# HKUDS/GPT-ST

Hardware: AMD Instinct MI355X
Metric: pretrain steps/sec at (B=32,T=12,N=170,C=64) (higher is better)
Workload: dtype f32; 1 GPU; BASELINE configs[1]: PEMS08-shape synthetic pretrain step, per-GPU B=32 T=12 N=170 C=64 base=1, epoch 200/300 (adaptive mask + KL), fwd+loss+bwd+clip+Adam, hipGraph=True, 4 full optimiser steps on 4 different resident batches per graph replay; global_batch=32, parallelism=dp1

## Files before the change

### gpt-st_amd/csrc/cap_mfma.hip

```cpp
#include "mfma_tile.h"
#include "poolgen_dev.h"
#include <vector>
#ifdef GPTST_DEBUG
__device__ long long g_cap_ts[64];
static thread_local int g_cap_dbg = 0;
extern "C" int gptst_tune2(int v) { g_cap_dbg = v; return 0; }
extern "C" int gptst_cap_ts(long long* out) { return (int)hipMemcpyFromSymbol(out, HIP_SYMBOL(g_cap_ts), sizeof(long long) * 64); }
#else
static constexpr int g_cap_dbg = 0;
#endif

GPTST_STAMP_TABLES(capmfma)
GPTST_HANDOFF_COUNTER(capmfma)

#define CM_NT 512
#define CM_NW (CM_NT / 64)

__host__ __device__ inline int cm_rows(int N) { return (N + 15) / 16 * 16; }
__host__ __device__ inline int cm_np(int N) { return ((N + 3) / 4 * 4) | 1; }
__host__ __device__ inline int cm_hsp(int HS) { return (HS + 15) / 16 * 16; }

template <int C>
__device__ __forceinline__ void cm_type1(const float* __restrict__ Ps, const float* __restrict__ cs, float* __restrict__ S, int N,
                                         int NP, int HSP) {
// ... 499 lines not shown
                const bool valid = i < nz;
                const int k = valid ? i / LPR : 0, c4 = i % LPR;
                const float4 sv = valid ? sv4[u] : f4zero(), rt = valid ? rt4[u] : f4zero(), g = valid ? g4[u] : f4zero();
                const float4 u_ = f4add(rt, sv);
                const float q = group_sum<LPR>(f4dot(u_, u_));
                const float udg = group_sum<LPR>(f4dot(u_, g));
                const float r = sqrtf(q), den = (1.f + q) * (r + 1e-8f);
                const float gq = q / den;
                float gp = 0.f;
                if (r > 0.f) gp = (den - q * ((r + 1e-8f) + (1.f + q) * 0.5f / r)) / (den * den);
                const float k2 = 2.f * gp * udg;
                const float4 du = make_float4(fmaf(k2, u_.x, gq * g.x), fmaf(k2, u_.y, gq * g.y), fmaf(k2, u_.z, gq * g.z), fmaf(k2, u_.w, gq * g.w));
                if (valid) {
                    st4(Gs + k * P + 4 * c4, make_float4(du.x * lrelu_grad_from_out(rt.x), du.y * lrelu_grad_from_out(rt.y),
                                                         du.z * lrelu_grad_from_out(rt.z), du.w * lrelu_grad_from_out(rt.w)));
                    if (k >= k0 && k < k0 + nown) {
                        const float tm = tmpl[k / HS];
                        st4((GLOBAL ? Uo : Vs) + (k - k0) * P + 4 * c4, du);
                        st4(Zo + (k - k0) * P + 4 * c4, make_float4(sv.x + tm, sv.y + tm, sv.z + tm, sv.w + tm));
                    }
                }
            }
        }
        for (int i = CM_NT + tid; i < nd; i += CM_NT) st4(dyns + 4 * i, ld4(db + 4 * (size_t)i));
        for (int i = CM_NT + tid; i < nh; i += CM_NT) st4(Hs + (i / LPR) * P + 4 * (i % LPR), ld4(hb + 4 * (size_t)i));
    }
    __syncthreads();
    {
        const int lane = tid & 63, wave = tid >> 6, li = lane & 15, kk = lane >> 4;
        if (wave < C / 16) {
            for (int jt = 0; jt < HT; jt += 16) {
                const int ja = jt + li;
                f32x4 acc = {0.f, 0.f, 0.f, 0.f};
                const float* ar = dyns + min(ja, HT - 1) * KK + kk;
                const float* br = Gs + kk * P + 16 * wave + li;
                const int ns4 = KK / 4;
                int s4 = 0;
                for (; s4 + 6 <= ns4; s4 += 6) {
                    float av[6], bv[6];
#pragma unroll
                    for (int u = 0; u < 6; ++u) { av[u] = ja < HT ? ar[4 * (s4 + u)] : 0.f; bv[u] = br[4 * (s4 + u) * P]; }
#pragma unroll
                    for (int u = 0; u < 6; ++u) acc = __builtin_amdgcn_mfma_f32_16x16x4f32(av[u], bv[u], acc, 0, 0, 0);
                }
                for (; s4 < ns4; ++s4) acc = __builtin_amdgcn_mfma_f32_16x16x4f32(ja < HT ? ar[4 * s4] : 0.f, br[4 * s4 * P], acc, 0, 0, 0);
#pragma unroll
                for (int r = 0; r < 4; ++r) {
                    const int jj = jt + 4 * kk + r;
                    if (jj < HT) dHs[jj * P + 16 * wave + li] = acc[r] * lrelu_grad_from_out(Hs[jj * P + 16 * wave + li]);
                }
            }
        }
    }
    __syncthreads();
    for (int i = tid; i < HT * nown; i += CM_NT) {
        const int j = i / nown, h = i % nown, k = k0 + h;
        float acc = 0.f;
#pragma unroll 4
        for (int c4 = 0; c4 < LPR; ++c4) {
            acc += f4dot(ld4(Hs + j * P + 4 * c4), ld4(Gs + k * P + 4 * c4));
            acc += f4dot(ld4(dHs + j * P + 4 * c4), ld4(Zo + h * P + 4 * c4));
        }
        ddyn[((size_t)b * HT + j) * KK + k] = acc;
    }
    for (int i = tid; i < nown * LPR; i += CM_NT) {
        const int h = i / LPR, c4 = i % LPR, k = k0 + h;
        float4 acc = f4zero();
#pragma unroll 8
        for (int j = 0; j < HT; ++j) acc = f4fma(dyns[j * KK + k], ld4(dHs + j * P + 4 * c4), acc);
        if (GLOBAL) {
            typedef int i32x4_ __attribute__((ext_vector_type(4)));
            const float4 r4 = f4add(ld4(Uo + h * P + 4 * c4), acc);
            const f32x4 v4 = {r4.x, r4.y, r4.z, r4.w};
            const __amdgpu_buffer_rsrc_t rs = __builtin_amdgcn_make_buffer_rsrc(dSg + ((size_t)b * KK + k0) * C, 0, nown * C * 4, 0x00020000);
            __builtin_amdgcn_raw_buffer_store_b128(__builtin_bit_cast(i32x4_, v4), rs, (h * C + 4 * c4) * 4, 0, 16);
        } else {
            st4(Vs + h * P + 4 * c4, f4add(ld4(Vs + h * P + 4 * c4), acc));
        }
    }
    __syncthreads();
}

template <bool JOBS> struct RouteJobs { };
template <> struct RouteJobs<true> { PJobs t; int npool, npb, neb, first; };

template <int C, int ROLES, bool LIN = false, bool JOBS = false>
__global__ __launch_bounds__(CM_NT, 4) void cap_route_bwd2_kernel(const float* __restrict__ X, const float* __restrict__ Wp,
                                                                  const float* __restrict__ bp, const float* __restrict__ c,
                                                                  const float* __restrict__ dc1, const float* __restrict__ dS,
                                                                  float* __restrict__ dY, float* __restrict__ dlogit, int N, int HS,
                                                                  int region2, CrossBwdArgs cx, LinArgs lin, RouteJobs<JOBS> jr, int nfull, int nhr) {
    if constexpr (JOBS) {
        if ((int)blockIdx.x >= jr.first) {
            extern __shared__ __attribute__((aligned(16))) float jsmem[];
            const int half = (int)(threadIdx.x >> 8), tid_ = (int)(threadIdx.x & 255);
            float (*fold)[PG_MAXK][65] = reinterpret_cast<float (*)[PG_MAXK][65]>(jsmem + half * (4 * PG_MAXK * 65));
            const int w = (int)blockIdx.x - jr.first, wp = (jr.npb + 1) >> 1;
            if (w < wp) {
                const int vb = __builtin_amdgcn_readfirstlane(2 * w + half);
                if (vb < jr.npb) {
                    int p = 0;
                    for (int q = 1; q < jr.npool; ++q) if (vb >= jr.t.j[q].blk0) p = q;
                    const PJob& a = jr.t.j[p];
                    if (((a.cols | a.ldx) & 3) == 0) pj_bwd_pool<4>(a, vb - a.blk0, fold, tid_); else pj_bwd_pool<1>(a, vb - a.blk0, fold, tid_);
                } else {
                    __syncthreads();
                }
            } else {
                const int vb = __builtin_amdgcn_readfirstlane(2 * (w - wp) + half);
                if (vb < jr.neb) {
                    int p = jr.npool;
                    for (int q = jr.npool + 1; q < jr.t.n; ++q) if (vb >= jr.t.j[q].blk0) p = q;
                    const PJob& a = jr.t.j[p];
                    const int rel = vb - a.blk0;
                    if (((a.cols | a.ldx) & 3) == 0) pj_bwd_emb<4>(a, rel % a.nbx, rel / a.nbx, tid_); else pj_bwd_emb<1>(a, rel % a.nbx, rel / a.nbx, tid_);
                }
            }
            return;
        }
    }
    using T = Tile<C>;
    constexpr int P = T::PITCH, LPR = C / 4, RPP = CM_NT / LPR;
    extern __shared__ __attribute__((aligned(16))) float smem[];
    const int NR = cm_rows(N), NP = cm_np(N), HSP = cm_hsp(HS);
    float* Ys = smem;
    float* Wl = Ys + NR * P;
    float* cs = Wl;
    float* dcs = cs + HSP * NP;
    float* Vs = Wl + region2;
    float* gq = Vs + HSP * P;
    float* qq = gq + NR;
    const int tid = threadIdx.x, lane = tid & 63, wave = tid >> 6;
    unsigned* s_ok = reinterpret_cast<unsigned*>(qq + NR);
    GPTST_WG_BEGIN(); GPTST_STAMP(0);
    const int blk = (int)blockIdx.x;
    int ru;
    if (ROLES && blk < cx.nB) {
        constexpr int TS = 12 / CX_SPLIT;
        cap_cross_bwd_prologue<C, true>(cx.dv, cx.s, cx.Rt, cx.Ht, cx.dyn, cx.tmpl, cx.ddyn, smem, nullptr, blk / CX_SPLIT,
                                                    (blk % CX_SPLIT) * TS, TS, cx.T, HS, cx.HT, cx.dSg);
        asm volatile("s_waitcnt vmcnt(0)" ::: "memory");
        __syncthreads();
        if (tid == 0) { gptst_publish_fence(); __hip_atomic_store(cx.flags + blk, 1u, __ATOMIC_RELAXED, __HIP_MEMORY_SCOPE_AGENT); }
        GPTST_STAMP(1);
        if (blk >= nhr) { GPTST_WG_END(); return; }
        ru = nfull + blk;
        __syncthreads();
    } else {
        const int r = ROLES ? blk - cx.nB : blk;
        ru = r < nfull ? r : r + nhr;
    }
    int bt = ru, tlo = 0, thi = NR / 16;
    if (ru >= nfull) {
        const int k = ru - nfull, th = (NR / 16 + 1) >> 1;
        bt = nfull + (k >> 1);
        if (k & 1) tlo = th; else thi = th;
    }
    const float* Xbt = X + (size_t)bt * N * C;
    const bool fold = !ROLES && cx.dv != nullptr;
    if constexpr (!ROLES) {
        if (fold) {
            for (int i = tid; i < HSP * P; i += CM_NT) Vs[i] = 0.f;
            __syncthreads();
            cap_cross_bwd_prologue<C, false>(cx.dv, cx.s, cx.Rt, cx.Ht, cx.dyn, cx.tmpl, cx.ddyn, smem, Vs, bt / cx.T, bt % cx.T, 1, cx.T, HS, cx.HT);
        }
    }
    GPTST_STAMP(1);

    if constexpr (C == 64) {
        const int j = lane & 15, kk = lane >> 4;
        float4 a[4];
        cm_fetch_a16(a, Xbt, tlo + wave, N, j, kk);
        const float4 b4 = ld4(bp + 4 * j);
        load_w_lds<C, CM_NT>(Wl, Wp, 1, tid);
        if (!fold) for (int i = tid; i < HSP * P; i += CM_NT) Vs[i] = 0.f;
        __syncthreads();
        GPTST_STAMP(2);
        float4 bv[4][4];
        cm_load_bfrag(bv, Wl, j, kk);
        for (int tile = tlo + wave; tile < thi; tile += CM_NW) {
            if (tile != tlo + wave) cm_fetch_a16(a, Xbt, tile, N, j, kk);
            float4 y[4];
            cm_tile16(a, bv, b4, y);
#pragma unroll
            for (int r = 0; r < 4; ++r) {
                const int n = tile * 16 + kk * 4 + r;
                const float4 v = n < N ? y[r] : f4zero();
                const float q = group_sum<16>(f4dot(v, v));
                st4(Ys + n * P + 4 * j, v);
                if (j == 0) { qq[n] = q; gq[n] = q / ((1.f + q) * (sqrtf(q) + 1e-8f)); }
            }
        }
        __syncthreads();
        GPTST_STAMP(3);
        for (int i = tid; i < 2 * HSP * NP; i += CM_NT) cs[i] = 0.f;
// ... 245 lines not shown
                const float g0 = (sgn >> (4 * r)) & 1u ? 1.f : LRELU_SLOPE, g1 = (sgn >> (4 * r)) & 2u ? 1.f : LRELU_SLOPE;
                const float g2 = (sgn >> (4 * r)) & 4u ? 1.f : LRELU_SLOPE, g3 = (sgn >> (4 * r)) & 8u ? 1.f : LRELU_SLOPE;
                if (lin.out != nullptr) {
                    o4.x = fmaf(rv[r].x, g0, o4.x); o4.y = fmaf(rv[r].y, g1, o4.y); o4.z = fmaf(rv[r].z, g2, o4.z); o4.w = fmaf(rv[r].w, g3, o4.w);
                } else {
                    o4 = f4add(o4, rv[r]);
                    if (lin.premul) { o4.x *= g0; o4.y *= g1; o4.z *= g2; o4.w *= g3; }
                }
                if (nn < N) st4(lin.dX + ((size_t)bt * N + nn) * 64 + 4 * j_, o4);
            }
        }
#undef CRL_LOAD_RES
        GPTST_STAMP(7);
        {
            const int ot = wave_ >> 1, it0 = 2 * (wave_ & 1);
            f32x4 w0 = {0.f, 0.f, 0.f, 0.f}, w1 = {0.f, 0.f, 0.f, 0.f};
            const float* xcol = Xbt + 16 * it0 + j_;
            const float* ycol = Ys + 16 * ot + j_;
            constexpr int UB = 11;
            const int sbeg = 4 * tlo, nsteps = 4 * thi;
            float b0[UB], b1[UB], n0[UB], n1[UB];
#define CRL_LOADX(d0, d1, s0_) _Pragma("unroll") for (int u = 0; u < UB; ++u) {                          \
                const int n_ = min(4 * ((s0_) + u) + kk_, N - 1);                                          \
                d0[u] = xcol[(size_t)n_ * 64]; d1[u] = xcol[(size_t)n_ * 64 + 16]; }
            CRL_LOADX(b0, b1, sbeg);
#pragma unroll 1
            for (int s0 = sbeg; s0 < nsteps; s0 += UB) {
                if (s0 + UB < nsteps) { CRL_LOADX(n0, n1, s0 + UB); }
                float av[UB];
#pragma unroll
                for (int u = 0; u < UB; ++u) av[u] = (s0 + u < nsteps) ? ycol[(4 * (s0 + u) + kk_) * P] : 0.f;
                SB();
#pragma unroll
                for (int u = 0; u < UB; ++u) {
                    w0 = __builtin_amdgcn_mfma_f32_16x16x4f32(av[u], b0[u], w0, 0, 0, 0);
                    w1 = __builtin_amdgcn_mfma_f32_16x16x4f32(av[u], b1[u], w1, 0, 0, 0);
                }
                SB();
#pragma unroll
                for (int u = 0; u < UB; ++u) { b0[u] = n0[u]; b1[u] = n1[u]; }
            }
#undef CRL_LOADX
            float* dw = lin.dWp + (size_t)ru * 64 * 64;
#pragma unroll
            for (int r = 0; r < 4; ++r) {
                const int o = 16 * ot + 4 * kk_ + r;
                dw[o * 64 + 16 * it0 + j_] = w0[r];
                dw[o * 64 + 16 * it0 + 16 + j_] = w1[r];
            }
        }
        GPTST_STAMP(8);
    }
    GPTST_WG_END();
}

thread_local int g_cap_split_roles = 1;
thread_local int g_cap_bwd_noroles = 0;

template <int C>
static int launch_route_bwd2(const float* X, const float* Wp, const float* bp, const float* c, const float* dc1, const float* dS,
                             float* dY, float* dlogit, int BT, int N, int HS, hipStream_t st, CrossBwdArgs cx = CrossBwdArgs{nullptr, nullptr, nullptr, nullptr, nullptr, nullptr, nullptr, 0, 0, nullptr, nullptr, 0},
                             LinArgs lin = LinArgs{nullptr, nullptr, nullptr, nullptr, nullptr, 0}, RouteJobs<true>* jobs = nullptr, int nsplit = 0) {
    if (HS > 64) return GPTST_ESHAPE;
    if (nsplit < 0 || nsplit > BT || (nsplit > 0 && (C != 64 || lin.dX == nullptr))) return GPTST_EARG;
    const int nfull = BT - nsplit;
    if (lin.dX != nullptr && C != 64) return GPTST_ESHAPE;
    const int NR = cm_rows(N), NP = cm_np(N), HSP = cm_hsp(HS);
    size_t r2 = (size_t)C * C, need = (size_t)2 * HSP * NP;
    if (need > r2) r2 = need;
    r2 = (r2 + 3) & ~(size_t)3;
    const size_t smem = ((size_t)NR * Tile<C>::PITCH + r2 + (size_t)HSP * Tile<C>::PITCH + 2 * (size_t)NR + 4) * sizeof(float);
    if (smem > 160 * 1024) return GPTST_ESHAPE;
    if (cx.dv) {
        const size_t need_cx = (size_t)(cx.T * HS + 2 * cx.HT + HS) * Tile<C>::PITCH + (size_t)cx.HT * cx.T * HS;
        if (need_cx > (size_t)NR * Tile<C>::PITCH + r2 || (cx.HT * cx.T * HS) % 4 != 0) return GPTST_ESHAPE;
    }
    if (cx.nB > 0) {
        const int no = (12 / CX_SPLIT) * HS;
        const size_t need_r = (size_t)(cx.T * HS + 2 * cx.HT + 2 * no) * Tile<C>::PITCH + (size_t)cx.HT * cx.T * HS;
        if (smem > 80 * 1024 || BT + cx.nB > 512 || cx.T != 12 || need_r > (size_t)NR * Tile<C>::PITCH + r2) cx.nB = 0;
    }
    const int nhr = (cx.nB > 0 && g_cap_split_roles) ? (2 * nsplit < cx.nB ? 2 * nsplit : cx.nB) : 0;
    const int NU = BT + nsplit - nhr;
    if (jobs != nullptr && !(cx.nB > 0 && lin.dX != nullptr && smem >= 2 * (4 * PG_MAXK * 65) * sizeof(float))) return GPTST_ESHAPE;
    if (jobs != nullptr) {
        static size_t curJ = 0;
        if (smem > curJ) { (void)hipFuncSetAttribute((const void*)cap_route_bwd2_kernel<C, 1, true, true>, hipFuncAttributeMaxDynamicSharedMemorySize, (int)smem); curJ = smem; }
        jobs->first = NU + cx.nB;
        const int njw = ((jobs->npb + 1) >> 1) + ((jobs->neb + 1) >> 1);
        hipLaunchKernelGGL((cap_route_bwd2_kernel<C, 1, true, true>), dim3(NU + cx.nB + njw), dim3(CM_NT), smem, st, X, Wp, bp, c, dc1, dS, dY, dlogit, N, HS, (int)r2, cx, lin, *jobs, nfull, nhr);
        GPTST_CHECK_LAUNCH();
        return GPTST_OK;
    }
    if (cx.nB > 0 && lin.dX != nullptr) {
        static size_t curRL = 0;
        if (smem > curRL) { (void)hipFuncSetAttribute((const void*)cap_route_bwd2_kernel<C, 1, true>, hipFuncAttributeMaxDynamicSharedMemorySize, (int)smem); curRL = smem; }
        hipLaunchKernelGGL((cap_route_bwd2_kernel<C, 1, true>), dim3(NU + cx.nB), dim3(CM_NT), smem, st, X, Wp, bp, c, dc1, dS, dY, dlogit, N, HS, (int)r2, cx, lin, RouteJobs<false>{}, nfull, nhr);
        GPTST_CHECK_LAUNCH();
        return GPTST_OK;
    }
    if (cx.nB > 0) {
        static size_t curR = 0;
        if (smem > curR) { (void)hipFuncSetAttribute((const void*)cap_route_bwd2_kernel<C, 1>, hipFuncAttributeMaxDynamicSharedMemorySize, (int)smem); curR = smem; }
        hipLaunchKernelGGL((cap_route_bwd2_kernel<C, 1>), dim3(BT + cx.nB), dim3(CM_NT), smem, st, X, Wp, bp, c, dc1, dS, dY, dlogit, N, HS, (int)r2, cx, lin, RouteJobs<false>{}, BT, 0);
        GPTST_CHECK_LAUNCH();
        return GPTST_OK;
    }
    if (lin.dX != nullptr) {
        static size_t curL = 0;
        if (smem > curL) { (void)hipFuncSetAttribute((const void*)cap_route_bwd2_kernel<C, 0, true>, hipFuncAttributeMaxDynamicSharedMemorySize, (int)smem); curL = smem; }
        hipLaunchKernelGGL((cap_route_bwd2_kernel<C, 0, true>), dim3(NU), dim3(CM_NT), smem, st, X, Wp, bp, c, dc1, dS, dY, dlogit, N, HS, (int)r2, cx, lin, RouteJobs<false>{}, nfull, nhr);
        GPTST_CHECK_LAUNCH();
        return GPTST_OK;
    }
    static size_t cur = 0;
    if (smem > cur) { (void)hipFuncSetAttribute((const void*)cap_route_bwd2_kernel<C, 0>, hipFuncAttributeMaxDynamicSharedMemorySize, (int)smem); cur = smem; }
    hipLaunchKernelGGL((cap_route_bwd2_kernel<C, 0>), dim3(BT), dim3(CM_NT), smem, st, X, Wp, bp, c, dc1, dS, dY, dlogit, N, HS, (int)r2, cx, lin, RouteJobs<false>{}, BT, 0);
    GPTST_CHECK_LAUNCH();
    return GPTST_OK;
}

GPTST_INTERNAL int gptst_cap_route_bwd_v1(const float* X, const float* Wp, const float* bp, const float* c, const float* dc1,
                                      const float* dS, float* dY, float* dlogit, int BT, int N, int C, int HS, void* stream);

extern "C" int gptst_cap_route_bwd(const float* X, const float* Wp, const float* bp, const float* c, const float* dc1,
                                   const float* dS, float* dY, float* dlogit, int BT, int N, int C, int HS, void* stream) {
    if (!X || !Wp || !bp || !c || !dc1 || !dS || !dY || !dlogit) return GPTST_EARG;
    int rc = GPTST_ESHAPE;
    if (C == 64) rc = launch_route_bwd2<64>(X, Wp, bp, c, dc1, dS, dY, dlogit, BT, N, HS, (hipStream_t)stream);
    if (rc == GPTST_ESHAPE) return gptst_cap_route_bwd_v1(X, Wp, bp, c, dc1, dS, dY, dlogit, BT, N, C, HS, stream);
    return rc;
}

extern "C" int gptst_cap_cross_route_bwd(const float* X, const float* Wp, const float* bp, const float* c, const float* dc1, const float* dv,
                                         const float* s, const float* Rt, const float* Ht, const float* dyn, const float* tmpl, float* dY,
                                         float* dlogit, float* ddyn, float* dS_ws, void* flags, int B, int T, int N, int C, int HS, int HT, void* stream) {
    if (!X || !Wp || !bp || !c || !dc1 || !dv || !s || !Rt || !Ht || !dyn || !tmpl || !dY || !dlogit || !ddyn || B <= 0 || T <= 0) return GPTST_EARG;
    if (C != 64) return GPTST_ESHAPE;
    const bool roles = dS_ws != nullptr && flags != nullptr && !g_cap_bwd_noroles;
    return launch_route_bwd2<64>(X, Wp, bp, c, dc1, nullptr, dY, dlogit, B * T, N, HS, (hipStream_t)stream,
                                 CrossBwdArgs{dv, s, Rt, Ht, dyn, tmpl, ddyn, T, HT, roles ? dS_ws : nullptr, roles ? (unsigned*)flags : nullptr, roles ? B * CX_SPLIT : 0});
}

extern "C" int gptst_cap_cross_route_lin_bwd(const float* X, const float* Wp, const float* bp, const float* c, const float* dc1, const float* dv,
                                             const float* s, const float* Rt, const float* Ht, const float* dyn, const float* tmpl,
                                             const float* dPre, const float* out, int premul, float* dX, float* dWp, float* dbp, float* dlogit,
                                             float* ddyn, float* dS_ws, void* flags, int B, int T, int N, int C, int HS, int HT, void* stream) {
    if (!X || !Wp || !bp || !c || !dc1 || !dv || !s || !Rt || !Ht || !dyn || !tmpl || !dPre || !dX || !dWp || !dbp || !dlogit || !ddyn || B <= 0 ||
        T <= 0 || (out && premul)) return GPTST_EARG;
    if (C != 64) return GPTST_ESHAPE;
    const bool roles = dS_ws != nullptr && flags != nullptr && !g_cap_bwd_noroles;
    return launch_route_bwd2<64>(X, Wp, bp, c, dc1, nullptr, nullptr, dlogit, B * T, N, HS, (hipStream_t)stream,
                                 CrossBwdArgs{dv, s, Rt, Ht, dyn, tmpl, ddyn, T, HT, roles ? dS_ws : nullptr, roles ? (unsigned*)flags : nullptr, roles ? B * CX_SPLIT : 0},
                                 LinArgs{dPre, out, dX, dWp, dbp, premul});
}

GPTST_INTERNAL int gptst_cap_rec_bwd_v1(const float* drec, const float* c, const float* v, float* dc1, float* dv, int BT, int N, int C,
                                    int HS, void* stream);

GPTST_INTERNAL int gptst_pj_reduce_table(PJobs* t, int njobs, const int* kind, const void* const* emb, const void* const* x, const void* const* pool,
                                         const void* const* out, const int* R, const int* K, const int* cols, const int* nsplit, const int* ldx,
                                         int* npool, int* npb, int* neb);
extern "C" int gptst_pool_jobs(int njobs, const int* kind, const void* const* emb, const void* const* x, const void* const* pool,
                               const void* const* out, const int* R, const int* K, const int* cols, const int* nsplit, const int* ldx, void* stream);
extern "C" int gptst_cap_route_roles_ok(int B, int T, int N, int C, int HS, int HT) {
    if (C != 64 || HS > 64 || HS <= 0 || B <= 0 || N <= 0 || T != 12 || g_cap_bwd_noroles) return 0;
    const int NR = cm_rows(N), NP = cm_np(N), HSP = cm_hsp(HS), BT = B * T, nB = B * CX_SPLIT;
    size_t r2 = (size_t)C * C, need = (size_t)2 * HSP * NP;
    if (need > r2) r2 = need;
    r2 = (r2 + 3) & ~(size_t)3;
    const size_t smem = ((size_t)NR * Tile<64>::PITCH + r2 + (size_t)HSP * Tile<64>::PITCH + 2 * (size_t)NR + 4) * sizeof(float);
    const int no = (12 / CX_SPLIT) * HS;
    const size_t need_r = (size_t)(T * HS + 2 * HT + 2 * no) * Tile<64>::PITCH + (size_t)HT * T * HS;
    if (smem > 80 * 1024 || BT + nB > 512 || need_r > (size_t)NR * Tile<64>::PITCH + r2 || (HT * T * HS) % 4 != 0) return 0;
    return smem >= 2 * (4 * PG_MAXK * 65) * sizeof(float) ? 1 : 0;
}

thread_local int g_cap_split = 0;
static int cap_cu_count() {
    static thread_local int dev_cached = -1, ncu = 0;
    int dev = 0;
    if (hipGetDevice(&dev) != hipSuccess) return 0;
    if (dev != dev_cached) {
        if (hipDeviceGetAttribute(&ncu, hipDeviceAttributeMultiprocessorCount, dev) != hipSuccess) ncu = 0;
        dev_cached = dev;
    }
    return ncu;
}
extern "C" int gptst_cap_split_units(int BT, int N, int C, int HS) {
    if (C != 64 || HS <= 0 || HS > 64 || N < 32 || BT <= 0) return 0;
    if (g_cap_split >= 0) return g_cap_split < BT ? g_cap_split : BT;
    const int ncu = cap_cu_count();
    if (ncu <= 0 || BT <= ncu || 2 * BT > 3 * ncu) return 0;
    return BT - ncu;
}

static int cap_cross_route_lin_bwd_any(const float* X, const float* Wp, const float* bp, const float* c, const float* dc1, const float* dv,
                                       const float* s, const float* Rt, const float* Ht, const float* dyn, const float* tmpl,
                                       const float* dPre, const float* out, int premul, float* dX, float* dWp, float* dbp, float* dlogit,
                                       float* ddyn, float* dS_ws, void* flags, int B, int T, int N, int C, int HS, int HT, int nsplit,
                                       int njobs, const int* jkind, const void* const* jemb, const void* const* jx, const void* const* jpool,
                                       const void* const* jout, const int* jR, const int* jK, const int* jcols, const int* jnsplit, const int* jldx,
                                       void* stream) {
    if (!X || !Wp || !bp || !c || !dc1 || !dv || !s || !Rt || !Ht || !dyn || !tmpl || !dPre || !dX || !dWp || !dbp || !dlogit || !ddyn || B <= 0 ||
        T <= 0 || (out && premul) || nsplit < 0 || nsplit > B * T) return GPTST_EARG;
    if (njobs < 0 || (njobs && (!jkind || !jemb || !jx || !jpool || !jout || !jR || !jK || !jcols || !jnsplit))) return GPTST_EARG;
    if (C != 64) return GPTST_ESHAPE;
    if (nsplit > 0 && N < 32) return GPTST_EARG;
    const bool roles = dS_ws != nullptr && flags != nullptr && !g_cap_bwd_noroles;
    const CrossBwdArgs cx{dv, s, Rt, Ht, dyn, tmpl, ddyn, T, HT, roles ? dS_ws : nullptr, roles ? (unsigned*)flags : nullptr, roles ? B * CX_SPLIT : 0};
    const LinArgs lin{dPre, out, dX, dWp, dbp, premul};
    if (njobs > 0 && roles) {
        RouteJobs<true> jr;
        if (gptst_pj_reduce_table(&jr.t, njobs, jkind, jemb, jx, jpool, jout, jR, jK, jcols, jnsplit, jldx, &jr.npool, &jr.npb, &jr.neb) == GPTST_OK) {
            const int rc = launch_route_bwd2<64>(X, Wp, bp, c, dc1, nullptr, nullptr, dlogit, B * T, N, HS, (hipStream_t)stream, cx, lin, &jr, nsplit);
            if (rc != GPTST_ESHAPE) return rc;
        }
    }
    const int rc = launch_route_bwd2<64>(X, Wp, bp, c, dc1, nullptr, nullptr, dlogit, B * T, N, HS, (hipStream_t)stream, cx, lin, nullptr, nsplit);
    if (rc || njobs == 0) return rc;
    return gptst_pool_jobs(njobs, jkind, jemb, jx, jpool, jout, jR, jK, jcols, jnsplit, jldx, stream);
}

extern "C" int gptst_cap_cross_route_lin_bwd_jobs(const float* X, const float* Wp, const float* bp, const float* c, const float* dc1, const float* dv,
                                                  const float* s, const float* Rt, const float* Ht, const float* dyn, const float* tmpl,
                                                  const float* dPre, const float* out, int premul, float* dX, float* dWp, float* dbp, float* dlogit,
                                                  float* ddyn, float* dS_ws, void* flags, int B, int T, int N, int C, int HS, int HT,
                                                  int njobs, const int* jkind, const void* const* jemb, const void* const* jx, const void* const* jpool,
                                                  const void* const* jout, const int* jR, const int* jK, const int* jcols, const int* jnsplit, const int* jldx,
                                                  void* stream) {
    return cap_cross_route_lin_bwd_any(X, Wp, bp, c, dc1, dv, s, Rt, Ht, dyn, tmpl, dPre, out, premul, dX, dWp, dbp, dlogit, ddyn, dS_ws, flags, B, T, N, C, HS,
                                       HT, 0, njobs, jkind, jemb, jx, jpool, jout, jR, jK, jcols, jnsplit, jldx, stream);
}

extern "C" int gptst_cap_cross_route_lin_bwd_split(const float* X, const float* Wp, const float* bp, const float* c, const float* dc1, const float* dv,
                                                   const float* s, const float* Rt, const float* Ht, const float* dyn, const float* tmpl,
                                                   const float* dPre, const float* out, int premul, float* dX, float* dWp, float* dbp, float* dlogit,
                                                   float* ddyn, float* dS_ws, void* flags, int B, int T, int N, int C, int HS, int HT, int nsplit,
                                                   int njobs, const int* jkind, const void* const* jemb, const void* const* jx, const void* const* jpool,
                                                   const void* const* jout, const int* jR, const int* jK, const int* jcols, const int* jnsplit, const int* jldx,
                                                   void* stream) {
    return cap_cross_route_lin_bwd_any(X, Wp, bp, c, dc1, dv, s, Rt, Ht, dyn, tmpl, dPre, out, premul, dX, dWp, dbp, dlogit, ddyn, dS_ws, flags, B, T, N, C, HS,
                                       HT, nsplit, njobs, jkind, jemb, jx, jpool, jout, jR, jK, jcols, jnsplit, jldx, stream);
}

extern "C" int gptst_cap_rec_bwd(const float* drec, const float* c, const float* v, float* dc1, float* dv, int BT, int N, int C, int HS,
                                 void* stream) {
    if (!drec || !c || !v || !dc1 || !dv) return GPTST_EARG;
    if (C == 64 && HS <= 64) {
        const int NR = cm_rows(N), NP = cm_np(N), HSP = cm_hsp(HS);
        const size_t smem = ((size_t)NR * Tile<64>::PITCH + (size_t)(HSP + HS) * NP + (size_t)HSP * Tile<64>::PITCH + (size_t)HSP * 64) * sizeof(float);
        if (smem <= 160 * 1024) {
            static size_t cur = 0;
            if (smem > cur) { hipFuncSetAttribute((const void*)cap_rec_bwd2_kernel<64>, hipFuncAttributeMaxDynamicSharedMemorySize, (int)smem); cur = smem; }
            hipLaunchKernelGGL((cap_rec_bwd2_kernel<64>), dim3(BT), dim3(CM_NT), smem, (hipStream_t)stream, drec, c, v, dc1, dv, N, HS);
            GPTST_CHECK_LAUNCH();
            return GPTST_OK;
        }
    }
    return gptst_cap_rec_bwd_v1(drec, c, v, dc1, dv, BT, N, C, HS, stream);
}
```

### gpt-st_amd/csrc/poolgen.hip

```cpp
#include "common.h"
#include "poolgen_dev.h"
#include <algorithm>
#include <vector>

#define PG_ROWS 16


#ifndef PJ_OCC
#define PJ_OCC 6
#endif

#define PG_MAXROWS 64
template <int V>
__device__ __forceinline__ void pj_fwd(const PJob& a, int bx, int by, int rows, float* __restrict__ embs ) {
    const float* __restrict__ emb = a.emb;
    const float* __restrict__ pool = a.pool;
    float* __restrict__ out = a.out;
    const int cols = a.cols, K = a.K, R = a.R;
    const int r0 = by * rows, nr = min(R, r0 + rows) - r0;
    for (int i = threadIdx.x; i < nr * PG_MAXK; i += 256) {
        const int r = i / PG_MAXK, k = i % PG_MAXK;
        embs[i] = k < K ? emb[(size_t)(r0 + r) * K + k] : 0.f;
    }
    const int c4 = bx * 256 + threadIdx.x;
    const bool ok = V * c4 < cols;
    float4 pv[PG_MAXK];
#pragma unroll
    for (int k = 0; k < PG_MAXK; ++k) pv[k] = (k < K && ok) ? ldv<V>(pool + (size_t)k * cols + V * c4) : f4zero();
    __syncthreads();
    if (!ok) return;
#pragma unroll 2
    for (int r = 0; r < nr; ++r) {
        float4 acc = f4zero();
#pragma unroll
        for (int k = 0; k < PG_MAXK; k += 4) {
            const float4 e = ld4(embs + r * PG_MAXK + k);
            acc = f4fma(e.x, pv[k], acc); acc = f4fma(e.y, pv[k + 1], acc); acc = f4fma(e.z, pv[k + 2], acc); acc = f4fma(e.w, pv[k + 3], acc);
        }
        stv<V>(out + (size_t)(r0 + r) * cols + V * c4, acc);
    }
}




#define PJ_DET_T 1024
__global__ __launch_bounds__(PJ_DET_T) void pool_emb_det_kernel(PJobs t) {
    __shared__ float fold[PJ_DET_T / 64][16][17];
    const int lane = threadIdx.x & 63, wave = threadIdx.x >> 6;
    const int i = lane & 15, kk = lane >> 4;
    int q0 = 0;
    for (int q = 1; q < t.n; ++q) if ((int)blockIdx.x >= t.j[q].blk0) q0 = q;
    const int g0 = t.j[q0].blk0, tile = blockIdx.x - g0;
    f32x4 acc = {0.f, 0.f, 0.f, 0.f};
    int chunk_id = 0, first = q0;
    for (int q = 0; q <= q0; ++q) {
        const PJob& a = t.j[q];
        if (a.blk0 != g0) continue;
        if (q < first) first = q;
        const bool v4 = ((a.cols | a.ldx) & 3) == 0;
        const int nch = (a.cols + 255) / 256;
        for (int ch = 0; ch < nch; ++ch, ++chunk_id) {
            if ((chunk_id & (PJ_DET_T / 64 - 1)) != wave) continue;
            if (v4) pj_emb_accum<4>(a, tile, ch, acc, threadIdx.x); else pj_emb_accum<1>(a, tile, ch, acc, threadIdx.x);
        }
    }
#pragma unroll
    for (int r = 0; r < 4; ++r) fold[wave][kk * 4 + r][i] = acc[r];
    __syncthreads();
    if (threadIdx.x < 256) {
        const int R = t.j[first].R, K = t.j[first].K;
        const int rr = threadIdx.x >> 4, k = threadIdx.x & 15, orow = tile * 16 + rr;
        float s = 0.f;
#pragma unroll
        for (int w = 0; w < PJ_DET_T / 64; ++w) s += fold[w][rr][k];
        if (orow < R && k < K) t.j[first].out[(size_t)orow * K + k] += s;
    }
}

__global__ __launch_bounds__(256, PJ_OCC) void pool_jobs_kernel(PJobs t, int fwd_rows, int fwd_mfma) {
    __shared__ __attribute__((aligned(16))) float fold[4][PG_MAXK][65];
    int p = 0;
    for (int q = 1; q < t.n; ++q) if ((int)blockIdx.x >= t.j[q].blk0) p = q;
    const PJob& a = t.j[p];
    const int rel = blockIdx.x - a.blk0, bx = rel % a.nbx, by = rel / a.nbx;
    const bool v4 = ((a.cols | a.ldx) & 3) == 0;
    if (a.kind == PJ_FWD) {
        if (v4 && fwd_mfma) pj_fwd_mfma(a, bx, by, fwd_mfma, threadIdx.x);
        else if (v4) pj_fwd<4>(a, bx, by, fwd_rows, &fold[0][0][0]);
        else pj_fwd<1>(a, bx, by, fwd_rows, &fold[0][0][0]);
    }
    else if (a.kind == PJ_GRAM) pj_gram(a, rel, &fold[0][0][0], 256);
    else if (a.kind == PJ_BWD_POOL) { if (v4) pj_bwd_pool<4>(a, bx, fold, threadIdx.x); else pj_bwd_pool<1>(a, bx, fold, threadIdx.x); }
    else { if (v4) pj_bwd_emb<4>(a, bx, by, threadIdx.x); else pj_bwd_emb<1>(a, bx, by, threadIdx.x); }
}

thread_local int g_pg_rows = PG_ROWS;
thread_local int g_pg_sort = 1;
thread_local int g_pg_mfma = 1;
static int pj_blocks(PJob& j) {
    const int V = ((j.cols | j.ldx) & 3) ? 1 : 4;
    if (j.kind == PJ_FWD && V == 4 && g_pg_mfma) { j.nbx = (j.cols + 255) / 256; return j.nbx * ((j.R + PG_MFMA_ROWS - 1) / PG_MFMA_ROWS); }
    if (j.kind == PJ_FWD) { j.nbx = ((j.cols + V - 1) / V + 255) / 256; return j.nbx * ((j.R + g_pg_rows - 1) / g_pg_rows); }
    if (j.kind == PJ_GRAM) { const int nb = pj_gram_rows(j.K, j.cols); j.nbx = (j.R + nb - 1) / nb; return j.nbx; }
    if (j.kind == PJ_BWD_POOL) { j.nbx = (j.cols + 16 * V - 1) / (16 * V); return j.nbx; }
    j.nbx = (j.R + 15) / 16;
    return j.nbx * (((j.cols + 255) / 256 + 3) / 4);
}

extern "C" int gptst_pool_jobs_gram_rows(int K, int cols) { return (K <= 0 || K > PG_MAXK || cols <= 0 || cols % 12) ? 0 : pj_gram_rows(K, cols); }

static int pj_launch(PJobs& t, hipStream_t st) {
    int nb = 0;
    for (int p = 0; p < t.n; ++p) {
        PJob& j = t.j[p];
        if (j.R <= 0 || j.K <= 0 || j.K > PG_MAXK || j.cols <= 0 || j.nsplit <= 0 || !j.out) return GPTST_EARG;
        if ((j.kind == PJ_FWD || j.kind == PJ_BWD_POOL || j.kind == PJ_GRAM) && !j.emb) return GPTST_EARG;
        if (j.kind == PJ_GRAM && (!j.pool || j.cols % 12 || pj_gram_rows(j.K, j.cols) <= 0)) return GPTST_EARG;
        if ((j.kind == PJ_BWD_POOL || j.kind == PJ_BWD_EMB) && !j.x) return GPTST_EARG;
        if ((j.kind == PJ_FWD || j.kind == PJ_BWD_EMB) && !j.pool) return GPTST_EARG;
        j.blk0 = nb;
        if (j.ldx <= 0) j.ldx = j.cols;
        if (j.ldx < j.cols) return GPTST_EARG;
        nb += pj_blocks(j);
    }
    if (nb == 0) return GPTST_OK;
    hipLaunchKernelGGL(pool_jobs_kernel, dim3(nb), dim3(256), 0, st, t, g_pg_rows, g_pg_mfma ? PG_MFMA_ROWS : 0);
    GPTST_CHECK_LAUNCH();
    return GPTST_OK;
}

GPTST_INTERNAL int gptst_pj_embed_table(PJobs* t, int njobs, const int* kind, const void* const* emb, const void* const* pool, const void* const* out,
                                        const int* R, const int* K, const int* cols, int* nf, int* nvb, int* ngw) {
    if (njobs > PJ_MAX || !g_pg_mfma) return GPTST_ESHAPE;
    t->n = 0;
    *nf = *nvb = *ngw = 0;
    for (int pass = 0; pass < 2; ++pass) {
        for (int p = 0; p < njobs; ++p) {
            const int kd = kind ? kind[p] : (int)PJ_FWD;
            if (kd != PJ_FWD && kd != PJ_GRAM) return GPTST_ESHAPE;
            if ((kd == PJ_GRAM) != (pass == 1)) continue;
            PJob j{(const float*)emb[p], nullptr, (const float*)pool[p], (float*)out[p], R[p], K[p], cols[p], 1, 0, kd, 0, cols[p]};
            if (!j.emb || !j.pool || !j.out || j.R <= 0 || j.K <= 0 || j.K > PG_MAXK || j.cols <= 0) return GPTST_EARG;
            if (kd == PJ_FWD) {
                if (j.cols & 3) return GPTST_ESHAPE;
                j.blk0 = *nvb; *nvb += pj_blocks(j); ++*nf;
            } else {
                if (j.cols % 12 || pj_gram_rows(j.K, j.cols) <= 0) return GPTST_EARG;
                j.blk0 = *ngw; *ngw += pj_blocks(j);
            }
            t->j[t->n++] = j;
        }
    }
    return GPTST_OK;
}

GPTST_INTERNAL int gptst_pj_reduce_table(PJobs* t, int njobs, const int* kind, const void* const* emb, const void* const* x, const void* const* pool,
                                         const void* const* out, const int* R, const int* K, const int* cols, const int* nsplit, const int* ldx,
                                         int* npool, int* npb, int* neb) {
    if (njobs > PJ_MAX || g_deterministic) return GPTST_ESHAPE;
    t->n = 0;
    *npool = *npb = *neb = 0;
    for (int pass = 0; pass < 2; ++pass) {
        for (int p = 0; p < njobs; ++p) {
            if (kind[p] != PJ_BWD_POOL && kind[p] != PJ_BWD_EMB) return GPTST_ESHAPE;
            if ((kind[p] == PJ_BWD_EMB) != (pass == 1)) continue;
            PJob j{(const float*)emb[p], (const float*)x[p], (const float*)pool[p], (float*)out[p], R[p], K[p], cols[p], nsplit[p], 0, kind[p], 0, ldx ? ldx[p] : 0};
            if (j.R <= 0 || j.K <= 0 || j.K > PG_MAXK || j.cols <= 0 || j.nsplit <= 0 || !j.out || !j.x) return GPTST_EARG;
            if (kind[p] == PJ_BWD_POOL ? !j.emb : !j.pool) return GPTST_EARG;
            if (j.ldx <= 0) j.ldx = j.cols;
            if (j.ldx < j.cols) return GPTST_EARG;
            if (pass == 0) { j.blk0 = *npb; *npb += pj_blocks(j); ++*npool; }
            else { j.blk0 = *neb; *neb += pj_blocks(j); }
            t->j[t->n++] = j;
        }
    }
    return GPTST_OK;
}

extern "C" int gptst_pool_jobs(int njobs, const int* kind, const void* const* emb, const void* const* x, const void* const* pool,
                               const void* const* out, const int* R, const int* K, const int* cols, const int* nsplit, const int* ldx,
                               void* stream) {
    if (njobs < 0 || (njobs && (!kind || !emb || !x || !pool || !out || !R || !K || !cols || !nsplit))) return GPTST_EARG;
    for (int p = 0; p < njobs; ++p) if (kind[p] < PJ_FWD || kind[p] > PJ_GRAM) return GPTST_EARG;
    auto job = [&](int p) {
        return PJob{(const float*)emb[p], (const float*)x[p], (const float*)pool[p], (float*)out[p], R[p], K[p], cols[p], nsplit[p],
                    0, kind[p], 0, ldx ? ldx[p] : 0};
    };
    const bool det = g_deterministic != 0;
    std::vector<int> ord(njobs);
    std::vector<long> cost(njobs);
    for (int p = 0; p < njobs; ++p) {
        ord[p] = p;
        const long rr = (long)R[p] * nsplit[p], cc = cols[p];
        cost[p] = kind[p] == PJ_BWD_POOL ? rr * (cc < 64 ? cc : 64) : kind[p] == PJ_BWD_EMB ? 16L * nsplit[p] * (cc < 1024 ? cc : 1024)
                : kind[p] == PJ_FWD ? 64L * (cc < 256 ? cc : 256) : 1L;
    }
    if (g_pg_sort) std::stable_sort(ord.begin(), ord.end(), [&](int a, int b) { return cost[a] > cost[b]; });
    PJobs t; t.n = 0;
    for (int o = 0; o < njobs; ++o) {
        const int p = ord[o];
        if (det && kind[p] == PJ_BWD_EMB) continue;
        t.j[t.n++] = job(p);
        if (t.n == PJ_MAX) { const int rc = pj_launch(t, (hipStream_t)stream); if (rc) return rc; t.n = 0; }
    }
    if (t.n) { const int rc = pj_launch(t, (hipStream_t)stream); if (rc) return rc; }
    if (!det) return GPTST_OK;
    PJobs g; g.n = 0;
    int nb = 0;
    auto flush = [&]() {
        if (g.n) { hipLaunchKernelGGL(pool_emb_det_kernel, dim3(nb), dim3(PJ_DET_T), 0, (hipStream_t)stream, g); g.n = 0; nb = 0; }
    };
    for (int p = 0; p < njobs; ++p) {
        if (kind[p] != PJ_BWD_EMB) continue;
        bool seen = false;
        for (int q = 0; q < p; ++q) if (kind[q] == PJ_BWD_EMB && out[q] == out[p]) seen = true;
        if (seen) continue;
        int members = 0;
        for (int q = p; q < njobs; ++q) if (kind[q] == PJ_BWD_EMB && out[q] == out[p]) ++members;
        if (members > PJ_MAX) return GPTST_EARG;
        if (g.n + members > PJ_MAX) flush();
        const int tiles = (R[p] + 15) / 16;
        for (int q = p; q < njobs; ++q) {
            if (kind[q] != PJ_BWD_EMB || out[q] != out[p]) continue;
            if (R[q] != R[p] || K[q] != K[p]) return GPTST_EARG;
            PJob j = job(q);
            if (!j.x || !j.pool || !j.out || j.R <= 0 || j.K <= 0 || j.K > PG_MAXK || j.cols <= 0 || j.nsplit <= 0) return GPTST_EARG;
            if (j.ldx <= 0) j.ldx = j.cols;
            if (j.ldx < j.cols) return GPTST_EARG;
            j.blk0 = nb; j.nbx = tiles;
            g.j[g.n++] = j;
        }
        nb += tiles;
    }
    flush();
    GPTST_CHECK_LAUNCH();
    return GPTST_OK;
}

extern thread_local int g_wgrad_ns_override;
extern thread_local int g_wgrad_ns0_override;
extern thread_local int g_apply_v1;
extern thread_local int g_apply_tpw;
extern thread_local int g_tl_nb;
extern thread_local int g_wgrad_v1;
extern thread_local int g_apply128_v1;
extern thread_local int g_apply128_minwg;
extern thread_local int g_tl_mfma;
extern thread_local int g_cap_route_v2;
extern thread_local int g_cap_bwd_noroles;
extern thread_local int g_cap_split;
extern thread_local int g_cap_split_roles;
extern "C" int gptst_tune(int id, int value) {
    if (id == 15) g_tl_mfma = value;
    if (id == 20) g_cap_route_v2 = value;
    if (id == 23) g_cap_bwd_noroles = value;
    if (id == 25) g_cap_split = value;
    if (id == 26) g_cap_split_roles = value;
    if (id == 19) g_pg_sort = value;
    if (id == 1 && value > 0 && value <= PG_MAXROWS) g_pg_rows = value;
    if (id == 6 && value > 0) g_tl_nb = value;
    if (id == 2) g_wgrad_ns_override = value;
    if (id == 5) g_wgrad_ns0_override = value;
    if (id == 3) g_apply_v1 = value;
    if (id == 4) g_apply_tpw = value;
    if (id == 7) g_wgrad_v1 = value;
    if (id == 8) g_apply128_v1 = value;
    if (id == 24 && value > 0) g_apply128_minwg = value;
    if (id == 10) g_pg_mfma = value;
    return GPTST_OK;
}

extern "C" int gptst_poolgen_fwd_multi(const float* emb, int nprob, const void* pools, const void* outs, const int* cols, int R, int K,
                                       void* stream) {
    if (!emb || !pools || !outs || !cols || nprob <= 0 || nprob > PJ_MAX || K > PG_MAXK || K <= 0) return GPTST_EARG;
    PJobs t; t.n = nprob;
    for (int p = 0; p < nprob; ++p)
        t.j[p] = PJob{emb, nullptr, ((const float* const*)pools)[p], ((float* const*)outs)[p], R, K, cols[p], 1, 0, PJ_FWD, 0, 0};
    return pj_launch(t, (hipStream_t)stream);
}

extern "C" int gptst_poolgen_bwd_pool_multi(const float* emb, int nprob, const void* dWs, const void* dpools, const int* cols,
                                            const int* nsplit, int R, int K, void* stream) {
    if (!emb || !dWs || !dpools || !cols || nprob <= 0 || nprob > PJ_MAX || K > PG_MAXK || K <= 0) return GPTST_EARG;
    PJobs t; t.n = nprob;
    for (int p = 0; p < nprob; ++p)
        t.j[p] = PJob{emb, ((const float* const*)dWs)[p], nullptr, ((float* const*)dpools)[p], R, K, cols[p], nsplit ? nsplit[p] : 1, 0,
                      PJ_BWD_POOL, 0, 0};
    return pj_launch(t, (hipStream_t)stream);
}

extern "C" int gptst_poolgen_bwd_emb_multi(int nprob, const void* dWs, const void* pools, const int* cols, const int* nsplit, float* demb,
                                           int R, int K, void* stream) {
    if (!dWs || !pools || !cols || !demb || nprob <= 0 || nprob > PJ_MAX || K > PG_MAXK || K <= 0) return GPTST_EARG;
    PJobs t; t.n = nprob;
    for (int p = 0; p < nprob; ++p)
        t.j[p] = PJob{nullptr, ((const float* const*)dWs)[p], ((const float* const*)pools)[p], demb, R, K, cols[p], nsplit ? nsplit[p] : 1, 0,
                      PJ_BWD_EMB, 0, 0};
    return pj_launch(t, (hipStream_t)stream);
}

extern "C" int gptst_poolgen_fwd(const float* emb, const float* pool, float* out, int cols, const float* pool2, float* out2,
                                 int cols2, int R, int K, void* stream) {
    const float* pools[2] = {pool, pool2}; float* outs[2] = {out, out2}; int cc[2] = {cols, cols2};
    return gptst_poolgen_fwd_multi(emb, pool2 ? 2 : 1, pools, outs, cc, R, K, stream);
}

extern "C" int gptst_poolgen_bwd_pool(const float* emb, const float* dW, float* dpool, int cols, const float* dW2, float* dpool2,
                                      int cols2, int R, int nsplit, int K, void* stream) {
    const float* dWs[2] = {dW, dW2}; float* dps[2] = {dpool, dpool2}; int cc[2] = {cols, cols2}; int ns[2] = {nsplit, 1};
    return gptst_poolgen_bwd_pool_multi(emb, dW2 ? 2 : 1, dWs, dps, cc, ns, R, K, stream);
}

extern "C" int gptst_poolgen_bwd_emb(const float* dW, const float* pool, int cols, const float* dW2, const float* pool2, int cols2,
                                     float* demb, int R, int nsplit, int K, void* stream) {
    const float* dWs[2] = {dW, dW2}; const float* pls[2] = {pool, pool2}; int cc[2] = {cols, cols2}; int ns[2] = {nsplit, 1};
    return gptst_poolgen_bwd_emb_multi(dW2 ? 2 : 1, dWs, pls, cc, ns, demb, R, K, stream);
}
```

### gpt-st_amd/csrc/poolgen_dev.h

```cpp
#pragma once
#include "common.h"

#define PG_MAXK 16
#define PG_MFMA_ROWS 64
#define PJ_MAX 112
enum { PJ_FWD = 0, PJ_BWD_POOL = 1, PJ_BWD_EMB = 2, PJ_GRAM = 3 };
struct PJob {
    const float* emb;
    const float* x;
    const float* pool;
    float* out;
    int R, K, cols, nsplit;
    int blk0, kind, nbx, ldx;
};
struct PJobs { PJob j[PJ_MAX]; int n; };

__device__ __forceinline__ void pj_fwd_mfma(const PJob& a, int bx, int by, int rows, int tid) {
    const float* __restrict__ emb = a.emb;
    const float* __restrict__ pool = a.pool;
    float* __restrict__ out = a.out;
    const int cols = a.cols, K = a.K, R = a.R;
    const int lane = tid & 63, wave = tid >> 6, j = lane & 15, kk = lane >> 4;
    const int c = bx * 256 + wave * 64 + 4 * j;
    if (bx * 256 + wave * 64 >= cols) return;
    const bool cok = c < cols;
    const int nks = (K + 3) >> 2;
    float4 bf[4];
#pragma unroll
    for (int s = 0; s < 4; ++s) bf[s] = (cok && 4 * s + kk < K) ? ld4(pool + (size_t)(4 * s + kk) * cols + c) : f4zero();
    const int r0 = by * rows, r1 = min(R, r0 + rows);
    for (int rt = r0; rt < r1; rt += 16) {
        float av[4];
        const int row = rt + j;
#pragma unroll
        for (int s = 0; s < 4; ++s) av[s] = (row < r1 && 4 * s + kk < K) ? emb[(size_t)row * K + 4 * s + kk] : 0.f;
        f32x4 acc[4];
#pragma unroll
        for (int ct = 0; ct < 4; ++ct) acc[ct] = (f32x4){0.f, 0.f, 0.f, 0.f};
#pragma unroll
        for (int s = 0; s < 4; ++s) {
            if (s < nks) {
                acc[0] = __builtin_amdgcn_mfma_f32_16x16x4f32(av[s], bf[s].x, acc[0], 0, 0, 0);
                acc[1] = __builtin_amdgcn_mfma_f32_16x16x4f32(av[s], bf[s].y, acc[1], 0, 0, 0);
                acc[2] = __builtin_amdgcn_mfma_f32_16x16x4f32(av[s], bf[s].z, acc[2], 0, 0, 0);
                acc[3] = __builtin_amdgcn_mfma_f32_16x16x4f32(av[s], bf[s].w, acc[3], 0, 0, 0);
            }
        }
        if (cok) {
#pragma unroll
            for (int r = 0; r < 4; ++r) {
                const int orow = rt + 4 * kk + r;
                if (orow < r1) st4(out + (size_t)orow * cols + c, make_float4(acc[0][r], acc[1][r], acc[2][r], acc[3][r]));
            }
        }
    }
}

#define PJ_GRAM_SCR (4 * PG_MAXK * 65)
__host__ __device__ inline int pj_gram_rows(int K, int cols) {
    const int nb = (PJ_GRAM_SCR - K * cols) / cols;
    return nb > 16 ? 16 : nb;
}
__device__ __forceinline__ void pj_gram(const PJob& a, int bx, float* __restrict__ scr, int nt) {
    const int K = a.K, cols = a.cols, Hm = cols / 12, NB = pj_gram_rows(K, cols);
    float* pl = scr;
    float* As = scr + K * cols;
    const int r0 = bx * NB, nr = min(NB, a.R - r0);
    for (int i = threadIdx.x; i < K * cols; i += nt) pl[i] = a.pool[i];
    __syncthreads();
    for (int i = threadIdx.x; i < nr * cols; i += nt) {
        const int r = i / cols, c = i % cols;
        const float* __restrict__ e = a.emb + (size_t)(r0 + r) * K;
        float acc = 0.f;
        for (int k = 0; k < K; ++k) acc = fmaf(e[k], pl[k * cols + c], acc);
        As[i] = acc;
    }
    __syncthreads();
    for (int i = threadIdx.x; i < nr * 144; i += nt) {
        const int r = i / 144, t = (i % 144) / 12, u = i % 12;
        const float* ar = As + r * cols;
        float s = 0.f;
        for (int h = 0; h < Hm; ++h) s = fmaf(ar[h * 12 + t], ar[h * 12 + u], s);
        a.out[(size_t)(r0 + r) * 144 + i % 144] = s;
    }
}

#ifndef PJ_UC
#define PJ_UC 4
#endif
#ifndef PJ_NU
#define PJ_NU 4
#endif
template <int V> __device__ __forceinline__ float4 ldv(const float* p) { return ld4(p); }
template <> __device__ __forceinline__ float4 ldv<1>(const float* p) { return make_float4(*p, 0.f, 0.f, 0.f); }
template <int V> __device__ __forceinline__ void stv(float* p, float4 v) { st4(p, v); }
template <> __device__ __forceinline__ void stv<1>(float* p, float4 v) { *p = v.x; }

// ... 40 lines not shown
        }
    }
#pragma unroll
    for (int e = 0; e < V; ++e)
#pragma unroll
        for (int r = 0; r < 4; ++r) fold[wave][kk * 4 + r][V * j + e] = acc[e][r];
    __syncthreads();
    for (int o = tid; o < PG_MAXK * SLAB; o += 256) {
        const int k = o / SLAB, cc = o % SLAB, col = bx * SLAB + cc;
        if (k < K && col < cols) {
            float* d = dpool + (size_t)k * cols + col;
            *d += (fold[0][k][cc] + fold[1][k][cc]) + (fold[2][k][cc] + fold[3][k][cc]);
        }
    }
}

template <int V>
__device__ __forceinline__ void pj_emb_accum(const PJob& a, int bx, int chunk, f32x4& acc, int tid) {
    constexpr int chunk_cols = 256;
    const int lane = tid & 63;
    const int i = lane & 15, kk = lane >> 4;
    const int R = a.R, K = a.K;
    const int row = bx * 16 + i;
    const float* __restrict__ w = a.x;
    const float* __restrict__ pl = a.pool;
    const int cc = a.cols, ns = a.nsplit, ldx = a.ldx;
    const int cbeg = chunk * chunk_cols, cend = min(cc, cbeg + chunk_cols);
    if (cbeg >= cc) return;
    if (V == 4) {
        constexpr int UC = PJ_UC;
        const int rowc = min(row, R - 1), ic = min(i, K - 1);
        const bool rok = row < R, kok = i < K;
        for (int c0 = cbeg; c0 < cend; c0 += 16 * UC) {
            float4 av[UC], b[UC];
#pragma unroll
            for (int u = 0; u < UC; ++u) {
                const int c = min(c0 + 16 * u + 4 * kk, cc - 4);
                av[u] = ld4(w + (size_t)rowc * ldx + c);
                b[u] = ld4(pl + (size_t)ic * cc + c);
            }
            for (int s = 1; s < ns; ++s) {
#pragma unroll
                for (int u = 0; u < UC; ++u) {
                    const int c = min(c0 + 16 * u + 4 * kk, cc - 4);
                    av[u] = f4add(av[u], ld4(w + ((size_t)s * R + rowc) * ldx + c));
                }
            }
            SB();
#pragma unroll
            for (int u = 0; u < UC; ++u) {
                const bool ok = c0 + 16 * u + 4 * kk < cend;
                const float4 a_ = (ok && rok) ? av[u] : f4zero();
                const float4 b_ = (ok && kok) ? b[u] : f4zero();
                acc = __builtin_amdgcn_mfma_f32_16x16x4f32(a_.x, b_.x, acc, 0, 0, 0);
                acc = __builtin_amdgcn_mfma_f32_16x16x4f32(a_.y, b_.y, acc, 0, 0, 0);
                acc = __builtin_amdgcn_mfma_f32_16x16x4f32(a_.z, b_.z, acc, 0, 0, 0);
                acc = __builtin_amdgcn_mfma_f32_16x16x4f32(a_.w, b_.w, acc, 0, 0, 0);
            }
        }
    } else {
        for (int c = cbeg + kk; c < cend + kk; c += 4) {
            float av = 0.f, b = 0.f;
            if (c < cend) {
                if (row < R) for (int s = 0; s < ns; ++s) av += w[((size_t)s * R + row) * ldx + c];
                if (i < K) b = pl[(size_t)i * cc + c];
            }
            acc = __builtin_amdgcn_mfma_f32_16x16x4f32(av, b, acc, 0, 0, 0);
        }
    }
}

template <int V>
__device__ __forceinline__ void pj_bwd_emb(const PJob& a, int bx, int by, int tid) {
    const int lane = tid & 63, wave = tid >> 6;
    const int i = lane & 15, kk = lane >> 4;
    f32x4 acc = {0.f, 0.f, 0.f, 0.f};
    pj_emb_accum<V>(a, bx, by * 4 + wave, acc, tid);
#pragma unroll
    for (int r = 0; r < 4; ++r) {
        const int orow = bx * 16 + kk * 4 + r;
        if (orow < a.R && i < a.K && (by * 4 + wave) * 256 < a.cols) atomicAdd(a.out + (size_t)orow * a.K + i, acc[r]);
    }
}
```

### gpt-st_amd/engine.py

```python
import contextlib
import os
import threading

import torch

from . import _C, ops
from .ops import (EPI_ADD_DPRE, EPI_ADD_PREMUL, EPI_LRELU, EPI_PREMUL, EPI_PLAIN, EPI_RES_LRELU, MODE_NODE, MODE_SHARED, MODE_TIME, PRO_DPRE, PRO_NONE)

TF_NAMES = ("ln_day", "ln_week", "ln1", "ln2", "ln")


class ZeroArena:

    def __init__(self, device):
        self.device, self.buf, self.off, self.need = device, None, 0, 0

    def begin(self, zero=True):
        pending = None
        if self.buf is None or self.buf.numel() < self.need:
            self.buf = torch.zeros(max(self.need, 1), device=self.device) if self.need else None
        elif self.buf is not None:
            if zero:
                self.buf.zero_()
            else:
                pending = self.buf
        self.off, self.need = 0, 0
        return pending

    def zeros(self, *shape):
        n = 1
        for d in shape:
            n *= d
        n4 = (n + 3) // 4 * 4
        self.need += n4
        if self.buf is None or self.off + n4 > self.buf.numel():
            return torch.zeros(*shape, device=self.device)
        t = self.buf[self.off:self.off + n].view(*shape)
        self.off += n4
        return t


class _Context(threading.local):
    ARENA = None
    NODE_REDUCE = None
    NO_HANDOFFS = False


CTX = _Context()




class Reductions:

    def __init__(self):
        self.jobs = ops.PoolJobs()
        self.late = ops.PoolJobs()
        self.no_carry = False
        self.grams = []
        self.tf = []
        self.keep = []
        self.on_bucket = None
        self.nbucket = 0

    def take_carry(self, mb):
        if not CARRY_RED or self.no_carry or self.on_bucket is not None or CTX.NODE_REDUCE is not None or not self.jobs.jobs:
            return None
        take, rest, nb = [], [], 0.0
        for j in self.jobs.jobs:
            b = 4.0 * j[5] * j[7] * j[8] / 2 ** 20
            if j[0] in (ops.PoolJobs.BWD_POOL, ops.PoolJobs.BWD_EMB) and nb + b <= mb and len(take) < 100 and (j[7] | j[9]) % 4 == 0:
                take.append(j); nb += b
            else:
                rest.append(j)
        if not take:
            return None
        self.jobs.jobs = rest
        c = ops.PoolJobs()
        c.jobs = take
        return c

    def untake(self, carry):
        if carry is not None and carry.jobs:
            self.jobs.jobs = carry.jobs + self.jobs.jobs
            carry.jobs = []

    def gram(self, A, dG, dA, N, nsG):
        self.grams.append((A, dG, dA, N, nsG))

    def timefeat(self, p, g, pfx, tidx, dout, spg=False):
        B, T = tidx.shape[0], tidx.shape[1]
        rows, K = (B, T) if spg else (B * T, 1)
        self.tf.append((_tf_tensors(p, pfx), _tf_tensors(g, pfx), dout, rows, K))

    def flush_async(self, tidx):
        if getattr(self, "bucket_inline", False) and self.on_bucket is not None and self.nbucket == 0 and (self.jobs.jobs or self.late.jobs or self.grams or self.tf):
            self._run(tidx)
            self.fork_side.wait_stream(torch.cuda.current_stream())
            with torch.cuda.stream(self.fork_side):
                self.on_bucket(0)
            self.forked = True
            self.nbucket += 1

    def flush(self, tidx):
        self._run(tidx)
        if getattr(self, "forked", False):
            torch.cuda.current_stream().wait_stream(self.fork_side)
            self.forked = False

    def _run(self, tidx):
        gr, self.grams = sorted(self.grams, key=lambda t: t[0].data_ptr()), []
        while gr:
            A, dG, dA, N, nsG = gr.pop(0)
            while gr and gr[0][0].data_ptr() == A.data_ptr() + 4 * A.numel() and gr[0][1].data_ptr() == dG.data_ptr() + 4 * dG.numel() \
                    and gr[0][2].data_ptr() == dA.data_ptr() + 4 * dA.numel() and gr[0][3:] == (N, nsG):
                A2, dG2, dA2 = gr.pop(0)[:3]
                A = torch.as_strided(A, (A.shape[0] + A2.shape[0],) + tuple(A.shape[1:]), A.stride())
                dG = torch.as_strided(dG, (dG.shape[0] + dG2.shape[0],) + tuple(dG.shape[1:]), dG.stride())
                dA = torch.as_strided(dA, (dA.shape[0] + dA2.shape[0],) + tuple(dA.shape[1:]), dA.stride())
            ops.gram_bwd(A, dG, out=dA, layers=A.shape[0] // N, nsplit=nsG)
        self.jobs.jobs, self.late.jobs = self.jobs.jobs + self.late.jobs, []
        self.jobs.launch()
        tf, self.tf = self.tf, []
        ops.timefeat_jobs_bwd(tf, tidx)
        self.keep = []


def _zeros(ref, *shape):
    if CTX.ARENA is not None:
        return CTX.ARENA.zeros(*shape)
    return torch.zeros(*shape, device=ref.device)


def _tf_tensors(d, pfx):
    out = []
    for n in TF_NAMES:
        out += [d[pfx + n + ".weight"], d[pfx + n + ".bias"]]
    return out


def _tf_job(p, pfx, tidx, spg=False):
    B, T = tidx.shape[0], tidx.shape[1]
    rows, K = (B, T) if spg else (B * T, 1)
    return (_tf_tensors(p, pfx), rows, K)


DROP_R = os.environ.get("GPTST_DROP_R", "0") == "1"


def _ht_fused_bwd(dims):
    return dims[3] == 64 and FUSE_HT_BWD


def hypertem_core_fwd(x, G, Wbt, bbt, dims):
    B, T, N, C = dims
    if C == 64:
        keep = not (DROP_R and _ht_fused_bwd(dims) and ops.wgrad_nsplit(MODE_TIME, B * T, N, C) == 1)
        R, out = ops.hypertem_fwd(x.view(B, T, N, C), G, Wbt, bbt, want_R=keep)
        R, out = (R.view(-1, C) if keep else None), out.view(-1, C)
    else:
        R = ops.tmix(x.view(B, T, N, C), G).view(-1, C)
        out = ops.apply(R, Wbt, MODE_TIME, B * T, N, bias=bbt, resid=x, epi=EPI_RES_LRELU)
    return out, (x, R, out, G, Wbt)


FUSE_HT_BWD = True


def graph_grad_splits(dims):
    return dims[0] if dims[3] == 64 else 1


CHAIN128 = os.environ.get("GPTST_CHAIN128", "1") == "1"


def chain_ok(dims):
    return _ht_fused_bwd(dims) or (CHAIN128 and dims[3] == 128)


def hypertem_core_bwd(saved, dout, dG_out, dims, chain=False, premul=False):
    B, T, N, C = dims
    x, R, out, G, Wbt = saved
    BT = B * T
    assert not chain or chain_ok(dims)
    if _ht_fused_bwd(dims):
        dx, dWb, ns, _ = ops.hypertem_bwd_wgrad(dout.view(B, T, N, C), None if chain else out.view(B, T, N, C), x.view(B, T, N, C), G, Wbt,
                                                R.view(B, T, N, C) if R is not None else None, dG=dG_out, premul=chain and premul)
        dWbt, dbias, nsb = dWb[:, :C * C], dWb[:, C * C:], ns
        dx = dx.view(-1, C)
    elif C == 64:
        dWb, ns = ops.wgrad(R, dout, MODE_TIME, BT, N, D2=out, pro=PRO_DPRE, colsum_d=True)
        dWbt, dbias, nsb = dWb[:, :C * C], dWb[:, C * C:], ns
        dx, _, _ = ops.hypertem_bwd(dout.view(B, T, N, C), out.view(B, T, N, C), x.view(B, T, N, C), G, Wbt, dG=dG_out, want_dbias=False)
        dx = dx.view(-1, C)
    elif chain:
        dWb, ns = ops.wgrad(R, dout, MODE_TIME, BT, N, colsum_d=True)
        dWbt, dbias, nsb = dWb[:, :C * C], dWb[:, C * C:], ns
        dR = ops.apply(dout, Wbt, MODE_TIME, BT, N, transw=True)
        dx, _ = ops.tmix_bwd_chain(dR.view(B, T, N, C), x.view(B, T, N, C), G, dout.view(B, T, N, C), premul=premul, dG=dG_out[0])
        dx = dx.view(-1, C)
    else:
        dWb, ns = ops.wgrad(R, dout, MODE_TIME, BT, N, D2=out, pro=PRO_DPRE, colsum_d=True)
        dWbt, dbias, nsb = dWb[:, :C * C], dWb[:, C * C:], ns
        dR = ops.apply(dout, Wbt, MODE_TIME, BT, N, A2=out, transw=True, pro=PRO_DPRE)
        dx, _ = ops.tmix_bwd(dR.view(B, T, N, C), x.view(B, T, N, C), G, dout.view(B, T, N, C), out.view(B, T, N, C), dG=dG_out[0])
        dx = dx.view(-1, C)
    return dx, (dWbt, ns, (dbias, nsb))


CARRY_RED = os.environ.get("GPTST_CARRY_RED", "1") == "1"
CARRY_MB = float(os.environ.get("GPTST_CARRY_MB", "25"))
CARRY_KL = os.environ.get("GPTST_CARRY_KL", "1") == "1"
PAIR_UNDER_DP = os.environ.get("GPTST_PAIR_UNDER_DP", "1") == "1"
PAIR_BWD = os.environ.get("GPTST_PAIR_BWD", "1") == "1"


@contextlib.contextmanager
def no_handoffs():
    from . import _C
    keep = (CTX.NO_HANDOFFS, _C.lib().value("gptst_mask_cooperative_state"))
    CTX.NO_HANDOFFS = True
    _C.lib().call("gptst_mask_cooperative", 0)
    try:
        yield
    finally:
        CTX.NO_HANDOFFS = keep[0]
        _C.lib().call("gptst_mask_cooperative", keep[1])


def pair_bwd_on():
    return PAIR_BWD and not CTX.NO_HANDOFFS


def cross_role():
    return 0 if CTX.NO_HANDOFFS else CROSS_ROLE


def _ht_pair_shape_ok(dims):
    B, T, N, C = dims
    if T != 12 or C != 64:
        return False
    ns = ops.wgrad_nsplit(MODE_TIME, B * T, N, C)
    rps = (-(-N // ns) + 1) & ~1
    return -(-N // rps) == ns


def ht_pair_ok(saved1, saved0, dims):
    return (pair_bwd_on() and dims[3] == 64 and not isinstance(saved1, EncIn) and saved1[1] is not None and saved0[1] is not None
            and _ht_fused_bwd(dims) and _ht_pair_shape_ok(dims))


class PendingH1:

    def __init__(self, saved, dd, dG, dWb):
        self.saved, self.dd, self.dG, self.dWb = saved, dd, dG, dWb


def ht_pair_bwd(saved1, saved0, dout, dG1, dG0, dims, dWb1=None):
    B, T, N, C = dims
    if not ht_pair_ok(saved1, saved0, dims):
        assert dWb1 is None
        return None
    x1, R1, _, G1, Wbt1 = saved1
    x0, R0, _, G0, Wbt0 = saved0
    v = lambda a: a.view(B, T, N, C)
    r = ops.hypertem_bwd_pair(v(dout), v(x1), G1, Wbt1, v(R1), v(x0), G0, Wbt0, v(R0), dG1, dG0, _zeros(dout, B), dWb1=dWb1)
    assert r is not None or dWb1 is None
    if r is None:
        return None
    dmid, dx0, dWb1, dWb0, ns = r
    return dx0.view(-1, C), (dWb1[:, :C * C], ns, (dWb1[:, C * C:], ns)), (dWb0[:, :C * C], ns, (dWb0[:, C * C:], ns))


FUSE_CROSS = os.environ.get("GPTST_FUSE_CROSS", "1") == "1"
CAP_LIN = os.environ.get("GPTST_CAP_LIN", "1") == "1"
CROSS_ROLE = int(os.environ.get("GPTST_CROSS_ROLE", "1"))


def cap_head_fwd(p, pfx, x, dadj, dyn, dims, num_route, HS, HT):
    B, T, N, C = dims
    c, s, Y = ops.cap_route_fwd(x.view(B, T, N, C), p[pfx + "ln_p.weight"], p[pfx + "ln_p.bias"], dadj, HS, num_route,
                                reduce_nodes=CTX.NODE_REDUCE, want_Y=True)
    fused = ops.cap_cross_rec_fwd(s, dyn, p[pfx + "mask_template"], c, B, T, N, HS, HT) if (FUSE_CROSS and CTX.NODE_REDUCE is None) else None
    if fused is not None:
        v, Ht, Rt, rec = fused
    else:
        v, Ht, Rt = ops.cap_cross_fwd(s, dyn, p[pfx + "mask_template"], B, T, HS, HT)
        rec = ops.cap_rec_fwd(c, v, N, C)
    return rec, c, (s, v, Ht, Rt, Y)


def cap_core_fwd(p, pfx, x, dadj, dyn, Wn, bn, dims, num_route, HS, HT):
# ... 30 lines not shown
        drec, dWn, dbn, ns = ops.apply_wgrad(dout, None if chain else out, rec, Wn, MODE_NODE, BT, N)
        nsb = ns
    elif chain:
        drec = ops.apply(dout, Wn, MODE_NODE, BT, N, transw=True)
        dWb, ns = ops.wgrad(rec, dout, MODE_NODE, BT, N, colsum_d=True)
        dWn, dbn, nsb = dWb[:, :C * C], dWb[:, C * C:], ns
    else:
        drec = ops.apply(dout, Wn, MODE_NODE, BT, N, A2=out, transw=True, pro=PRO_DPRE)
        dWb, ns = ops.wgrad(rec, dout, MODE_NODE, BT, N, D2=out, pro=PRO_DPRE, colsum_d=True)
        dWn, dbn, nsb = dWb[:, :C * C], dWb[:, C * C:], ns
    fused = None
    dc1, dv = ops.cap_rec_bwd(drec, c, v, reduce_nodes=CTX.NODE_REDUCE)
    gw, gb = g[pfx + "ln_p.weight"], g[pfx + "ln_p.bias"]
    if fused is None and FUSE_CROSS and CAP_LIN and C == 64 and CTX.NODE_REDUCE is None and Y is None:
        carry = red.take_carry(CARRY_MB) if cross_role() and _C.lib().value("gptst_cap_route_roles_ok", B, T, N, C, HS, HT) == 1 else None
        lin = ops.cap_cross_route_lin_bwd(x.view(B, T, N, C), p[pfx + "ln_p.weight"], p[pfx + "ln_p.bias"], c, dc1, dv, s, Rt, Ht, dyn,
                                          p[pfx + "mask_template"], dout, None if chain else out, chain, B, T, HS, HT,
                                          flags=_zeros(x, 4 * B) if cross_role() else None, jobs=carry)
        red.untake(carry)
        if lin is not None:
            dx, dWp, dbp, dlogit, ddyn = lin
            red.jobs.bwd_pool(_ones(dev, dWp.shape[0]), dWp, gw.view(1, C * C))
            red.jobs.bwd_pool(_ones(dev, dbp.shape[0]), dbp, gb.view(1, C))
            return dx, (dWn, ns, (dbn, nsb), ddyn, dlogit)
    if fused is None and FUSE_CROSS and CTX.NODE_REDUCE is None and Y is None:
        fused = ops.cap_cross_route_bwd(x.view(B, T, N, C), p[pfx + "ln_p.weight"], p[pfx + "ln_p.bias"], c, dc1, dv, s, Rt, Ht, dyn,
                                        p[pfx + "mask_template"], B, T, HS, HT, flags=_zeros(x, 4 * B) if cross_role() else None)
    if fused is not None:
        dY, dlogit, ddyn = fused
    else:
        dS, ddyn = ops.cap_cross_bwd(dv, s, Rt, Ht, dyn, p[pfx + "mask_template"], B, T, HS, HT)
        dY, dlogit = ops.cap_route_bwd(x.view(B, T, N, C), p[pfx + "ln_p.weight"], p[pfx + "ln_p.bias"], c, dc1, dS, Y=Y)
    if C == 64:
        dx, dWp, dbp, ns2 = ops.linear_bwd(dY, x, p[pfx + "ln_p.weight"], dout, None if chain else out, premul=chain)
        red.jobs.bwd_pool(_ones(dev, ns2), dWp, gw.view(1, C * C))
        red.jobs.bwd_pool(_ones(dev, ns2), dbp, gb.view(1, C))
    else:
        if chain:
            dx = ops.apply(dY, p[pfx + "ln_p.weight"], MODE_SHARED, BT, N, resid=dout, resid2=x, epi=EPI_ADD_PREMUL)
        else:
            dx = ops.apply(dY, p[pfx + "ln_p.weight"], MODE_SHARED, BT, N, resid=dout, resid2=out, epi=EPI_ADD_DPRE)
        dWp, ns2 = ops.wgrad(dY, x, MODE_SHARED, BT, N, colsum_a=True)
        red.jobs.bwd_pool(_ones(dev, ns2), dWp[:, :C * C], gw.view(1, C * C))
        red.jobs.bwd_pool(_ones(dev, ns2), dWp[:, C * C:], gb.view(1, C))
    return dx, (dWn, ns, (dbn, nsb), ddyn, dlogit)


_ONES = {}


def _ones(dev, n=1):
    if (dev, n) not in _ONES:
        _ONES[(dev, n)] = torch.ones(n, 1, device=dev)
    return _ONES[(dev, n)]


def condlin_fwd(x, Wg, bg, mode, dims):
    B, T, N, C = dims
    out = ops.apply(x, Wg, mode, B * T, N, bias=bg, epi=EPI_LRELU)
    return out, (x, out, Wg)


def condlin_bwd(saved, dout, emb, wpool, bpool, g_wpool, g_bpool, d_emb, mode, dims, red, chain=False, premul=False, carried=None):
    B, T, N, C = dims
    x, out, Wg = saved
    R, K = emb.shape
    assert not chain or chain_ok(dims)
    if carried is not None:
        dx, dW, db, ns = carried
        nsb = ns
    elif C == 64:
        dx, dW, db, ns = ops.apply_wgrad(dout, None if chain else out, x, Wg, mode, B * T, N, premul=chain and premul)
        nsb = ns
    elif chain:
        dx = (ops.apply(dout, Wg, mode, B * T, N, transw=True, resid2=x, epi=EPI_PREMUL) if premul
              else ops.apply(dout, Wg, mode, B * T, N, transw=True))
        dWb, ns = ops.wgrad(x, dout, mode, B * T, N, colsum_d=True)
        dW, db, nsb = dWb[:, :C * C], dWb[:, C * C:], ns
    else:
        dx = ops.apply(dout, Wg, mode, B * T, N, A2=out, transw=True, pro=PRO_DPRE)
        dWb, ns = ops.wgrad(x, dout, mode, B * T, N, D2=out, pro=PRO_DPRE, colsum_d=True)
        dW, db, nsb = dWb[:, :C * C], dWb[:, C * C:], ns
    dW = dW if dW.dim() == 2 else dW.view(ns * R, C * C)
    red.jobs.bwd_pool(emb, dW, g_wpool.view(K, C * C), nsplit=ns)
    red.jobs.bwd_pool(emb, db, g_bpool, nsplit=nsb)
    red.jobs.bwd_emb(dW, wpool.view(K, C * C), d_emb, nsplit=ns)
    red.jobs.bwd_emb(db, bpool, d_emb, nsplit=nsb)
    return dx


ENC, DEC = "encoder.STHCN_encode.", "decoder.STHCN_decode."
GUIDE_TF = "encoder.teb4mask."


def _sthcn_names(pfx):
    return [pfx + "hyperTem%d." % i for i in (1, 2, 3, 4)], [pfx + "cap1.", pfx + "cap2."]


def _sthcn_gen_jobs(p, pfx, emb, jobs, A_all, dims, G_all=None, gjobs=None):
    gjobs = jobs if gjobs is None else gjobs
    B, T, N, C = dims
    time_eb, teb, tes = emb
    ne, nes = p[pfx + "node_embeddings"], p[pfx + "node_embeddings_spg"]
    hts, cps = _sthcn_names(pfx)
    adj0 = p[hts[0] + "adj"]
    d, Hm = adj0.shape[0], adj0.shape[1]
    cadj, tadj = p[cps[0] + "adj"], p[cps[0] + "t_adj"]
    ds, HS, HT = cadj.shape[0], cadj.shape[1], tadj.shape[1]
    for i, h in enumerate(hts):
        jobs.fwd(ne, p[h + "adj"].view(d, Hm * T), out=A_all[i])
        if G_all is not None:
            gjobs.gram(ne, p[h + "adj"].view(d, Hm * T), out=G_all[i], A=A_all[i])
    Wb = [jobs.fwd(time_eb, t) for h in hts for t in (p[h + "weights_pool"], p[h + "bias_pool"])]
    Wn = [jobs.fwd(nes, t) for c in cps for t in (p[c + "weights_spa"], p[c + "bias_spa"])]
    dadj = [jobs.fwd(teb, p[c + "adj"].view(ds, HS * N)) for c in cps]
    dyn = [jobs.fwd(tes, p[c + "t_adj"].view(ds, HT * T * HS)).view(B, HT, T * HS) for c in cps]
    return dict(emb=emb, gen=(A_all, hts, cps, d, Hm, ds, HS, HT), Wb=Wb, Wn=Wn, dadj=dadj, dyn=dyn)


def gen_all(p, tidx, dims, which=(ENC, DEC), guide=True, defer=False):
    B, T, N, C = dims
    tfj = []
    for pfx in which:
        tfj += [_tf_job(p, pfx + "time_feature1.", tidx), _tf_job(p, pfx + "time_feature1_.", tidx),
                _tf_job(p, pfx + "time_feature2.", tidx, spg=True)]
    if guide:
        tfj.append(_tf_job(p, GUIDE_TF, tidx))
    embs = ops.timefeat_jobs_fwd(tfj, tidx)
    jobs = ops.PoolJobs()
    now = ops.PoolJobs() if defer else jobs
    res = {}
    L = 4 * len(which)
    if guide:
        gj = now
        m = "encoder.MLP_RL."
        t4m = embs[-1]
        res["guide"] = (t4m, gj.fwd(p["encoder.neb4mask"], p[m + "weights_pool_spa"]), gj.fwd(p["encoder.neb4mask"], p[m + "bias_pool_spa"]),
                        gj.fwd(t4m, p[m + "weights_pool_tem"]), gj.fwd(t4m, p[m + "bias_pool_tem"]))
    if L:
        adj0 = p[which[0] + "hyperTem1.adj"]
        Hm = adj0.shape[1]
        A_all = torch.empty(L, N, Hm * T, device=tidx.device)
        G_all = torch.empty(L, N, T, T, device=tidx.device)
        for k, pfx in enumerate(which):
            res[pfx] = _sthcn_gen_jobs(p, pfx, embs[3 * k:3 * k + 3], jobs, A_all[4 * k:4 * k + 4], dims, G_all[4 * k:4 * k + 4])
            res[pfx]["slot"] = (k, len(which))
            res[pfx]["G_all"] = G_all[4 * k:4 * k + 4]

    if defer:
        now.launch()
        res["pending"] = jobs
        return res
    jobs.launch()
    return res


def sthcn_fwd(p, pfx, tidx, x, dims, num_route, gen=None, head=None, next_gen=None, kl=None):
    if gen is None:
        gen = gen_all(p, tidx, dims, which=(pfx,), guide=False)[pfx]
    A_all, hts, cps, d, Hm, ds, HS, HT = gen["gen"]
    G_all, Wb, Wn, dadj, dyn = gen["G_all"], gen["Wb"], gen["Wn"], gen["dadj"], gen["dyn"]
    sv = {}
    nhead = None
    if head is not None:
        x, sv["h1"] = head
    else:
        x, sv["h1"] = hypertem_core_fwd(x, G_all[0], Wb[0], Wb[1], dims)
    if chain_fwd_ok(dims):
        x, c1, sv["c1"] = cap_core_fwd(p, cps[0], x, dadj[0], dyn[0], Wn[0], Wn[1], dims, num_route, HS, HT)
        if kl is not None and kl.c1 is None:
            kl.c1 = c1
        (sv["h2"], sv["h3"]), x = ht_chain_fwd(x, [(G_all[1], Wb[2], Wb[3]), (G_all[2], Wb[4], Wb[5])], dims, kl)
        x, _, sv["c2"] = cap_core_fwd(p, cps[1], x, dadj[1], dyn[1], Wn[2], Wn[3], dims, num_route, HS, HT)
        if next_gen is not None:
            hs, xl = ht_chain_fwd(x, [(G_all[3], Wb[6], Wb[7]), (next_gen["G_all"][0], next_gen["Wb"][0], next_gen["Wb"][1])], dims, kl)
            sv["h4"] = hs[0]
            x = hs[0][2]
            nhead = (xl, hs[1])
        else:
            x, sv["h4"] = hypertem_core_fwd(x, G_all[3], Wb[6], Wb[7], dims)
    else:
        x, c1, sv["c1"] = cap_core_fwd(p, cps[0], x, dadj[0], dyn[0], Wn[0], Wn[1], dims, num_route, HS, HT)
        x, sv["h2"] = hypertem_core_fwd(x, G_all[1], Wb[2], Wb[3], dims)
        x, sv["h3"] = hypertem_core_fwd(x, G_all[2], Wb[4], Wb[5], dims)
        x, _, sv["c2"] = cap_core_fwd(p, cps[1], x, dadj[1], dyn[1], Wn[2], Wn[3], dims, num_route, HS, HT)
        x, sv["h4"] = hypertem_core_fwd(x, G_all[3], Wb[6], Wb[7], dims)
    sv["emb"] = gen["emb"]
    sv["gen"] = gen["gen"]
    sv["slot"] = gen.get("slot")
    if next_gen is not None:
        return x, c1, sv, nhead
    return x, c1, sv


def _grad_buffers(red, slot, N, T, HmT, ref, nsG):
    if slot is None:
        return torch.empty(4, nsG, N, T, T, device=ref.device), torch.empty(4, N, HmT, device=ref.device)
    k, n = slot
    if getattr(red, "_dG", None) is None or red._dG.shape[0] != 4 * n:
        red._dG = torch.empty(4 * n, nsG, N, T, T, device=ref.device)
        red._dA = torch.empty(4 * n, N, HmT, device=ref.device)
    return red._dG[4 * k:4 * k + 4], red._dA[4 * k:4 * k + 4]


def sthcn_bwd(p, g, pfx, tidx, sv, dout, dims, red, chain=False, premul_in=False, defer_h1=False, after_pending=None):
    B, T, N, C = dims
    time_eb, teb, tes = sv["emb"]
    A_all, hts, cps, d, Hm, ds, HS, HT = sv["gen"]
    ne, nes = p[pfx + "node_embeddings"], p[pfx + "node_embeddings_spg"]
    dne, dnes = g[pfx + "node_embeddings"], g[pfx + "node_embeddings_spg"]
    d_te, d_teb, d_tes = _zeros(time_eb, *time_eb.shape), _zeros(teb, *teb.shape), _zeros(tes, *tes.shape)
    nsG = graph_grad_splits(dims)
    dG_all, dA_all = _grad_buffers(red, sv.get("slot"), N, T, Hm * T, dout, nsG)
    J = red.jobs
    CC, BT = C * C, B * T

    def queue_ht(h, hp):
        dWbt, ns, (dbias, nsb) = hp
        J.bwd_pool(time_eb, dWbt, g[h + "weights_pool"].view(d, CC), nsplit=ns)
        J.bwd_pool(time_eb, dbias, g[h + "bias_pool"], nsplit=nsb)
        J.bwd_emb(dWbt, p[h + "weights_pool"].view(d, CC), d_te, nsplit=ns)
        J.bwd_emb(dbias, p[h + "bias_pool"], d_te, nsplit=nsb)

    def queue_cap(c, cp):
        dWn, ns, (dbn, nsb), ddyn, dlogit = cp
        dW2 = dWn if dWn.dim() == 2 else dWn.view(ns * N, CC)
        J.bwd_pool(nes, dW2, g[c + "weights_spa"].view(d, CC), nsplit=ns)
        J.bwd_pool(nes, dbn, g[c + "bias_spa"], nsplit=nsb)
        J.bwd_emb(dW2, p[c + "weights_spa"].view(d, CC), dnes, nsplit=ns)
        J.bwd_emb(dbn, p[c + "bias_spa"], dnes, nsplit=nsb)
        dd2 = ddyn.view(B, HT * T * HS)
        J.bwd_pool(tes, dd2, g[c + "t_adj"].view(ds, HT * T * HS))
        J.bwd_emb(dd2, p[c + "t_adj"].view(ds, HT * T * HS), d_tes)
        dl2 = dlogit.view(BT, HS * N)
        J.bwd_pool(teb, dl2, g[c + "adj"].view(ds, HS * N))
        J.bwd_emb(dl2, p[c + "adj"].view(ds, HS * N), d_teb)

    if isinstance(dout, PendingH1):
        up = dout
        dd, _, hp4 = ht_pair_bwd(up.saved, sv["h4"], up.dd, up.dG, dG_all[3], dims, dWb1=up.dWb)
        red.keep.append(up)
        if after_pending is not None:
            after_pending()
    else:
        dd, hp4 = hypertem_core_bwd(sv["h4"], dout, dG_all[3], dims, chain, True)
    queue_ht(hts[3], hp4)
    dd, cp2 = cap_core_bwd(p, g, cps[1], sv["c2"], dd, dims, HS, HT, red, chain)
    queue_cap(cps[1], cp2)
    pair = ht_pair_bwd(sv["h3"], sv["h2"], dd, dG_all[2], dG_all[1], dims) if chain and pair_bwd_on() else None
    if pair is not None:
        dd, hp3, hp2 = pair
    else:
        dd, hp3 = hypertem_core_bwd(sv["h3"], dd, dG_all[2], dims, chain, True)
        dd, hp2 = hypertem_core_bwd(sv["h2"], dd, dG_all[1], dims, chain, True)
    queue_ht(hts[2], hp3)
    queue_ht(hts[1], hp2)
    dd, cp1 = cap_core_bwd(p, g, cps[0], sv["c1"], dd, dims, HS, HT, red, chain)
    queue_cap(cps[0], cp1)
    if isinstance(sv["h1"], EncIn):
        assert chain
        e = sv["h1"]
        w, bi = p["encoder.dim_in_flow.weight"], p["encoder.dim_in_flow.bias"]
        if nsG == B:
            dWb, _, dinp = ops.encin_ht1_bwd(dd.view(B, T, N, C), e.source, e.mask, e.fill, w, bi, e.Wbt, e.ab, e.wv, dG=dG_all[0])
        else:
            dWb, dGb, dinp = ops.encin_ht1_bwd(dd.view(B, T, N, C), e.source, e.mask, e.fill, w, bi, e.Wbt, e.ab, e.wv)
            torch.sum(dGb, 0, out=dG_all[0][0])
        hp1 = (dWb[:, :C * C], 1, (dWb[:, C * C:], 1))
        wb = _wb_view(g["encoder.dim_in_flow.weight"], g["encoder.dim_in_flow.bias"])
        if wb is not None:
            red.jobs.bwd_pool(_ones(dd.device, dinp.shape[0]), dinp, wb)
        else:
            g["encoder.dim_in_flow.weight"].add_(dinp[:, :C].sum(0).view(C, 1))
            g["encoder.dim_in_flow.bias"].add_(dinp[:, C:].sum(0))
        red.keep.append((dinp, dWb))
        dd = None
    elif defer_h1:
        assert chain and premul_in
        ns = ops.wgrad_nsplit(MODE_TIME, B * T, N, C)
        dWb = torch.empty(ns * B * T, C * C + C, device=dd.device, dtype=torch.float32)
        hp1 = (dWb[:, :C * C], ns, (dWb[:, C * C:], ns))
        dd = PendingH1(sv["h1"], dd, dG_all[0], dWb)
    else:
        dd, hp1 = hypertem_core_bwd(sv["h1"], dd, dG_all[0], dims, chain, premul_in)
    queue_ht(hts[0], hp1)
    red.gram(A_all.view(4 * N, Hm, T), dG_all, dA_all.view(4 * N, Hm, T), N, nsG)
    for i, h in enumerate(hts):
        red.late.bwd_pool(ne, dA_all[i], g[h + "adj"].view(d, Hm * T))
        red.late.bwd_emb(dA_all[i], p[h + "adj"].view(d, Hm * T), dne)
    red.timefeat(p, g, pfx + "time_feature1.", tidx, d_te)
    red.timefeat(p, g, pfx + "time_feature1_.", tidx, d_teb)
    red.timefeat(p, g, pfx + "time_feature2.", tidx, d_tes, spg=True)
    red.keep.append((sv, hp1, hp2, hp3, hp4, cp1, cp2, dout))
    return dd


class EncIn:

    def __init__(self, source, mask, fill, Wbt, ab, wv):
        self.source, self.mask, self.fill, self.Wbt, self.ab, self.wv = source, mask, fill, Wbt, ab, wv


ENCIN = os.environ.get("GPTST_ENCIN", "1") == "1"


def encin_ok(dims, base):
    return ENCIN and base == 1 and dims[3] in (64, 128) and dims[1] == 12 and chain_ok(dims)


GUIDEIN = os.environ.get("GPTST_GUIDEIN", "1") == "1"
GUIDE_HEAD = os.environ.get("GPTST_GUIDE_HEAD", "1") == "1"


def guide_fwd(p, source, tidx, dims, base, gen=None, lowrank_in=False):
    B, T, N, C = dims
    if gen is None:
        gen = gen_all(p, tidx, dims, which=(), guide=True)["guide"]
    t4m, Wspa, bspa, Wtem, btem = gen
    m = "encoder.MLP_RL."
    if lowrank_in and GUIDEIN and GUIDE_HEAD and base == 1 and C == 64:
        r = ops.guide_head_fwd(source, p[m + "ln1.weight"], p[m + "ln1.bias"], Wspa, bspa, Wtem, btem, p[m + "ln3.weight"], p[m + "ln3.bias"])
        if r is not None:
            h1, h2, prob, label = r
            return prob, (t4m, ("lowrank", Wspa), (h1, h2, Wtem), h2, label)
    if lowrank_in and GUIDEIN and base == 1 and C in (64, 128):
        h1 = ops.guide_in_fwd(source, p[m + "ln1.weight"], p[m + "ln1.bias"], Wspa, bspa)
        s1 = ("lowrank", Wspa)
    else:
        h0 = ops.lin_in(source, base + 2, base, p[m + "ln1.weight"], p[m + "ln1.bias"], C)
        h1, s1 = condlin_fwd(h0, Wspa, bspa, MODE_NODE, dims)
    h2, s2 = condlin_fwd(h1, Wtem, btem, MODE_TIME, dims)
    prob, label = ops.rowdot(h2, p[m + "ln3.weight"], p[m + "ln3.bias"], softmax=True, want_label=True)
    return prob, (t4m, s1, s2, h2, label)


def _wb_view(gw, gb):
    n = gw.numel() + gb.numel()
    if gb.data_ptr() != gw.data_ptr() + 4 * gw.numel():
        return None
    return torch.as_strided(gw, (1, n), (n, 1))


def fused_tails_ok(p, C, base, HS):
    return (C in (64, 128) and base <= ops.TAIL_MAXJ and HS <= ops.TAIL_MAXJ
            and _wb_view(p["decoder.dim_flow_out.weight"], p["decoder.dim_flow_out.bias"]) is not None
            and _wb_view(p["encoder.MLP_RL.ln3.weight"], p["encoder.MLP_RL.ln3.bias"]) is not None)


def loss_tail(p, g, dec, source, mask, base, sigma, mu, thresh, sws, red, chain=False):
    wo = "decoder.dim_flow_out."
    out, dd, part = ops.tail_mae(dec, p[wo + "weight"], p[wo + "bias"], source, base + 2, mask, sigma, mu, thresh, sws, premul=chain)
    red.jobs.bwd_pool(_ones(dec.device, part.shape[0]), part, _wb_view(g[wo + "weight"], g[wo + "bias"]))
    red.keep.append((part, dd))
    return out, dd


def kl_head(p, g, sv_g, prob, c1, N, w, sws, red, chain=False, carried=None):
    m = "encoder.MLP_RL."
    dh2, part = carried if carried is not None else ops.tail_kl(sv_g[3], p[m + "ln3.weight"], prob, c1, N, w, sws, premul=chain)
    red.jobs.bwd_pool(_ones(prob.device, part.shape[0]), part, _wb_view(g[m + "ln3.weight"], g[m + "ln3.bias"]))
    red.keep.append((part, dh2))
    return dh2


def guide_bwd(p, g, source, tidx, saved, dlogit, dims, base, red, dh2=None, chain=False, carried=(None, None)):
    B, T, N, C = dims
    t4m, s1, s2, h2 = saved[:4]
    m = "encoder.MLP_RL."
    if dh2 is None:
        HS = dlogit.shape[1]
        dh2 = ops.lin_in(dlogit, HS, HS, p[m + "ln3.weight"], None, C, wlayout=1)
        ops.rowouter(dlogit, HS, HS, h2, g[m + "ln3.weight"], 1, asum=g[m + "ln3.bias"])
    d_t4m = _zeros(t4m, *t4m.shape)
    dh1 = condlin_bwd(s2, dh2, t4m, p[m + "weights_pool_tem"], p[m + "bias_pool_tem"], g[m + "weights_pool_tem"],
                      g[m + "bias_pool_tem"], d_t4m, MODE_TIME, dims, red, chain, True, carried=carried[0])
    if isinstance(s1[0], str):
        assert chain
        neb, wpool, bpool = p["encoder.neb4mask"], p[m + "weights_pool_spa"], p[m + "bias_pool_spa"]
        K = neb.shape[1]
        dWb, dinp = carried[1] if carried[1] is not None else ops.guide_in_bwd(dh1, source, p[m + "ln1.weight"], p[m + "ln1.bias"], s1[1])
        dW, db = dWb[:, :C * C], dWb[:, C * C:]
        red.jobs.bwd_pool(neb, dW, g[m + "weights_pool_spa"].view(K, C * C))
        red.jobs.bwd_pool(neb, db, g[m + "bias_pool_spa"])
        red.jobs.bwd_emb(dW, wpool.view(K, C * C), g["encoder.neb4mask"])
        red.jobs.bwd_emb(db, bpool, g["encoder.neb4mask"])
        wb = _wb_view(g[m + "ln1.weight"], g[m + "ln1.bias"])
        if wb is not None:
            red.jobs.bwd_pool(_ones(dh1.device, N), dinp, wb)
        else:
            g[m + "ln1.weight"].add_(dinp[:, :C].sum(0).view(C, 1))
            g[m + "ln1.bias"].add_(dinp[:, C:].sum(0))
        red.keep.append((dWb, dinp))
        dh0 = None
    else:
        dh0 = condlin_bwd(s1, dh1, p["encoder.neb4mask"], p[m + "weights_pool_spa"], p[m + "bias_pool_spa"],
                          g[m + "weights_pool_spa"], g[m + "bias_pool_spa"], g["encoder.neb4mask"], MODE_NODE, dims, red, chain, False)
        _in_proj_grads(source, base, dh0, g[m + "ln1.weight"], g[m + "ln1.bias"], None, 0.0, red)
    red.timefeat(p, g, GUIDE_TF, tidx, d_t4m)
    red.keep.append((saved, dlogit, dh2, dh1, dh0))


def kl_carry_ok(dims, HS, sv_g):
    B, T, N, C = dims
    return (CARRY_KL and C == 64 and T == 12 and HS <= ops.TAIL_MAXJ and chain_fwd_ok(dims) and chain_ok(dims)
            and sv_g is not None and isinstance(sv_g[1][0], str))


class KlCarry:

    def __init__(self, p, sv_g, prob, source, dims, w, sws):
        self.p, self.sv_g, self.prob, self.source, self.dims, self.w, self.sws = p, sv_g, prob, source, dims, w, sws
        self.c1 = None
        self.stage = 0
        self.out = {}

    def guest(self):
        if self.c1 is None or self.stage == 3:
            return None
        B, T, N, C = self.dims
        m = "encoder.MLP_RL."
        p, sv_g, dev = self.p, self.sv_g, self.prob.device
        HS = self.prob.shape[1]
        st = self.stage + 1
        f = dict(device=dev, dtype=torch.float32)
        if st == 1:
            h2, W3 = sv_g[3], p[m + "ln3.weight"]
            dh2 = torch.empty_like(h2)
            part = torch.empty(ops.tail_parts(B * T * N), HS * C + HS, **f)
            self.out[1] = (dh2, part)
            ts = [h2, W3, self.prob, self.c1, dh2, part, self.sws]
        elif st == 2:
            h1, _, Wtem = sv_g[2]
            dh2 = self.out[1][0]
            ns = _C.lib().value("gptst_apply_wgrad_nsplit", MODE_TIME, B * T, N)
            dh1, dW, db = torch.empty_like(h1), torch.empty(ns * B * T, C * C, **f), torch.empty(ns * B * T, C, **f)
            self.out[2] = (dh1, dW, db, ns)
            ts = [dh2, h1, Wtem, dh1, dW, db]
        else:
            dWb, dinp = torch.empty(N, C * C + C, **f), torch.empty(N, 2 * C, **f)
            self.out[3] = (dWb, dinp)
            ts = [self.out[2][0], self.source, p[m + "ln1.weight"], p[m + "ln1.bias"], sv_g[1][1], dWb, dinp]
        self.stage = st
        return (st, ts, 0, ops.kl_guest_blocks(st, B, T, N), HS, self.source.shape[-1], self.w)

    def carried(self, st):
        return self.out.get(st)


def _in_proj_grads(source, base, dY, gW, gb, mask, fill, red):
    wb = _wb_view(gW, gb)
    if base == 1 and wb is not None:
        C = dY.shape[1]
        part = ops.rowouter_part(source, base + 2, base, dY, mask=mask, fill=fill)
        red.jobs.bwd_pool(_ones(dY.device, part.shape[0]), part[:, :2 * C], wb)
        red.keep.append(part)
    else:
        ops.rowouter(source, base + 2, base, dY, gW, 0, csum=gb, mask=mask, fill=fill)


def model_fwd(p, source, mask, dims, base, num_route, scaler_zeros, gen=None, tidx=None, dec_gen=None, lowrank_in=False, kl=None):
    B, T, N, C = dims
    if tidx is None:
        tidx = source[:, :, 0, base:base + 2].contiguous()
    head = None
    if lowrank_in and gen is not None and encin_ok(dims, base):
        w, bi = p["encoder.dim_in_flow.weight"], p["encoder.dim_in_flow.bias"]
        G1, Wb = gen["G_all"][0], gen["Wb"]
        o1, ab, wv = ops.encin_ht1_fwd(source, base, mask, 0.0 if mask is None else scaler_zeros, w, bi, G1, Wb[0], Wb[1])
# ... 41 lines not shown
```

### gpt-st_amd/ops.py

```python
import torch

from . import _C

MODE_TIME, MODE_NODE, MODE_SHARED = 0, 1, 2
PRO_NONE, PRO_DPRE = 0, 1
EPI_PLAIN, EPI_RES_LRELU, EPI_ADD_DPRE, EPI_LRELU, EPI_ADD_PREMUL, EPI_PREMUL = 0, 1, 2, 3, 4, 5

_p = _C.ptr


TIMER = None
LAST_CALL = {}


CALL_LOCK = None


def _call(name, *args, tag="", nbytes=0):
    if CALL_LOCK is not None:
        with CALL_LOCK:
            _C.lib().call(name, *args, _C.stream())
        return
    if TIMER is None:
        _C.lib().call(name, *args, _C.stream())
        return
    e0, e1 = torch.cuda.Event(enable_timing=True), torch.cuda.Event(enable_timing=True)
    e0.record()
    _C.lib().call(name, *args, _C.stream())
    e1.record()
    TIMER.append((name, tag, e0, e1, nbytes))
    LAST_CALL[(name, tag)] = args


def _nb(*ts):
    return sum(t.numel() * t.element_size() for t in ts if t is not None)


def _chk(*ts):
    for t in ts:
        if t is not None:
            assert t.is_cuda and t.dtype == torch.float32 and t.is_contiguous(), (t.device, t.dtype, t.is_contiguous())


def poolgen(emb, pool, pool2=None):
    _chk(emb, pool, pool2)
    R, K = emb.shape
    cols = pool.numel() // K
    out = torch.empty((R,) + tuple(pool.shape[1:]), device=emb.device, dtype=torch.float32)
    out2, cols2 = None, 0
    if pool2 is not None:
        cols2 = pool2.numel() // K
        out2 = torch.empty((R,) + tuple(pool2.shape[1:]), device=emb.device, dtype=torch.float32)
    _call("gptst_poolgen_fwd", _p(emb), _p(pool), _p(out), cols, _p(pool2), _p(out2), cols2, R, K, nbytes=_nb(emb, pool, out, pool2, out2))
    return (out, out2) if pool2 is not None else out


def poolgen_bwd_pool(emb, dW, dpool, dW2=None, dpool2=None, nsplit=1):
    _chk(emb, dW, dpool, dW2, dpool2)
    R, K = emb.shape
    cols = dpool.numel() // K
    cols2 = dpool2.numel() // K if dpool2 is not None else 0
    _call("gptst_poolgen_bwd_pool", _p(emb), _p(dW), _p(dpool), cols, _p(dW2), _p(dpool2), cols2, R, nsplit, K,
          nbytes=_nb(emb, dW, dpool, dW2, dpool2))


def poolgen_bwd_emb(dW, pool, demb, dW2=None, pool2=None, nsplit=1):
    _chk(dW, pool, demb, dW2, pool2)
    R, K = demb.shape
    cols = pool.numel() // K
    cols2 = pool2.numel() // K if pool2 is not None else 0
    _call("gptst_poolgen_bwd_emb", _p(dW), _p(pool), cols, _p(dW2), _p(pool2), cols2, _p(demb), R, nsplit, K,
          nbytes=_nb(dW, pool, dW2, pool2, demb))


def _ptrs(ts):
    import ctypes
    return (ctypes.c_void_p * len(ts))(*[t.data_ptr() for t in ts])


def _ints(vs):
    import ctypes
    return (ctypes.c_int * len(vs))(*[int(v) for v in vs])


def poolgen_multi(emb, pools, outs=None):
    _chk(emb, *pools)
    R, K = emb.shape
    if outs is None:
        outs = [torch.empty((R,) + tuple(pl.shape[1:]), device=emb.device, dtype=torch.float32) for pl in pools]
    cols = [pl.numel() // K for pl in pools]
    _call("gptst_poolgen_fwd_multi", _p(emb), len(pools), _ptrs(pools), _ptrs(outs), _ints(cols), R, K, nbytes=_nb(emb, *pools, *outs))
    return outs


def poolgen_bwd_pool_multi(emb, dWs, dpools, nsplits=None):
    _chk(emb, *dWs, *dpools)
    R, K = emb.shape
    cols = [dp.numel() // K for dp in dpools]
    ns = nsplits if nsplits is not None else [1] * len(dWs)
    _call("gptst_poolgen_bwd_pool_multi", _p(emb), len(dWs), _ptrs(dWs), _ptrs(dpools), _ints(cols), _ints(ns), R, K,
          nbytes=_nb(emb, *dWs, *dpools))


def poolgen_bwd_emb_multi(dWs, pools, demb, nsplits=None):
    _chk(demb, *dWs, *pools)
    R, K = demb.shape
    cols = [pl.numel() // K for pl in pools]
    ns = nsplits if nsplits is not None else [1] * len(dWs)
    _call("gptst_poolgen_bwd_emb_multi", len(dWs), _ptrs(dWs), _ptrs(pools), _ints(cols), _ints(ns), _p(demb), R, K,
          nbytes=_nb(demb, *dWs, *pools))


class PoolJobs:
    FWD, BWD_POOL, BWD_EMB, GRAM = 0, 1, 2, 3

    def __init__(self):
        self.jobs = []
        self.post = []

    def fwd(self, emb, pool, out=None):
        _chk(emb, pool, out)
        R, K = emb.shape
        if out is None:
            out = torch.empty((R,) + tuple(pool.shape[1:]), device=emb.device, dtype=torch.float32)
        self.jobs.append((self.FWD, emb, None, pool, out, R, K, pool.numel() // K, 1, 0))
        return out

    def gram(self, emb, pool, out, A=None):
        _chk(emb, pool, out, A)
        R, K = emb.shape
        cols = pool.numel() // K
        assert cols % 12 == 0 and out.numel() == R * 144 and out.is_contiguous()
        if _C.lib().value("gptst_pool_jobs_gram_rows", K, cols) <= 0:
            assert A is not None and A.numel() == R * cols, "gram job does not fit and no forward output was given"
            self.post.append((A, out, R, cols // 12))
            return out
        self.jobs.append((self.GRAM, emb, None, pool, out, R, K, cols, 1, 0))
        return out

    @staticmethod
    def _ldx(dW, cols):
        assert dW.is_cuda and dW.dtype == torch.float32 and dW.dim() == 2 and dW.shape[1] == cols and dW.stride(1) == 1, (dW.shape, dW.stride(), cols)
        return dW.stride(0)

    def bwd_pool(self, emb, dW, dpool, nsplit=1):
        _chk(emb, dpool)
        R, K = emb.shape
        cols = dpool.numel() // K
        self.jobs.append((self.BWD_POOL, emb, dW, None, dpool, R, K, cols, nsplit, self._ldx(dW, cols)))

    def bwd_emb(self, dW, pool, demb, nsplit=1):
        _chk(pool, demb)
        R, K = demb.shape
        cols = pool.numel() // K
        self.jobs.append((self.BWD_EMB, None, dW, pool, demb, R, K, cols, nsplit, self._ldx(dW, cols)))

    def launch(self):
        js, self.jobs = self.jobs, []
        post, self.post = self.post, []
        if js:
            col = lambda i: [j[i] for j in js]
            _call("gptst_pool_jobs", len(js), _ints(col(0)), _ptrs0(col(1)), _ptrs0(col(2)), _ptrs0(col(3)), _ptrs0(col(4)), _ints(col(5)),
                  _ints(col(6)), _ints(col(7)), _ints(col(8)), _ints(col(9)), nbytes=_nb(*[t for j in js for t in j[1:5]]))
        for A, G, rows, Hm in post:
            _call("gptst_gram_fwd", _p(A), _p(G), rows, Hm)


def _ptrs0(ts):
    import ctypes
    return (ctypes.c_void_p * len(ts))(*[(t.data_ptr() if t is not None else None) for t in ts])


def apply(A, W, mode, BT, N, bias=None, resid=None, A2=None, transw=False, pro=PRO_NONE, epi=EPI_PLAIN, colsum=None,
          out=None, resid2=None):
    _chk(A, W, bias, resid, A2, resid2)
    C = A.shape[-1]
    if out is None:
        out = torch.empty_like(A)
    cs, ns = None, 0
    if colsum is not None:
        G = BT if mode == MODE_TIME else (N if mode == MODE_NODE else 1)
        ns = _C.lib().value("gptst_apply_nsplit", mode, BT, N, C)
        cs = torch.empty(ns * G, C, device=A.device, dtype=torch.float32)
    _call("gptst_apply", _p(A), _p(A2), _p(W), int(W.dim() == 3), int(transw), _p(bias), _p(resid), _p(resid2), _p(out), _p(cs),
          mode, pro, epi, BT, N, C, tag="mode%d pro%d epi%d" % (mode, pro, epi), nbytes=_nb(A, A2, W, bias, resid, resid2, out))
    if colsum is True:
        return out, cs, ns
    if colsum is not None:
        colsum.add_(cs.view(ns, -1, C).sum(0).view_as(colsum))
    return out


def apply_wgrad(dOut, Y, S, W, mode, BT, N, premul=False):
    _chk(dOut, Y, S, W)
    C = dOut.shape[-1]
    G = BT if mode == MODE_TIME else N
    ns = _C.lib().value("gptst_apply_wgrad_nsplit", mode, BT, N)
    dS = torch.empty_like(dOut)
    dW = torch.empty(ns * G, C * C, device=dOut.device, dtype=torch.float32)
    db = torch.empty(ns * G, C, device=dOut.device, dtype=torch.float32)
    _call("gptst_apply_wgrad", _p(dOut), _p(Y), _p(S), _p(W), _p(dS), _p(dW), _p(db), int(premul), mode, BT, N, C, tag="mode%d" % mode,
          nbytes=_nb(dOut, Y, S, W, dS, dW))
    return dS, dW, db, ns


def linear_bwd(dY, X, Wp, dOut, out, premul=False):
    _chk(dY, X, Wp, dOut, out)
    rows, C = dY.shape
    ns = _C.lib().value("gptst_linear_bwd_nsplit", rows)
    dX = torch.empty_like(dY)
    dWp = torch.empty(ns, C * C, device=dY.device, dtype=torch.float32)
    dbp = torch.empty(ns, C, device=dY.device, dtype=torch.float32)
    _call("gptst_linear_bwd", _p(dY), _p(X), _p(Wp), _p(dOut), _p(out), _p(dX), _p(dWp), _p(dbp), int(premul), rows, C,
          nbytes=_nb(dY, X, dOut, out, dX, dWp))
    return dX, dWp, dbp, ns


def wgrad_nsplit(mode, BT, N, C=64):
    return _C.lib().value("gptst_wgrad_nsplit", mode, BT, N, C)


def wgrad(A, D, mode, BT, N, D2=None, pro=PRO_NONE, colsum_a=False, colsum_d=False):
    _chk(A, D, D2)
    C = A.shape[-1]
    ns = wgrad_nsplit(mode, BT, N, C)
    G = BT if mode == MODE_TIME else (N if mode == MODE_NODE else 1)
    if colsum_a or colsum_d:
        dW = torch.empty(ns * G, C * C + C, device=A.device, dtype=torch.float32)
        _call("gptst_wgrad_colsum", _p(A), _p(D), _p(D2), _p(dW), mode, pro, 1 if colsum_a else 2, BT, N, C,
              tag="mode%d pro%d cs" % (mode, pro), nbytes=_nb(A, D, D2, dW))
    else:
        dW = torch.empty(ns * G, C, C, device=A.device, dtype=torch.float32)
        _call("gptst_wgrad", _p(A), _p(D), _p(D2), _p(dW), mode, pro, BT, N, C, tag="mode%d pro%d" % (mode, pro), nbytes=_nb(A, D, D2, dW))
    return dW, ns


def gram_fwd(A):
    N, Hm, T = A.shape
    G = torch.empty(N, T, T, device=A.device, dtype=torch.float32)
    _call("gptst_gram_fwd", _p(A), _p(G), N, Hm)
    return G


def gram_bwd(A, dG, out=None, layers=1, nsplit=1):
    LN, Hm, T = A.shape
# ... 344 lines not shown
        return _call("gptst_capbig_rec_fwd", _p(c), _p(v), _p(rec), BT, HS, N, C)
    _lds_or_stream(lambda: _call("gptst_cap_rec_fwd", _p(c), _p(v), _p(rec), BT, N, C, HS, nbytes=_nb(c, v, rec)), stream)
    return rec


def cap_rec_bwd(drec, c, v, reduce_nodes=None):
    _chk(drec, c, v)
    BT, HS, N = c.shape
    C = v.shape[-1]
    dc1 = torch.empty_like(c)
    dv = torch.empty_like(v)

    def stream():
        if capflow_ok(HS, C):
            npart = _C.lib().value("gptst_capflow_nparts", N)
            part = torch.empty(BT, npart, HS, C, device=c.device, dtype=torch.float32)
            _call("gptst_capflow_route", _p(drec), _p(v), None, _p(dc1), None, _p(c), None, _p(part), BT, HS, N, C)
            _capflow_post(part, npart, HS, None, dv, 2, BT, HS, C, reduce_nodes)
            return
        _call("gptst_capbig_rec_bwd_dc", _p(drec), _p(v), _p(dc1), BT, HS, N, C)
        _capbig_type1(c, drec, dv, BT, HS, N, C, reduce_nodes)
    if reduce_nodes is not None or (HS > 16 and capflow_ok(HS, C)):
        stream()
    else:
        _lds_or_stream(lambda: _call("gptst_cap_rec_bwd", _p(drec), _p(c), _p(v), _p(dc1), _p(dv), BT, N, C, HS, nbytes=_nb(drec, c, v, dc1, dv)),
                       stream)
    return dc1, dv


def cap_route_bwd(X, Wp, bp, c, dc1, dS, Y=None):
    _chk(X, Wp, bp, c, dc1, dS)
    B, T, N, C = X.shape
    HS = c.shape[1]
    dY = torch.empty(B * T * N, C, device=X.device, dtype=torch.float32)
    dlogit = torch.empty_like(c)

    def stream():
        Yv = Y if Y is not None else _capbig_linear(X, Wp, bp)
        name = "gptst_capflow_route_bwd" if capflow_ok(HS, C) else "gptst_capbig_route_bwd_rows"
        _call(name, _p(Yv), _p(c), _p(dc1), _p(dS), _p(dY), _p(dlogit), B * T, HS, N, C)
    if Y is not None:
        stream()
    else:
        _lds_or_stream(lambda: _call("gptst_cap_route_bwd", _p(X), _p(Wp), _p(bp), _p(c), _p(dc1), _p(dS), _p(dY), _p(dlogit), B * T, N, C, HS,
                                     nbytes=_nb(X, Wp, bp, c, dc1, dS, dY, dlogit)), stream)
    return dY, dlogit


def cap_cross_route_bwd(X, Wp, bp, c, dc1, dv, s, Rt, Ht, dyn, tmpl, B, T, HS, HT, flags=None):
    _chk(X, Wp, bp, c, dc1, dv, s, Rt, Ht, dyn, tmpl)
    N, C = X.shape[2], X.shape[3]
    if C != 64 or FORCE_CAP_BIG:
        return None
    dY = torch.empty(B * T * N, C, device=X.device, dtype=torch.float32)
    dlogit = torch.empty_like(c)
    ddyn = torch.empty_like(dyn)
    try:
        dS_ws = torch.empty(B * T, HS, C, device=X.device, dtype=torch.float32) if flags is not None else None
        _call("gptst_cap_cross_route_bwd", _p(X), _p(Wp), _p(bp), _p(c), _p(dc1), _p(dv), _p(s), _p(Rt), _p(Ht), _p(dyn), _p(tmpl), _p(dY),
              _p(dlogit), _p(ddyn), _p(dS_ws), _p(flags), B, T, N, C, HS, HT, nbytes=_nb(X, Wp, bp, c, dc1, dv, s, Rt, dY, dlogit))
    except _C.GptstError as e:
        if e.code != _C.ESHAPE:
            raise
        return None
    return dY, dlogit, ddyn


def cap_cross_route_lin_bwd(X, Wp, bp, c, dc1, dv, s, Rt, Ht, dyn, tmpl, dPre, out, premul, B, T, HS, HT, flags=None, jobs=None, nsplit=None):
    _chk(X, Wp, bp, c, dc1, dv, s, Rt, Ht, dyn, tmpl, dPre, out)
    N, C = X.shape[2], X.shape[3]
    if C != 64 or FORCE_CAP_BIG:
        return None
    dev = X.device
    if nsplit is None:
        nsplit = _C.lib().value("gptst_cap_split_units", B * T, N, C, HS)
    rows = B * T + nsplit
    dX = torch.empty(B * T * N, C, device=dev, dtype=torch.float32)
    dWp = torch.empty(rows, C * C, device=dev, dtype=torch.float32)
    dbp = torch.empty(rows, C, device=dev, dtype=torch.float32)
    dlogit = torch.empty_like(c)
    ddyn = torch.empty_like(dyn)
    try:
        dS_ws = torch.empty(B * T, HS, C, device=dev, dtype=torch.float32) if flags is not None else None
        js = jobs.jobs if jobs is not None and not jobs.post and all(j[0] in (PoolJobs.BWD_POOL, PoolJobs.BWD_EMB) for j in jobs.jobs) else []
        col = lambda i: [j[i] for j in js]
        _call("gptst_cap_cross_route_lin_bwd_split", _p(X), _p(Wp), _p(bp), _p(c), _p(dc1), _p(dv), _p(s), _p(Rt), _p(Ht), _p(dyn), _p(tmpl),
              _p(dPre), _p(out), int(bool(premul)), _p(dX), _p(dWp), _p(dbp), _p(dlogit), _p(ddyn), _p(dS_ws), _p(flags), B, T, N, C, HS, HT, nsplit,
              len(js), _ints(col(0)), _ptrs0(col(1)), _ptrs0(col(2)), _ptrs0(col(3)), _ptrs0(col(4)), _ints(col(5)), _ints(col(6)), _ints(col(7)),
              _ints(col(8)), _ints(col(9)), nbytes=_nb(X, Wp, bp, c, dc1, dv, s, Rt, dPre, out, dX, dWp, dlogit))
        if js:
            jobs.jobs = []
    except _C.GptstError as e:
        if e.code != _C.ESHAPE:
            raise
        return None
    return dX, dWp, dbp, dlogit, ddyn


_MASK_WS = {}


def _mask_ws(dev):
    if dev not in _MASK_WS:
        _MASK_WS[dev] = torch.zeros(_C.lib().value("gptst_mask_ws_bytes") // 4, dtype=torch.int32, device=dev)
    return _MASK_WS[dev]


def mask_ws_floats():
    return _C.lib().value("gptst_mask_ws_bytes") // 4


def _fused_jobs(jobs, u24):
    if jobs is None or not (jobs.jobs or jobs.post):
        return None
    if not u24 or jobs.post or any(j[0] not in (PoolJobs.FWD, PoolJobs.GRAM) for j in jobs.jobs):
        jobs.launch()
        return None
    odd = [j for j in jobs.jobs if j[0] == PoolJobs.FWD and j[7] % 4]
    if odd:
        rest = [j for j in jobs.jobs if not (j[0] == PoolJobs.FWD and j[7] % 4)]
        jobs.jobs = odd
        jobs.launch()
        jobs.jobs = rest
        if not rest:
            return None
    js, jobs.jobs = jobs.jobs, []
    col = lambda i: [j[i] for j in js]
    return js, (len(js), _ints(col(0)), _ptrs0(col(1)), _ptrs0(col(3)), _ptrs0(col(4)), _ints(col(5)), _ints(col(6)), _ints(col(7)))


def mask_random(noise, k, ws=None, u24=False, jobs=None):
    _chk(noise)
    mask = torch.empty_like(noise)
    fj = _fused_jobs(jobs, u24)
    if fj is not None:
        _call("gptst_mask_u24_fwd_jobs", 0, None, None, None, None, _p(noise), None, 0, noise.numel(), 0, 1, int(k), None, None, _p(mask),
              _p(ws if ws is not None else _mask_ws(noise.device)), int(ws is not None), *fj[1])
        return mask
    _call("gptst_mask_random_u24" if u24 else "gptst_mask_random", _p(noise), noise.numel(), int(k), _p(mask),
          _p(ws if ws is not None else _mask_ws(noise.device)), int(ws is not None))
    return mask


MASK_SMALL = 1 << 13


def labels_and_counts(prob, label):
    return label, None


def mask_labels(prob):
    _chk(prob)
    rows, HS = prob.shape
    label = torch.empty(rows, device=prob.device, dtype=torch.int32)
    counts = torch.empty(HS, device=prob.device, dtype=torch.int32)
    _call("gptst_mask_labels", _p(prob), rows, HS, _p(label), _p(counts))
    return label, counts


def mask_adaptive(label, counts, list_c, nums, noise_a, noise_r, ada_all, base, ws=None, u24=False, jobs=None):
    M, HS = label.numel(), list_c.numel()
    m_ada = torch.empty(M, device=label.device, dtype=torch.float32)
    m_rnd = torch.empty_like(m_ada)
    mask = torch.empty(M * base, device=label.device, dtype=torch.float32)
    fj = _fused_jobs(jobs, u24)
    if fj is not None:
        _call("gptst_mask_u24_fwd_jobs", 1, _p(label), _p(counts), _p(list_c), _p(nums), _p(noise_a), _p(noise_r), int(ada_all), M, HS, base, 0,
              _p(m_ada), _p(m_rnd), _p(mask), _p(ws if ws is not None else _mask_ws(label.device)), int(ws is not None), *fj[1])
        return m_ada, m_rnd, mask
    _call("gptst_mask_adaptive_u24" if u24 else "gptst_mask_adaptive", _p(label), _p(counts), _p(list_c), _p(nums), _p(noise_a), _p(noise_r),
          int(ada_all), M, HS, base, _p(m_ada), _p(m_rnd), _p(mask), _p(ws if ws is not None else _mask_ws(label.device)), int(ws is not None))
    return m_ada, m_rnd, mask


def lin_in(a, lda, J, W, b, C, mask=None, fill=0.0, wlayout=0, rows=None):
    rows = rows if rows is not None else a.numel() // lda
    Y = torch.empty(rows, C, device=a.device, dtype=torch.float32)
    _call("gptst_lin_in", _p(a), lda, _p(mask), float(fill), _p(W), wlayout, _p(b), _p(Y), rows, J, C, nbytes=_nb(a, mask, W, b, Y))
    return Y


def rowdot(X, W, b, softmax=False, want_label=False):
    rows, C = X.shape
    J = W.shape[0]
    Z = torch.empty(rows, J, device=X.device, dtype=torch.float32)
    label = torch.empty(rows, device=X.device, dtype=torch.int32) if want_label else None
    _call("gptst_rowdot", _p(X), _p(W), _p(b), _p(Z), rows, J, C, int(softmax), _p(label), nbytes=_nb(X, W, b, Z))
    return (Z, label) if want_label else Z


def rowouter(a, lda, J, X, out, olayout, csum=None, asum=None, mask=None, fill=0.0):
    rows, C = X.shape
    ws = torch.empty(_C.lib().value("gptst_rowouter_ws_floats", J, C), device=X.device, dtype=torch.float32)
    _call("gptst_rowouter", _p(a), lda, _p(mask), float(fill), _p(X), _p(out), olayout, _p(csum), _p(asum), _p(ws), rows, J, C,
          nbytes=_nb(a, mask, X, out))


def rowouter_part(a, lda, J, X, mask=None, fill=0.0, want_asum=False):
    rows, C = X.shape
    nparts = _C.lib().value("gptst_rowouter_nparts", rows)
    part = torch.empty(nparts, J * C + C + J, device=X.device, dtype=torch.float32)
    _call("gptst_rowouter_part", _p(a), lda, _p(mask), float(fill), _p(X), _p(part), int(want_asum), rows, J, C, nbytes=_nb(X))
    return part


def timefeat_fwd(params, tidx, rows, K):
    E = params[1].numel()
    out = torch.empty(rows, E, device=tidx.device, dtype=torch.float32)
    _call("gptst_timefeat_fwd", *[_p(t) for t in params], _p(tidx), _p(out), rows, K, E)
    return out


def timefeat_bwd(params, grads, tidx, dout, rows, K):
    E = params[1].numel()
    _call("gptst_timefeat_bwd", *[_p(t) for t in params], *[_p(t) for t in grads], _p(tidx), _p(dout), rows, K, E)


def timefeat_jobs_fwd(jobs, tidx):
    outs = [torch.empty(rows, params[1].numel(), device=tidx.device, dtype=torch.float32) for params, rows, K in jobs]
    _call("gptst_timefeat_jobs", len(jobs), 0, _ptrs([t for params, _, _ in jobs for t in params]), None, _p(tidx), _ptrs(outs),
          _ints([r for _, r, _ in jobs]), _ints([k for _, _, k in jobs]), _ints([params[1].numel() for params, _, _ in jobs]))
    return outs


def timefeat_jobs_bwd(jobs, tidx):
    if not jobs:
        return
    _call("gptst_timefeat_jobs", len(jobs), 1, _ptrs([t for j in jobs for t in j[0]]), _ptrs([t for j in jobs for t in j[1]]), _p(tidx),
          _ptrs([j[2] for j in jobs]), _ints([j[3] for j in jobs]), _ints([j[4] for j in jobs]), _ints([j[0][1].numel() for j in jobs]))


def mae_fwd(out, src, lda, mask, sigma, mu, thresh, rows, J, stats):
    _call("gptst_mae_fwd", _p(out), _p(src), lda, _p(mask), float(sigma), float(mu), float(thresh), rows, J, _p(stats))


def mae_bwd(out, src, lda, mask, sigma, mu, thresh, rows, J, stats, normalize=True):
    dOut = torch.empty_like(out)
    _call("gptst_mae_bwd", _p(out), _p(src), lda, _p(mask), float(sigma), float(mu), float(thresh), rows, J, _p(stats), int(normalize),
          _p(dOut))
    return dOut


def kl(prob, c, N, w, stats, want_grad=True):
    rows, HS = prob.shape
    dlogit = torch.empty_like(prob) if want_grad else None
    _call("gptst_kl", _p(prob), _p(c), rows, N, HS, float(w), _p(dlogit), _p(stats))
    return dlogit


TAIL_MAXJ = 16


def set_deterministic(on):
    _C.lib().call("gptst_set_deterministic", int(bool(on)))



def tail_parts(rows):
    return _C.lib().value("gptst_tail_parts", rows)


def tail_sws(rows, device):
    return torch.zeros(_C.lib().value("gptst_tail_parts", rows), 4, device=device, dtype=torch.float32)


def tail_mae(dec, W, b, src, lda, mask, sigma, mu, thresh, sws, premul=False):
    rows, C = dec.shape
    J = W.shape[0]
    nparts = _C.lib().value("gptst_tail_parts", rows)
    out = torch.empty(rows, J, device=dec.device, dtype=torch.float32)
    d_dec = torch.empty_like(dec)
    part = torch.empty(nparts, J * C + J, device=dec.device, dtype=torch.float32)
    _call("gptst_tail_mae", _p(dec), _p(W), _p(b), _p(src), lda, _p(mask), float(sigma), float(mu), float(thresh), _p(out), _p(d_dec),
          _p(part), _p(sws), int(premul), rows, J, C, nbytes=_nb(dec, d_dec))
    return out, d_dec, part


def tail_kl(h2, W3, prob, c, N, w, sws, premul=False):
    rows, C = h2.shape
    HS = W3.shape[0]
    nparts = _C.lib().value("gptst_tail_parts", rows)
    d_h2 = torch.empty_like(h2)
    part = torch.empty(nparts, HS * C + HS, device=h2.device, dtype=torch.float32)
    _call("gptst_tail_kl", _p(h2), _p(W3), _p(prob), _p(c), float(w), _p(d_h2), _p(part), _p(sws), int(premul), rows, N, HS, C, nbytes=_nb(h2, d_h2))
    return d_h2, part


def stats_fold(sws, stats):
    _call("gptst_stats_fold", _p(sws), sws.shape[0], _p(stats))


_ADAM_WS = {}


def step_begin(z0, z1, src, base, noise=None, rng=None):
    B, T, N, lda = src.shape
    tidx = torch.empty(B, T, 2, device=src.device, dtype=torch.float32)
    _call("gptst_step_begin", _p(z0), z0.numel(), _p(z1), z1.numel() if z1 is not None else 0, _p(src), _p(tidx), B * T, N, lda, base,
          _p(noise), noise.numel() if noise is not None else 0, _p(rng))
    return tidx


def clip_adam(p, g, m, v, nA, nB, hyper, stats, ws=None, stats_out=None, sws=None):
    if ws is None:
        if p.device not in _ADAM_WS:
            _ADAM_WS[p.device] = torch.empty(_C.lib().value("gptst_clip_adam_ws_floats"), device=p.device, dtype=torch.float32)
        ws = _ADAM_WS[p.device]
    _call("gptst_clip_adam", _p(p), _p(g), _p(m), _p(v), int(nA), int(nB), _p(hyper), _p(stats), _p(ws), _p(stats_out), _p(sws),
          sws.shape[0] if sws is not None else 0)


def metrics_new(T, N, device):
    return torch.zeros(T, 5, device=device, dtype=torch.float64), torch.zeros(T, N, 6, device=device, dtype=torch.float64)


def metrics_accum(out, src, lda, vis, sigma, mu, mae_thresh, mape_thresh, B, T, N, D, sums_t, sums_tn):
    _call("gptst_metrics_accum", _p(out), _p(src), lda, _p(vis), float(sigma), float(mu), int(mae_thresh is not None),
          float(mae_thresh if mae_thresh is not None else 0.0), float(mape_thresh), B, T, N, D, _p(sums_t), _p(sums_tn))


def metrics_report(sums_t, sums_tn):
    st, sn = sums_t.cpu(), sums_tn.cpu()

    def rows_of(a, m):
        mae, rmse, mape = a[..., 1] / a[..., 0], torch.sqrt(a[..., 2] / a[..., 0]), a[..., 4] / a[..., 3]
        K, sp, sy, spp, syy, spy = (m[..., k] for k in range(6))
        pm, ym = sp / K, sy / K
        cov = spy / K - pm * ym
        pvar, yvar = (spp - K * pm * pm) / (K - 1), (syy - K * ym * ym) / (K - 1)
        c = cov / torch.sqrt(pvar.clamp_min(0) * yvar.clamp_min(0))
        ok = yvar > 1e-9 * (syy / K).clamp_min(1e-30)
        corr = torch.stack([c[i][ok[i]].mean() for i in range(c.shape[0])]) if c.dim() == 2 else c[ok].mean()
        return torch.stack([mae, rmse, mape, corr], -1)

    per_t = rows_of(st, sn)
    avg = rows_of(st.sum(0), sn.sum(0))
    return torch.cat([per_t, avg[None]], 0)
# ... 1 lines not shown
```

### include/gptst_hip.h

```cpp
#ifndef GPTST_HIP_H
#define GPTST_HIP_H
#include <stdint.h>

#ifdef __cplusplus
extern "C" {
#endif
#if defined(__GNUC__)
#pragma GCC visibility push(default)
#endif

#define GPTST_ABI_VERSION 16
int gptst_abi_version(void);
int gptst_set_deterministic(int on);
int gptst_handoff_timeouts(int* out);
int gptst_handoff_reset(void);
int gptst_mask_cooperative(int on);
int gptst_mask_cooperative_state(void);
int gptst_set_handoff_guard(int on);

int gptst_poolgen_fwd(const float* emb, const float* pool, float* out, int cols, const float* pool2, float* out2,
                      int cols2, int R, int K, void* stream);
int gptst_poolgen_bwd_pool(const float* emb, const float* dW, float* dpool, int cols, const float* dW2, float* dpool2,
                           int cols2, int R, int nsplit, int K, void* stream);
int gptst_poolgen_bwd_emb(const float* dW, const float* pool, int cols, const float* dW2, const float* pool2, int cols2,
                          float* demb, int R, int nsplit, int K, void* stream);

int gptst_poolgen_fwd_multi(const float* emb, int nprob, const void* pools, const void* outs, const int* cols, int R, int K,
                            void* stream);
int gptst_poolgen_bwd_pool_multi(const float* emb, int nprob, const void* dWs, const void* dpools, const int* cols, const int* nsplit,
                                 int R, int K, void* stream);
int gptst_poolgen_bwd_emb_multi(int nprob, const void* dWs, const void* pools, const int* cols, const int* nsplit, float* demb, int R,
                                int K, void* stream);

int gptst_pool_jobs(int njobs, const int* kind, const void* const* emb, const void* const* x, const void* const* pool,
                    const void* const* out, const int* R, const int* K, const int* cols, const int* nsplit, const int* ldx, void* stream);
int gptst_pool_jobs_gram_rows(int K, int cols);

int gptst_apply_nsplit(int mode, int BT, int N, int C);
int gptst_apply(const float* A, const float* A2, const float* W, int w_per_group, int transw, const float* bias,
                const float* resid, const float* resid2, float* out, float* colsum, int mode, int pro, int epi, int BT,
                int N, int C, void* stream);
int gptst_wgrad_nsplit(int mode, int BT, int N, int C);
int gptst_wgrad(const float* A, const float* D, const float* D2, float* dW, int mode, int pro, int BT, int N, int C,
                void* stream);
int gptst_wgrad_colsum(const float* A, const float* D, const float* D2, float* dW, int mode, int pro, int which, int BT, int N, int C,
                       void* stream);

int gptst_apply_wgrad_nsplit(int mode, int BT, int N);
int gptst_apply_wgrad(const float* dOut, const float* Y, const float* S, const float* W, float* dS, float* dW, float* colsum, int premul,
                      int mode, int BT, int N, int C, void* stream);

int gptst_linear_bwd_nsplit(int rows);
int gptst_linear_bwd(const float* dY, const float* X, const float* Wp, const float* dOut, const float* out, float* dX, float* dWp, float* dbp,
                     int premul, int rows, int C, void* stream);

int gptst_gram_fwd(const float* A, float* G, int N, int Hm, void* stream);
int gptst_gram_bwd(const float* A, const float* dG, float* dA, int L, int N, int Hm, int nsplit, void* stream);
int gptst_tmix(const float* X, const float* G, const float* dOut, const float* Y, float* out, int B, int T, int N, int C,
               void* stream);
int gptst_tmix_dgraph(const float* dR, const float* X, float* dG, int B, int T, int N, int C, void* stream);
int gptst_tmix_bwd(const float* dR, const float* X, const float* G, const float* dOut, const float* Y, float* dX, float* dG, int B, int T,
                   int N, int C, void* stream);
int gptst_tmix_bwd_chain(const float* dR, const float* X, const float* G, const float* dPre, int premul, float* dX, float* dG, int B, int T,
                         int N, int C, void* stream);

int gptst_hypertem_fwd(const float* X, const float* G, const float* Wbt, const float* bbt, float* R_out, float* out, int B, int T,
                       int N, int C, void* stream);
int gptst_hypertem_chain_fwd(const float* X, int nstage, const void* Gs, const void* Wbts, const void* bbts, const void* Rs, const void* outs,
                             int B, int T, int N, int C, void* stream);
int gptst_hypertem_chain_fwd_kl(const float* X, int nstage, const void* Gs, const void* Wbts, const void* bbts, const void* Rs, const void* outs,
                                int B, int T, int N, int C, int stage, const void* ops, int v0, int v1, int HS, int lda, float w, void* stream);
int gptst_kl_guest_blocks(int stage, int B, int T, int N);

int gptst_encin_ht1_fwd(const float* src, int lda, const float* mask, float fill, const float* w, const float* bi, const float* G,
                        const float* Wbt, const float* bbt, float* out, float* ab, float* wv, int B, int T, int N, int C, void* stream);
int gptst_encin_ht1_bwd(const float* dPre, const float* src, int lda, const float* mask, float fill, const float* w, const float* bi,
                        const float* Wbt, const float* ab, const float* wv, float* dWb, float* dG, float* dinp, int B, int T, int N, int C,
                        void* stream);

int gptst_guide_in_fwd(const float* src, int lda, const float* w1, const float* b1, const float* Wn, const float* bn, float* h1, int BT, int N,
                       int C, void* stream);
int gptst_guide_in_bwd(const float* dPre, const float* src, int lda, const float* w1, const float* b1, const float* Wn, float* dWb, float* dinp,
                       int BT, int N, int C, void* stream);
int gptst_guide_uc_floats(int N, int C);
int gptst_guide_head_fwd(const float* src, int lda, const float* w1, const float* b1, const float* Wn, const float* bn, const float* Wbt,
                         const float* bbt, const float* W3, const float* b3, float* uc, float* h1, float* h2, float* prob, int* label,
                         int BT, int N, int C, int J, void* stream);

int gptst_hypertem_ntiles(int N);
int gptst_hypertem_bwd(const float* dOut, const float* Y, const float* X, const float* G, const float* Wbt, float* dX, float* dbias,
                       float* dG, int premul, int B, int T, int N, int C, void* stream);
int gptst_hypertem_bwd_wgrad(const float* dOut, const float* Y, const float* X, const float* G, const float* Wbt, const float* R, float* dX,
                             float* dG, float* dWb, int premul, int B, int T, int N, int C, void* stream);
int gptst_hypertem_bwd_pair(const float* dOut1, const float* X1, const float* G1, const float* Wbt1, const float* R1, const float* X0,
                            const float* G0, const float* Wbt0, const float* R0, float* dXmid, float* dX0, float* dG1, float* dG0,
                            float* dWb1, float* dWb0, void* cnt, int B, int T, int N, int C, void* stream);

int gptst_cap_route_fwd(const float* X, const float* Wp, const float* bp, const float* dadj, float* c_out, float* s_out, int BT, int N,
                        int C, int HS, int R, void* stream);
int gptst_cap_cross_fwd(const float* s, const float* dyn, const float* tmpl, float* v, float* Ht, float* Rt, int B, int T, int C,
                        int HS, int HT, void* stream);
int gptst_cap_cross_ws_floats(int B, int T, int C, int HS, int HT);
int gptst_cap_cross_bwd(const float* dv, const float* s, const float* Rt, const float* Ht, const float* dyn, const float* tmpl,
                        float* dS, float* ddyn, float* ws, int B, int T, int C, int HS, int HT, void* stream);
int gptst_cap_rec_fwd(const float* c, const float* v, float* rec, int BT, int N, int C, int HS, void* stream);
int gptst_cap_cross_rec_fwd(const float* s, const float* dyn, const float* tmpl, const float* c, float* v, float* Ht, float* Rt, float* rec,
                            int B, int T, int N, int C, int HS, int HT, void* stream);
int gptst_cap_rec_bwd(const float* drec, const float* c, const float* v, float* dc1, float* dv, int BT, int N, int C, int HS,
                      void* stream);
int gptst_cap_route_bwd(const float* X, const float* Wp, const float* bp, const float* c, const float* dc1, const float* dS,
                        float* dY, float* dlogit, int BT, int N, int C, int HS, void* stream);
int gptst_cap_cross_route_bwd(const float* X, const float* Wp, const float* bp, const float* c, const float* dc1, const float* dv,
                              const float* s, const float* Rt, const float* Ht, const float* dyn, const float* tmpl, float* dY,
                              float* dlogit, float* ddyn, float* dS_ws, void* flags, int B, int T, int N, int C, int HS, int HT, void* stream);
int gptst_cap_cross_route_lin_bwd(const float* X, const float* Wp, const float* bp, const float* c, const float* dc1, const float* dv,
                                  const float* s, const float* Rt, const float* Ht, const float* dyn, const float* tmpl,
                                  const float* dPre, const float* out, int premul, float* dX, float* dWp, float* dbp, float* dlogit,
                                  float* ddyn, float* dS_ws, void* flags, int B, int T, int N, int C, int HS, int HT, void* stream);
int gptst_cap_route_roles_ok(int B, int T, int N, int C, int HS, int HT);
int gptst_cap_cross_route_lin_bwd_jobs(const float* X, const float* Wp, const float* bp, const float* c, const float* dc1, const float* dv,
                                       const float* s, const float* Rt, const float* Ht, const float* dyn, const float* tmpl,
                                       const float* dPre, const float* out, int premul, float* dX, float* dWp, float* dbp, float* dlogit,
                                       float* ddyn, float* dS_ws, void* flags, int B, int T, int N, int C, int HS, int HT,
                                       int njobs, const int* jkind, const void* const* jemb, const void* const* jx, const void* const* jpool,
                                       const void* const* jout, const int* jR, const int* jK, const int* jcols, const int* jnsplit, const int* jldx,
                                       void* stream);
int gptst_cap_split_units(int BT, int N, int C, int HS);
int gptst_cap_cross_route_lin_bwd_split(const float* X, const float* Wp, const float* bp, const float* c, const float* dc1, const float* dv,
                                        const float* s, const float* Rt, const float* Ht, const float* dyn, const float* tmpl,
                                        const float* dPre, const float* out, int premul, float* dX, float* dWp, float* dbp, float* dlogit,
                                        float* ddyn, float* dS_ws, void* flags, int B, int T, int N, int C, int HS, int HT, int nsplit,
                                        int njobs, const int* jkind, const void* const* jemb, const void* const* jx, const void* const* jpool,
                                        const void* const* jout, const int* jR, const int* jK, const int* jcols, const int* jnsplit, const int* jldx,
                                        void* stream);

int gptst_cap_fits_lds(int N, int C, int HS);
int gptst_capbig_squash_rows(float* Y, long rows, int C, void* stream);
int gptst_capbig_softmax(const float* bl, const float* l0, float* cs, int BT, int HS, int N, int use_bl, int use_l0, void* stream);
int gptst_capbig_type1(const float* cs, const float* P, float* S, int BT, int HS, int N, int C, void* stream);
int gptst_capbig_post(const float* S, const float* V0, float* out, long rows, int C, int post, void* stream);
int gptst_capbig_type2(const float* V, const float* P, float* bl, int BT, int HS, int N, int C, void* stream);
int gptst_capbig_rec_fwd(const float* c, const float* v, float* rec, int BT, int HS, int N, int C, void* stream);
int gptst_capbig_rec_bwd_dc(const float* drec, const float* v, float* dc1, int BT, int HS, int N, int C, void* stream);
int gptst_capbig_route_bwd_rows(const float* Y, const float* c, const float* dc1, const float* dS, float* dY, float* dlogit, int BT,
                                int HS, int N, int C, void* stream);

int gptst_capflow_supported(int HS, int C);
int gptst_capflow_nparts(int N);
int gptst_capflow_squash(const float* Y, const float* dadj, float* P, float* part, int BT, int HS, int N, int C, void* stream);
int gptst_capflow_route(const float* rows, const float* V, const float* bl_in, float* bl_out, const float* l0, const float* c_in,
                        float* c_out, float* part, int BT, int HS, int N, int C, void* stream);
int gptst_capflow_post(const float* part, int nparts, int prow, float* V0, float* Vout, int mode, int BT, int HS, int C, void* stream);
int gptst_capflow_rec_fwd(const float* c, const float* v, float* rec, int BT, int HS, int N, int C, void* stream);
int gptst_capflow_route_bwd(const float* Y, const float* c, const float* dc1, const float* dS, float* dY, float* dlogit, int BT,
                            int HS, int N, int C, void* stream);

int gptst_metrics_accum(const float* out, const float* src, int lda, const float* vis, float sigma, float mu, int has_mae_thresh,
                        float mae_thresh, float mape_thresh, int B, int T, int N, int D, double* sums_t, double* sums_tn, void* stream);

int gptst_mask_ws_bytes(void);
int gptst_mask_random(const float* noise, int M, int k, float* mask, void* ws, int ws_zeroed, void* stream);
int gptst_mask_labels(const float* prob, int rows, int HS, int* label, int* counts, void* stream);
int gptst_mask_adaptive(const int* label, const int* counts, const int* list_c, const int* nums, const float* noise_a,
                        const float* noise_r, int ada_all, int M, int HS, int base, float* m_ada, float* m_rnd, float* mask,
                        void* ws, int ws_zeroed, void* stream);

int gptst_mask_random_u24(const float* noise, int M, int k, float* mask, void* ws, int ws_zeroed, void* stream);
int gptst_mask_adaptive_u24(const int* label, const int* counts, const int* list_c, const int* nums, const float* noise_a, const float* noise_r,
                            int ada_all, int M, int HS, int base, float* m_ada, float* m_rnd, float* mask, void* ws, int ws_zeroed, void* stream);
int gptst_mask_u24_fwd_jobs(int adaptive, const int* label, const int* counts, const int* list_c, const int* nums, const float* noise_a,
                            const float* noise_r, int ada_all, int M, int HS, int base, int k, float* m_ada, float* m_rnd, float* mask, void* ws,
                            int ws_zeroed, int njobs, const int* kind, const void* const* emb, const void* const* pool, const void* const* out,
                            const int* R, const int* K, const int* cols, void* stream);

int gptst_lin_in(const float* a, int lda, const float* mask, float fill, const float* W, int wlayout, const float* b, float* Y,
                 int rows, int J, int C, void* stream);
int gptst_rowdot(const float* X, const float* W, const float* b, float* Z, int rows, int J, int C, int do_softmax, int* label,
                 void* stream);
int gptst_fusion_gate_fwd(const float* F, const float* src, int lda, int base, const float* Ws, const float* bs, const float* Wh,
                          const float* bh, const float* Wo, const float* bo, const float* Wt, const float* bt, float* out, float* z,
                          int rows, int C, void* stream);
int gptst_fusion_gate_bwd(const float* dOut, const float* F, const float* z, const float* src, int lda, int base, const float* Wo,
                          const float* Wt, const float* bt, float* dpre, float* dxd, float* Hm, float* xt, int rows, int C, void* stream);
int gptst_rowouter_ws_floats(int J, int C);
int gptst_rowouter_nparts(int rows);
int gptst_rowouter_part(const float* a, int lda, const float* mask, float fill, const float* X, float* part, int want_asum, int rows,
                        int J, int C, void* stream);
int gptst_rowouter(const float* a, int lda, const float* mask, float fill, const float* X, float* out, int olayout, float* csum,
                   float* asum, float* ws, int rows, int J, int C, void* stream);

int gptst_timefeat_fwd(const float* wd, const float* bd, const float* ww, const float* bw, const float* w1, const float* b1,
                       const float* w2, const float* b2, const float* w3, const float* b3, const float* tidx, float* out, int rows,
                       int K, int E, void* stream);
int gptst_timefeat_bwd(const float* wd, const float* bd, const float* ww, const float* bw, const float* w1, const float* b1,
                       const float* w2, const float* b2, const float* w3, const float* b3, float* gwd, float* gbd, float* gww,
                       float* gbw, float* gw1, float* gb1, float* gw2, float* gb2, float* gw3, float* gb3, const float* tidx,
                       const float* dout, int rows, int K, int E, void* stream);

int gptst_tail_parts(int rows);
int gptst_tail_mae(const float* dec, const float* W, const float* b, const float* src, int lda, const float* mask, float sigma, float mu,
                   float thresh, float* out, float* d_dec, float* part, float* sws, int premul, int rows, int J, int C, void* stream);
int gptst_tail_kl(const float* h2, const float* W3, const float* prob, const float* c, float w, float* d_h2, float* part, float* sws,
                  int premul, int rows, int N, int HS, int C, void* stream);
int gptst_stats_fold(const float* sws, int rows, float* stats, void* stream);

int gptst_timefeat_jobs(int njobs, int bwd, const void* const* params, const void* const* grads, const float* tidx,
                        const void* const* io, const int* rows, const int* K, const int* E, void* stream);

int gptst_step_begin(float* z0, long n0, float* z1, long n1, const float* src, float* tidx, int BT, int N, int lda, int base,
                     float* noise, long n_noise, const int* rng, void* stream);

int gptst_mae_fwd(const float* out, const float* src, int lda, const float* mask, float sigma, float mu, float thresh, int rows,
                  int J, float* stats, void* stream);
int gptst_mae_bwd(const float* out, const float* src, int lda, const float* mask, float sigma, float mu, float thresh, int rows,
                  int J, const float* stats, int normalize, float* dOut, void* stream);
int gptst_kl(const float* prob, const float* c, int rows, int N, int HS, float w, float* dlogit, float* stats, void* stream);
// ... 49 lines not shown
```

Measured before the change: 926.6 steps/s.

## Fuse pool and embedding backward reductions into a single BWD_BOTH job

Adds a PJ_BWD_BOTH job kind that computes both the pool-weight gradient and the embedding gradient from the same dW slice in one block. Previously these were separate bwd_pool and bwd_emb jobs. The new kind is wired into the standalone pool-jobs kernel and into the job tail of the fused route-backward kernel, and the Python call sites now use a paired helper. The aim is to read dW once and cut the number of job blocks. In exchange the kernel needs extra LDS scratch sized by R, shape limits that fall back to the two-job path, and a widened ABI.

```diff
diff --git a/gpt-st_amd/csrc/cap_mfma.hip b/gpt-st_amd/csrc/cap_mfma.hip
--- a/gpt-st_amd/csrc/cap_mfma.hip
+++ b/gpt-st_amd/csrc/cap_mfma.hip
@@ -605,7 +605,7 @@
 }
 
 template <bool JOBS> struct RouteJobs { };
-template <> struct RouteJobs<true> { PJobs t; int npool, npb, neb, first; };
+template <> struct RouteJobs<true> { PJobs t; int npool, npb, neb, first, nboth, nbb, bothR; };
 
 template <int C, int ROLES, bool LIN = false, bool JOBS = false>
 __global__ __launch_bounds__(CM_NT, 4) void cap_route_bwd2_kernel(const float* __restrict__ X, const float* __restrict__ Wp,
@@ -629,11 +629,22 @@
                 } else {
                     __syncthreads();
                 }
+            } else if (w < wp + ((jr.nbb + 1) >> 1)) {
+                const int vb = __builtin_amdgcn_readfirstlane(2 * (w - wp) + half);
+                if (vb < jr.nbb) {
+                    int p = jr.npool;
+                    for (int q = jr.npool + 1; q < jr.npool + jr.nboth; ++q) if (vb >= jr.t.j[q].blk0) p = q;
+                    const PJob& a = jr.t.j[p];
+                    pj_bwd_both<4, true>(a, vb - a.blk0, jsmem + half * (jr.bothR * PG_MAXK), tid_);
+                } else {
+#pragma unroll
+                    for (int q = 0; q < PJ_BOTH_NBAR; ++q) __syncthreads();
+                }
             } else {
-                const int vb = __builtin_amdgcn_readfirstlane(2 * (w - wp) + half);
+                const int vb = __builtin_amdgcn_readfirstlane(2 * (w - wp - ((jr.nbb + 1) >> 1)) + half);
                 if (vb < jr.neb) {
-                    int p = jr.npool;
-                    for (int q = jr.npool + 1; q < jr.t.n; ++q) if (vb >= jr.t.j[q].blk0) p = q;
+                    int p = jr.npool + jr.nboth;
+                    for (int q = jr.npool + jr.nboth + 1; q < jr.t.n; ++q) if (vb >= jr.t.j[q].blk0) p = q;
                     const PJob& a = jr.t.j[p];
                     const int rel = vb - a.blk0;
                     if (((a.cols | a.ldx) & 3) == 0) pj_bwd_emb<4>(a, rel % a.nbx, rel / a.nbx, tid_); else pj_bwd_emb<1>(a, rel % a.nbx, rel / a.nbx, tid_);
@@ -1045,12 +1056,13 @@
     }
     const int nhr = (cx.nB > 0 && g_cap_split_roles) ? (2 * nsplit < cx.nB ? 2 * nsplit : cx.nB) : 0;
     const int NU = BT + nsplit - nhr;
-    if (jobs != nullptr && !(cx.nB > 0 && lin.dX != nullptr && smem >= 2 * (4 * PG_MAXK * 65) * sizeof(float))) return GPTST_ESHAPE;
+    if (jobs != nullptr && !(cx.nB > 0 && lin.dX != nullptr && smem >= 2 * (4 * PG_MAXK * 65) * sizeof(float) &&
+                             smem >= 2 * (size_t)jobs->bothR * PG_MAXK * sizeof(float))) return GPTST_ESHAPE;
     if (jobs != nullptr) {
         static size_t curJ = 0;
         if (smem > curJ) { (void)hipFuncSetAttribute((const void*)cap_route_bwd2_kernel<C, 1, true, true>, hipFuncAttributeMaxDynamicSharedMemorySize, (int)smem); curJ = smem; }
         jobs->first = NU + cx.nB;
-        const int njw = ((jobs->npb + 1) >> 1) + ((jobs->neb + 1) >> 1);
+        const int njw = ((jobs->npb + 1) >> 1) + ((jobs->nbb + 1) >> 1) + ((jobs->neb + 1) >> 1);
         hipLaunchKernelGGL((cap_route_bwd2_kernel<C, 1, true, true>), dim3(NU + cx.nB + njw), dim3(CM_NT), smem, st, X, Wp, bp, c, dc1, dS, dY, dlogit, N, HS, (int)r2, cx, lin, *jobs, nfull, nhr);
         GPTST_CHECK_LAUNCH();
         return GPTST_OK;
@@ -1122,10 +1134,10 @@
                                     int HS, void* stream);
 
 GPTST_INTERNAL int gptst_pj_reduce_table(PJobs* t, int njobs, const int* kind, const void* const* emb, const void* const* x, const void* const* pool,
-                                         const void* const* out, const int* R, const int* K, const int* cols, const int* nsplit, const int* ldx,
-                                         int* npool, int* npb, int* neb);
-extern "C" int gptst_pool_jobs(int njobs, const int* kind, const void* const* emb, const void* const* x, const void* const* pool,
-                               const void* const* out, const int* R, const int* K, const int* cols, const int* nsplit, const int* ldx, void* stream);
+                                         const void* const* out, const void* const* out2, const int* R, const int* K, const int* cols, const int* nsplit,
+                                         const int* ldx, int* npool, int* npb, int* neb, int* nboth, int* nbb, int* bothR);
+extern "C" int gptst_pool_jobs2(int njobs, const int* kind, const void* const* emb, const void* const* x, const void* const* pool, const void* const* out,
+                                const void* const* out2, const int* R, const int* K, const int* cols, const int* nsplit, const int* ldx, void* stream);
 extern "C" int gptst_cap_route_roles_ok(int B, int T, int N, int C, int HS, int HT) {
     if (C != 64 || HS > 64 || HS <= 0 || B <= 0 || N <= 0 || T != 12 || g_cap_bwd_noroles) return 0;
     const int NR = cm_rows(N), NP = cm_np(N), HSP = cm_hsp(HS), BT = B * T, nB = B * CX_SPLIT;
@@ -1163,8 +1175,8 @@
                                        const float* dPre, const float* out, int premul, float* dX, float* dWp, float* dbp, float* dlogit,
                                        float* ddyn, float* dS_ws, void* flags, int B, int T, int N, int C, int HS, int HT, int nsplit,
                                        int njobs, const int* jkind, const void* const* jemb, const void* const* jx, const void* const* jpool,
-                                       const void* const* jout, const int* jR, const int* jK, const int* jcols, const int* jnsplit, const int* jldx,
-                                       void* stream) {
+                                       const void* const* jout, const void* const* jout2, const int* jR, const int* jK, const int* jcols, const int* jnsplit,
+                                       const int* jldx, void* stream) {
     if (!X || !Wp || !bp || !c || !dc1 || !dv || !s || !Rt || !Ht || !dyn || !tmpl || !dPre || !dX || !dWp || !dbp || !dlogit || !ddyn || B <= 0 ||
         T <= 0 || (out && premul) || nsplit < 0 || nsplit > B * T) return GPTST_EARG;
     if (njobs < 0 || (njobs && (!jkind || !jemb || !jx || !jpool || !jout || !jR || !jK || !jcols || !jnsplit))) return GPTST_EARG;
@@ -1175,14 +1187,15 @@
     const LinArgs lin{dPre, out, dX, dWp, dbp, premul};
     if (njobs > 0 && roles) {
         RouteJobs<true> jr;
-        if (gptst_pj_reduce_table(&jr.t, njobs, jkind, jemb, jx, jpool, jout, jR, jK, jcols, jnsplit, jldx, &jr.npool, &jr.npb, &jr.neb) == GPTST_OK) {
+        if (gptst_pj_reduce_table(&jr.t, njobs, jkind, jemb, jx, jpool, jout, jout2, jR, jK, jcols, jnsplit, jldx, &jr.npool, &jr.npb, &jr.neb, &jr.nboth, &jr.nbb,
+                                  &jr.bothR) == GPTST_OK) {
             const int rc = launch_route_bwd2<64>(X, Wp, bp, c, dc1, nullptr, nullptr, dlogit, B * T, N, HS, (hipStream_t)stream, cx, lin, &jr, nsplit);
             if (rc != GPTST_ESHAPE) return rc;
         }
     }
     const int rc = launch_route_bwd2<64>(X, Wp, bp, c, dc1, nullptr, nullptr, dlogit, B * T, N, HS, (hipStream_t)stream, cx, lin, nullptr, nsplit);
     if (rc || njobs == 0) return rc;
-    return gptst_pool_jobs(njobs, jkind, jemb, jx, jpool, jout, jR, jK, jcols, jnsplit, jldx, stream);
+    return gptst_pool_jobs2(njobs, jkind, jemb, jx, jpool, jout, jout2, jR, jK, jcols, jnsplit, jldx, stream);
 }
 
 extern "C" int gptst_cap_cross_route_lin_bwd_jobs(const float* X, const float* Wp, const float* bp, const float* c, const float* dc1, const float* dv,
@@ -1193,7 +1206,7 @@
                                                   const void* const* jout, const int* jR, const int* jK, const int* jcols, const int* jnsplit, const int* jldx,
                                                   void* stream) {
     return cap_cross_route_lin_bwd_any(X, Wp, bp, c, dc1, dv, s, Rt, Ht, dyn, tmpl, dPre, out, premul, dX, dWp, dbp, dlogit, ddyn, dS_ws, flags, B, T, N, C, HS,
-                                       HT, 0, njobs, jkind, jemb, jx, jpool, jout, jR, jK, jcols, jnsplit, jldx, stream);
+                                       HT, 0, njobs, jkind, jemb, jx, jpool, jout, nullptr, jR, jK, jcols, jnsplit, jldx, stream);
 }
 
 extern "C" int gptst_cap_cross_route_lin_bwd_split(const float* X, const float* Wp, const float* bp, const float* c, const float* dc1, const float* dv,
@@ -1201,11 +1214,12 @@
                                                    const float* dPre, const float* out, int premul, float* dX, float* dWp, float* dbp, float* dlogit,
                                                    float* ddyn, float* dS_ws, void* flags, int B, int T, int N, int C, int HS, int HT, int nsplit,
                                                    int njobs, const int* jkind, const void* const* jemb, const void* const* jx, const void* const* jpool,
-                                                   const void* const* jout, const int* jR, const int* jK, const int* jcols, const int* jnsplit, const int* jldx,
-                                                   void* stream) {
+                                                   const void* const* jout, const void* const* jout2, const int* jR, const int* jK, const int* jcols,
+                                                   const int* jnsplit, const int* jldx, void* stream) {
     return cap_cross_route_lin_bwd_any(X, Wp, bp, c, dc1, dv, s, Rt, Ht, dyn, tmpl, dPre, out, premul, dX, dWp, dbp, dlogit, ddyn, dS_ws, flags, B, T, N, C, HS,
-                                       HT, nsplit, njobs, jkind, jemb, jx, jpool, jout, jR, jK, jcols, jnsplit, jldx, stream);
-}
+                                       HT, nsplit, njobs, jkind, jemb, jx, jpool, jout, jout2, jR, jK, jcols, jnsplit, jldx, stream);
+}
+
 
 extern "C" int gptst_cap_rec_bwd(const float* drec, const float* c, const float* v, float* dc1, float* dv, int BT, int N, int C, int HS,
                                  void* stream) {
diff --git a/gpt-st_amd/csrc/poolgen.hip b/gpt-st_amd/csrc/poolgen.hip
--- a/gpt-st_amd/csrc/poolgen.hip
+++ b/gpt-st_amd/csrc/poolgen.hip
@@ -79,7 +79,8 @@
 }
 
 __global__ __launch_bounds__(256, PJ_OCC) void pool_jobs_kernel(PJobs t, int fwd_rows, int fwd_mfma) {
-    __shared__ __attribute__((aligned(16))) float fold[4][PG_MAXK][65];
+    __shared__ __attribute__((aligned(16))) float scr[PJ_BOTH_SCR];
+    float (*fold)[PG_MAXK][65] = reinterpret_cast<float (*)[PG_MAXK][65]>(scr);
     int p = 0;
     for (int q = 1; q < t.n; ++q) if ((int)blockIdx.x >= t.j[q].blk0) p = q;
     const PJob& a = t.j[p];
@@ -91,6 +92,7 @@
         else pj_fwd<1>(a, bx, by, fwd_rows, &fold[0][0][0]);
     }
     else if (a.kind == PJ_GRAM) pj_gram(a, rel, &fold[0][0][0], 256);
+    else if (a.kind == PJ_BWD_BOTH) pj_bwd_both<4, false>(a, bx, scr, threadIdx.x);
     else if (a.kind == PJ_BWD_POOL) { if (v4) pj_bwd_pool<4>(a, bx, fold, threadIdx.x); else pj_bwd_pool<1>(a, bx, fold, threadIdx.x); }
     else { if (v4) pj_bwd_emb<4>(a, bx, by, threadIdx.x); else pj_bwd_emb<1>(a, bx, by, threadIdx.x); }
 }
@@ -104,6 +106,7 @@
     if (j.kind == PJ_FWD) { j.nbx = ((j.cols + V - 1) / V + 255) / 256; return j.nbx * ((j.R + g_pg_rows - 1) / g_pg_rows); }
     if (j.kind == PJ_GRAM) { const int nb = pj_gram_rows(j.K, j.cols); j.nbx = (j.R + nb - 1) / nb; return j.nbx; }
     if (j.kind == PJ_BWD_POOL) { j.nbx = (j.cols + 16 * V - 1) / (16 * V); return j.nbx; }
+    if (j.kind == PJ_BWD_BOTH) { j.nbx = (j.cols + 255) / 256; return j.nbx; }
     j.nbx = (j.R + 15) / 16;
     return j.nbx * (((j.cols + 255) / 256 + 3) / 4);
 }
@@ -115,13 +118,15 @@
     for (int p = 0; p < t.n; ++p) {
         PJob& j = t.j[p];
         if (j.R <= 0 || j.K <= 0 || j.K > PG_MAXK || j.cols <= 0 || j.nsplit <= 0 || !j.out) return GPTST_EARG;
-        if ((j.kind == PJ_FWD || j.kind == PJ_BWD_POOL || j.kind == PJ_GRAM) && !j.emb) return GPTST_EARG;
+        if ((j.kind == PJ_FWD || j.kind == PJ_BWD_POOL || j.kind == PJ_GRAM || j.kind == PJ_BWD_BOTH) && !j.emb) return GPTST_EARG;
         if (j.kind == PJ_GRAM && (!j.pool || j.cols % 12 || pj_gram_rows(j.K, j.cols) <= 0)) return GPTST_EARG;
-        if ((j.kind == PJ_BWD_POOL || j.kind == PJ_BWD_EMB) && !j.x) return GPTST_EARG;
-        if ((j.kind == PJ_FWD || j.kind == PJ_BWD_EMB) && !j.pool) return GPTST_EARG;
+        if ((j.kind == PJ_BWD_POOL || j.kind == PJ_BWD_EMB || j.kind == PJ_BWD_BOTH) && !j.x) return GPTST_EARG;
+        if ((j.kind == PJ_FWD || j.kind == PJ_BWD_EMB || j.kind == PJ_BWD_BOTH) && !j.pool) return GPTST_EARG;
         j.blk0 = nb;
         if (j.ldx <= 0) j.ldx = j.cols;
         if (j.ldx < j.cols) return GPTST_EARG;
+        if (j.kind == PJ_BWD_BOTH && !j.out2) return GPTST_EARG;
+        if (j.kind == PJ_BWD_BOTH && !pj_both_ok(j.R, j.K, j.cols, j.nsplit, j.ldx)) return GPTST_ESHAPE;
         nb += pj_blocks(j);
     }
     if (nb == 0) return GPTST_OK;
@@ -140,7 +145,7 @@
             const int kd = kind ? kind[p] : (int)PJ_FWD;
             if (kd != PJ_FWD && kd != PJ_GRAM) return GPTST_ESHAPE;
             if ((kd == PJ_GRAM) != (pass == 1)) continue;
-            PJob j{(const float*)emb[p], nullptr, (const float*)pool[p], (float*)out[p], R[p], K[p], cols[p], 1, 0, kd, 0, cols[p]};
+            PJob j = pj_make(emb[p], nullptr, pool[p], out[p], nullptr, R[p], K[p], cols[p], 1, kd, cols[p]);
             if (!j.emb || !j.pool || !j.out || j.R <= 0 || j.K <= 0 || j.K > PG_MAXK || j.cols <= 0) return GPTST_EARG;
             if (kd == PJ_FWD) {
                 if (j.cols & 3) return GPTST_ESHAPE;
@@ -156,21 +161,23 @@
 }
 
 GPTST_INTERNAL int gptst_pj_reduce_table(PJobs* t, int njobs, const int* kind, const void* const* emb, const void* const* x, const void* const* pool,
-                                         const void* const* out, const int* R, const int* K, const int* cols, const int* nsplit, const int* ldx,
-                                         int* npool, int* npb, int* neb) {
+                                         const void* const* out, const void* const* out2, const int* R, const int* K, const int* cols, const int* nsplit,
+                                         const int* ldx, int* npool, int* npb, int* neb, int* nboth, int* nbb, int* bothR) {
     if (njobs > PJ_MAX || g_deterministic) return GPTST_ESHAPE;
     t->n = 0;
-    *npool = *npb = *neb = 0;
-    for (int pass = 0; pass < 2; ++pass) {
+    *npool = *npb = *neb = *nboth = *nbb = *bothR = 0;
+    for (int pass = 0; pass < 3; ++pass) {
         for (int p = 0; p < njobs; ++p) {
-            if (kind[p] != PJ_BWD_POOL && kind[p] != PJ_BWD_EMB) return GPTST_ESHAPE;
-            if ((kind[p] == PJ_BWD_EMB) != (pass == 1)) continue;
-            PJob j{(const float*)emb[p], (const float*)x[p], (const float*)pool[p], (float*)out[p], R[p], K[p], cols[p], nsplit[p], 0, kind[p], 0, ldx ? ldx[p] : 0};
+            if (kind[p] != PJ_BWD_POOL && kind[p] != PJ_BWD_EMB && kind[p] != PJ_BWD_BOTH) return GPTST_ESHAPE;
+            if ((kind[p] == PJ_BWD_POOL ? 0 : kind[p] == PJ_BWD_BOTH ? 1 : 2) != pass) continue;
+            PJob j = pj_make(emb[p], x[p], pool[p], out[p], out2 ? out2[p] : nullptr, R[p], K[p], cols[p], nsplit[p], kind[p], ldx ? ldx[p] : 0);
             if (j.R <= 0 || j.K <= 0 || j.K > PG_MAXK || j.cols <= 0 || j.nsplit <= 0 || !j.out || !j.x) return GPTST_EARG;
-            if (kind[p] == PJ_BWD_POOL ? !j.emb : !j.pool) return GPTST_EARG;
+            if ((kind[p] != PJ_BWD_EMB && !j.emb) || (kind[p] != PJ_BWD_POOL && !j.pool) || (kind[p] == PJ_BWD_BOTH && !j.out2)) return GPTST_EARG;
             if (j.ldx <= 0) j.ldx = j.cols;
             if (j.ldx < j.cols) return GPTST_EARG;
+            if (kind[p] == PJ_BWD_BOTH && !pj_both_ok(j.R, j.K, j.cols, j.nsplit, j.ldx)) return GPTST_ESHAPE;
             if (pass == 0) { j.blk0 = *npb; *npb += pj_blocks(j); ++*npool; }
+            else if (pass == 1) { j.blk0 = *nbb; *nbb += pj_blocks(j); ++*nboth; if (j.R > *bothR) *bothR = j.R; }
             else { j.blk0 = *neb; *neb += pj_blocks(j); }
             t->j[t->n++] = j;
         }
@@ -178,22 +185,23 @@
     return GPTST_OK;
 }
 
-extern "C" int gptst_pool_jobs(int njobs, const int* kind, const void* const* emb, const void* const* x, const void* const* pool,
-                               const void* const* out, const int* R, const int* K, const int* cols, const int* nsplit, const int* ldx,
-                               void* stream) {
+extern "C" int gptst_pool_jobs2(int njobs, const int* kind, const void* const* emb, const void* const* x, const void* const* pool,
+                                const void* const* out, const void* const* out2, const int* R, const int* K, const int* cols, const int* nsplit,
+                                const int* ldx, void* stream) {
     if (njobs < 0 || (njobs && (!kind || !emb || !x || !pool || !out || !R || !K || !cols || !nsplit))) return GPTST_EARG;
-    for (int p = 0; p < njobs; ++p) if (kind[p] < PJ_FWD || kind[p] > PJ_GRAM) return GPTST_EARG;
-    auto job = [&](int p) {
-        return PJob{(const float*)emb[p], (const float*)x[p], (const float*)pool[p], (float*)out[p], R[p], K[p], cols[p], nsplit[p],
-                    0, kind[p], 0, ldx ? ldx[p] : 0};
-    };
+    for (int p = 0; p < njobs; ++p) {
+        if (kind[p] < PJ_FWD || kind[p] > PJ_BWD_BOTH) return GPTST_EARG;
+        if (kind[p] == PJ_BWD_BOTH && (!out2 || !out2[p] || g_deterministic)) return GPTST_EARG;
+        if (kind[p] == PJ_BWD_BOTH && !pj_both_ok(R[p], K[p], cols[p], nsplit[p], ldx && ldx[p] > 0 ? ldx[p] : cols[p])) return GPTST_ESHAPE;
+    }
+    auto job = [&](int p) { return pj_make(emb[p], x[p], pool[p], out[p], out2 ? out2[p] : nullptr, R[p], K[p], cols[p], nsplit[p], kind[p], ldx ? ldx[p] : 0); };
     const bool det = g_deterministic != 0;
     std::vector<int> ord(njobs);
     std::vector<long> cost(njobs);
     for (int p = 0; p < njobs; ++p) {
         ord[p] = p;
         const long rr = (long)R[p] * nsplit[p], cc = cols[p];
-        cost[p] = kind[p] == PJ_BWD_POOL ? rr * (cc < 64 ? cc : 64) : kind[p] == PJ_BWD_EMB ? 16L * nsplit[p] * (cc < 1024 ? cc : 1024)
+        cost[p] = kind[p] == PJ_BWD_BOTH ? rr * (cc < 256 ? cc : 256) : kind[p] == PJ_BWD_POOL ? rr * (cc < 64 ? cc : 64) : kind[p] == PJ_BWD_EMB ? 16L * nsplit[p] * (cc < 1024 ? cc : 1024)
                 : kind[p] == PJ_FWD ? 64L * (cc < 256 ? cc : 256) : 1L;
     }
     if (g_pg_sort) std::stable_sort(ord.begin(), ord.end(), [&](int a, int b) { return cost[a] > cost[b]; });
@@ -236,6 +244,12 @@
     flush();
     GPTST_CHECK_LAUNCH();
     return GPTST_OK;
+}
+
+extern "C" int gptst_pool_jobs(int njobs, const int* kind, const void* const* emb, const void* const* x, const void* const* pool,
+                               const void* const* out, const int* R, const int* K, const int* cols, const int* nsplit, const int* ldx,
+                               void* stream) {
+    return gptst_pool_jobs2(njobs, kind, emb, x, pool, out, nullptr, R, K, cols, nsplit, ldx, stream);
 }
 
 extern thread_local int g_wgrad_ns_override;
@@ -276,7 +290,7 @@
     if (!emb || !pools || !outs || !cols || nprob <= 0 || nprob > PJ_MAX || K > PG_MAXK || K <= 0) return GPTST_EARG;
     PJobs t; t.n = nprob;
     for (int p = 0; p < nprob; ++p)
-        t.j[p] = PJob{emb, nullptr, ((const float* const*)pools)[p], ((float* const*)outs)[p], R, K, cols[p], 1, 0, PJ_FWD, 0, 0};
+        t.j[p] = pj_make(emb, nullptr, ((const float* const*)pools)[p], ((float* const*)outs)[p], nullptr, R, K, cols[p], 1, PJ_FWD, 0);
     return pj_launch(t, (hipStream_t)stream);
 }
 
@@ -285,8 +299,7 @@
     if (!emb || !dWs || !dpools || !cols || nprob <= 0 || nprob > PJ_MAX || K > PG_MAXK || K <= 0) return GPTST_EARG;
     PJobs t; t.n = nprob;
     for (int p = 0; p < nprob; ++p)
-        t.j[p] = PJob{emb, ((const float* const*)dWs)[p], nullptr, ((float* const*)dpools)[p], R, K, cols[p], nsplit ? nsplit[p] : 1, 0,
-                      PJ_BWD_POOL, 0, 0};
+        t.j[p] = pj_make(emb, ((const float* const*)dWs)[p], nullptr, ((float* const*)dpools)[p], nullptr, R, K, cols[p], nsplit ? nsplit[p] : 1, PJ_BWD_POOL, 0);
     return pj_launch(t, (hipStream_t)stream);
 }
 
@@ -295,8 +308,7 @@
     if (!dWs || !pools || !cols || !demb || nprob <= 0 || nprob > PJ_MAX || K > PG_MAXK || K <= 0) return GPTST_EARG;
     PJobs t; t.n = nprob;
     for (int p = 0; p < nprob; ++p)
-        t.j[p] = PJob{nullptr, ((const float* const*)dWs)[p], ((const float* const*)pools)[p], demb, R, K, cols[p], nsplit ? nsplit[p] : 1, 0,
-                      PJ_BWD_EMB, 0, 0};
+        t.j[p] = pj_make(nullptr, ((const float* const*)dWs)[p], ((const float* const*)pools)[p], demb, nullptr, R, K, cols[p], nsplit ? nsplit[p] : 1, PJ_BWD_EMB, 0);
     return pj_launch(t, (hipStream_t)stream);
 }
 
diff --git a/gpt-st_amd/csrc/poolgen_dev.h b/gpt-st_amd/csrc/poolgen_dev.h
--- a/gpt-st_amd/csrc/poolgen_dev.h
+++ b/gpt-st_amd/csrc/poolgen_dev.h
@@ -4,15 +4,28 @@
 #define PG_MAXK 16
 #define PG_MFMA_ROWS 64
 #define PJ_MAX 112
-enum { PJ_FWD = 0, PJ_BWD_POOL = 1, PJ_BWD_EMB = 2, PJ_GRAM = 3 };
+enum { PJ_FWD = 0, PJ_BWD_POOL = 1, PJ_BWD_EMB = 2, PJ_GRAM = 3, PJ_BWD_BOTH = 4 };
 struct PJob {
     const float* emb;
     const float* x;
     const float* pool;
     float* out;
-    int R, K, cols, nsplit;
-    int blk0, kind, nbx, ldx;
+    float* out2;
+    int R, cols;
+    int blk0, nbx, ldx;
+    unsigned char K, kind;
+    unsigned short nsplit;
 };
+static_assert(sizeof(PJob) == 64, "PJob: 64 B per job in the kernel arguments");
+__host__ __device__ inline PJob pj_make(const void* emb, const void* x, const void* pool, const void* out, const void* out2, int R, int K, int cols, int nsplit, int kind,
+                                        int ldx) {
+    PJob j;
+    j.emb = (const float*)emb; j.x = (const float*)x; j.pool = (const float*)pool; j.out = (float*)const_cast<void*>(out); j.out2 = (float*)const_cast<void*>(out2);
+    j.R = R; j.cols = cols; j.blk0 = 0; j.nbx = 0; j.ldx = ldx;
+    j.K = (unsigned char)((K < 0 || K > PG_MAXK) ? 0 : K); j.kind = (unsigned char)kind;
+    j.nsplit = (unsigned short)((nsplit < 0 || nsplit > 65535) ? 0 : nsplit);
+    return j;
+}
 struct PJobs { PJob j[PJ_MAX]; int n; };
 
 __device__ __forceinline__ void pj_fwd_mfma(const PJob& a, int bx, int by, int rows, int tid) {
@@ -219,3 +232,129 @@
         if (orow < a.R && i < a.K && (by * 4 + wave) * 256 < a.cols) atomicAdd(a.out + (size_t)orow * a.K + i, acc[r]);
     }
 }
+
+#define PJ_BOTH_MAXR 384
+#define PJ_BOTH_SCR (PJ_BOTH_MAXR * PG_MAXK)
+#define PJ_BOTH_NBAR 2
+__host__ __device__ inline bool pj_both_ok(int R, int K, int cols, int nsplit, int ldx) {
+    return R > 0 && R <= PJ_BOTH_MAXR && K > 0 && K <= PG_MAXK && cols > 0 && ((cols | ldx) & 3) == 0 && nsplit > 0 && (nsplit == 1 || R >= 16);
+}
+template <int V, bool PF>
+__device__ __forceinline__ void pj_bwd_both(const PJob& a, int bx, float* __restrict__ dacc, int tid) {
+    static_assert(V == 4, "the fused reduction serves float4 columns; scalar-column shapes are queued as kinds 1 + 2");
+    const float* __restrict__ emb = a.emb;
+    const float* __restrict__ dW = a.x;
+    const int cols = a.cols, R = a.R, K = a.K, RR = R * a.nsplit, ldx = a.ldx;
+    const int lane = tid & 63, wave = tid >> 6;
+    const int j = lane & 15, kk = lane >> 4;
+    for (int o = tid; o < R * PG_MAXK; o += 256) dacc[o] = 0.f;
+    __syncthreads();
+    const int c0 = bx * 256 + wave * 64, c = c0 + 4 * j;
+    const bool cok = c < cols;
+    f32x4 acc[4];
+#pragma unroll
+    for (int e = 0; e < 4; ++e) acc[e] = (f32x4){0.f, 0.f, 0.f, 0.f};
+    if (c0 < cols) {
+        const int cl = cok ? c : 0, jc = min(j, K - 1);
+        float4 pl[4];
+        int c2[4];
+#pragma unroll
+        for (int u = 0; u < 4; ++u) {
+            const int col = c0 + 16 * u + 4 * kk;
+            c2[u] = col < cols ? col : 0;
+            if (PF) pl[u] = (col < cols && j < K) ? ld4(a.pool + (size_t)jc * cols + col) : f4zero();
+        }
+        float av[4], avn[4];
+        float4 b[4], bn[4];
+        auto load1 = [&](int rb, int rsub, float (&av_)[4], float4 (&b_)[4]) {
+#pragma unroll
+            for (int u = 0; u < 4; ++u) {
+                const int row = min(rb + 4 * u + kk, RR - 1);
+                int er = row - rsub;
+                er = er >= R ? er - R : er;
+                av_[u] = emb[(size_t)er * K + jc];
+                b_[u] = ld4(dW + (size_t)row * ldx + cl);
+            }
+        };
+        int rsub = 0, cbeg = 0;
+        const int per = (((RR + 3) >> 2) + 15) & ~15;
+        if (PF) load1(0, 0, avn, bn);
+        for (int rb = 0; rb < RR; rb += 16) {
+            float4 a2[4];
+            const int row2 = min(rb + j, RR - 1);
+            if (PF) {
+#pragma unroll
+                for (int u = 0; u < 4; ++u) { av[u] = avn[u]; b[u] = bn[u]; }
+            } else {
+                load1(rb, rsub, av, b);
+            }
+            if (PF) {
+#pragma unroll
+                for (int u = 0; u < 4; ++u) a2[u] = ld4(dW + (size_t)row2 * ldx + c2[u]);
+            }
+            int rsubn = rsub;
+            if (rb + 16 - rsubn >= R && a.nsplit > 1) rsubn += R;
+            if (PF && rb + 16 < RR) load1(rb + 16, rsubn, avn, bn);
+            SB();
+#pragma unroll
+            for (int u = 0; u < 4; ++u) {
+                const float a_ = (rb + 4 * u + kk < RR && j < K) ? av[u] : 0.f;
+                acc[0] = __builtin_amdgcn_mfma_f32_16x16x4f32(a_, b[u].x, acc[0], 0, 0, 0);
+                acc[1] = __builtin_amdgcn_mfma_f32_16x16x4f32(a_, b[u].y, acc[1], 0, 0, 0);
+                acc[2] = __builtin_amdgcn_mfma_f32_16x16x4f32(a_, b[u].z, acc[2], 0, 0, 0);
+                acc[3] = __builtin_amdgcn_mfma_f32_16x16x4f32(a_, b[u].w, acc[3], 0, 0, 0);
+            }
+            f32x4 d = {0.f, 0.f, 0.f, 0.f};
+            const bool rok = rb + j < RR;
+#pragma unroll
+            for (int u = 0; u < 4; ++u) {
+                if (!PF && (u & 1) == 0) {
+                    SB();
+#pragma unroll
+                    for (int v = u; v < u + 2; ++v) {
+                        a2[v] = ld4(dW + (size_t)row2 * ldx + c2[v]);
+                        pl[v] = (c0 + 16 * v + 4 * kk < cols && j < K) ? ld4(a.pool + (size_t)jc * cols + c2[v]) : f4zero();
+                    }
+                    SB();
+                }
+                const float4 a_ = rok ? a2[u] : f4zero();
+                d = __builtin_amdgcn_mfma_f32_16x16x4f32(a_.x, pl[u].x, d, 0, 0, 0);
+                d = __builtin_amdgcn_mfma_f32_16x16x4f32(a_.y, pl[u].y, d, 0, 0, 0);
+                d = __builtin_amdgcn_mfma_f32_16x16x4f32(a_.z, pl[u].z, d, 0, 0, 0);
+                d = __builtin_amdgcn_mfma_f32_16x16x4f32(a_.w, pl[u].w, d, 0, 0, 0);
+            }
+#pragma unroll
+            for (int r = 0; r < 4; ++r) {
+                const int row = rb + 4 * kk + r;
+                int er = row - rsub;
+                er = er >= R ? er - R : er;
+                if (row < RR && j < K) atomicAdd(dacc + er * PG_MAXK + j, d[r]);
+            }
+            rsub = rsubn;
+            if (rb + 16 - cbeg >= per || rb + 16 >= RR) {
+                if (cok) {
+#pragma unroll 1
+                    for (int r = 0; r < 4; ++r) {
+                        const int k = 4 * kk + r;
+                        if (k < K) {
+                            float* p = a.out + (size_t)k * cols + c;
+                            const float4 o = ld4(p);
+                            const f32x4 a0 = acc[0], a1 = acc[1], a2_ = acc[2], a3 = acc[3];
+                            const float s0 = r == 0 ? a0[0] : r == 1 ? a0[1] : r == 2 ? a0[2] : a0[3], s1 = r == 0 ? a1[0] : r == 1 ? a1[1] : r == 2 ? a1[2] : a1[3];
+                            const float s2 = r == 0 ? a2_[0] : r == 1 ? a2_[1] : r == 2 ? a2_[2] : a2_[3], s3 = r == 0 ? a3[0] : r == 1 ? a3[1] : r == 2 ? a3[2] : a3[3];
+                            st4(p, make_float4(o.x + s0, o.y + s1, o.z + s2, o.w + s3));
+                        }
+                    }
+                }
+#pragma unroll
+                for (int e = 0; e < 4; ++e) acc[e] = (f32x4){0.f, 0.f, 0.f, 0.f};
+                cbeg = rb + 16;
+            }
+        }
+    }
+    __syncthreads();
+    for (int o = tid; o < R * PG_MAXK; o += 256) {
+        const int k = o & (PG_MAXK - 1);
+        if (k < K) atomicAdd(a.out2 + (size_t)(o >> 4) * K + k, dacc[o]);
+    }
+}
diff --git a/gpt-st_amd/engine.py b/gpt-st_amd/engine.py
--- a/gpt-st_amd/engine.py
+++ b/gpt-st_amd/engine.py
@@ -63,13 +63,27 @@
         self.on_bucket = None
         self.nbucket = 0
 
+    @property
+    def fuse(self):
+        return FUSE_RED and not self.no_carry and self.on_bucket is None and CTX.NODE_REDUCE is None
+
+    def pair(self, J, emb, parts, dpools, pools, demb):
+        if self.fuse:
+            for (dW, ns), dp, pl in zip(parts, dpools, pools):
+                J.bwd_both(emb, dW, pl, dp, demb, nsplit=ns)
+            return
+        for (dW, ns), dp in zip(parts, dpools):
+            J.bwd_pool(emb, dW, dp, nsplit=ns)
+        for (dW, ns), pl in zip(parts, pools):
+            J.bwd_emb(dW, pl, demb, nsplit=ns)
+
     def take_carry(self, mb):
         if not CARRY_RED or self.no_carry or self.on_bucket is not None or CTX.NODE_REDUCE is not None or not self.jobs.jobs:
             return None
         take, rest, nb = [], [], 0.0
         for j in self.jobs.jobs:
             b = 4.0 * j[5] * j[7] * j[8] / 2 ** 20
-            if j[0] in (ops.PoolJobs.BWD_POOL, ops.PoolJobs.BWD_EMB) and nb + b <= mb and len(take) < 100 and (j[7] | j[9]) % 4 == 0:
+            if j[0] in (ops.PoolJobs.BWD_POOL, ops.PoolJobs.BWD_EMB, ops.PoolJobs.BWD_BOTH) and nb + b <= mb and len(take) < 100 and (j[7] | j[9]) % 4 == 0:
                 take.append(j); nb += b
             else:
                 rest.append(j)
@@ -208,6 +222,7 @@
     return dx, (dWbt, ns, (dbias, nsb))
 
 
+FUSE_RED = os.environ.get("GPTST_FUSE_RED", "0") == "1"
 CARRY_RED = os.environ.get("GPTST_CARRY_RED", "1") == "1"
 CARRY_MB = float(os.environ.get("GPTST_CARRY_MB", "25"))
 CARRY_KL = os.environ.get("GPTST_CARRY_KL", "1") == "1"
@@ -404,10 +419,7 @@
         dWb, ns = ops.wgrad(x, dout, mode, B * T, N, D2=out, pro=PRO_DPRE, colsum_d=True)
         dW, db, nsb = dWb[:, :C * C], dWb[:, C * C:], ns
     dW = dW if dW.dim() == 2 else dW.view(ns * R, C * C)
-    red.jobs.bwd_pool(emb, dW, g_wpool.view(K, C * C), nsplit=ns)
-    red.jobs.bwd_pool(emb, db, g_bpool, nsplit=nsb)
-    red.jobs.bwd_emb(dW, wpool.view(K, C * C), d_emb, nsplit=ns)
-    red.jobs.bwd_emb(db, bpool, d_emb, nsplit=nsb)
+    red.pair(red.jobs, emb, [(dW, ns), (db, nsb)], [g_wpool.view(K, C * C), g_bpool], [wpool.view(K, C * C), bpool], d_emb)
     return dx
 
 
@@ -539,24 +551,18 @@
 
     def queue_ht(h, hp):
         dWbt, ns, (dbias, nsb) = hp
-        J.bwd_pool(time_eb, dWbt, g[h + "weights_pool"].view(d, CC), nsplit=ns)
-        J.bwd_pool(time_eb, dbias, g[h + "bias_pool"], nsplit=nsb)
-        J.bwd_emb(dWbt, p[h + "weights_pool"].view(d, CC), d_te, nsplit=ns)
-        J.bwd_emb(dbias, p[h + "bias_pool"], d_te, nsplit=nsb)
+        red.pair(J, time_eb, [(dWbt, ns), (dbias, nsb)], [g[h + "weights_pool"].view(d, CC), g[h + "bias_pool"]],
+                 [p[h + "weights_pool"].view(d, CC), p[h + "bias_pool"]], d_te)
 
     def queue_cap(c, cp):
         dWn, ns, (dbn, nsb), ddyn, dlogit = cp
         dW2 = dWn if dWn.dim() == 2 else dWn.view(ns * N, CC)
-        J.bwd_pool(nes, dW2, g[c + "weights_spa"].view(d, CC), nsplit=ns)
-        J.bwd_pool(nes, dbn, g[c + "bias_spa"], nsplit=nsb)
-        J.bwd_emb(dW2, p[c + "weights_spa"].view(d, CC), dnes, nsplit=ns)
-        J.bwd_emb(dbn, p[c + "bias_spa"], dnes, nsplit=nsb)
+        red.pair(J, nes, [(dW2, ns), (dbn, nsb)], [g[c + "weights_spa"].view(d, CC), g[c + "bias_spa"]],
+                 [p[c + "weights_spa"].view(d, CC), p[c + "bias_spa"]], dnes)
         dd2 = ddyn.view(B, HT * T * HS)
-        J.bwd_pool(tes, dd2, g[c + "t_adj"].view(ds, HT * T * HS))
-        J.bwd_emb(dd2, p[c + "t_adj"].view(ds, HT * T * HS), d_tes)
+        red.pair(J, tes, [(dd2, 1)], [g[c + "t_adj"].view(ds, HT * T * HS)], [p[c + "t_adj"].view(ds, HT * T * HS)], d_tes)
         dl2 = dlogit.view(BT, HS * N)
-        J.bwd_pool(teb, dl2, g[c + "adj"].view(ds, HS * N))
-        J.bwd_emb(dl2, p[c + "adj"].view(ds, HS * N), d_teb)
+        red.pair(J, teb, [(dl2, 1)], [g[c + "adj"].view(ds, HS * N)], [p[c + "adj"].view(ds, HS * N)], d_teb)
 
     if isinstance(dout, PendingH1):
         up = dout
@@ -608,8 +614,7 @@
     queue_ht(hts[0], hp1)
     red.gram(A_all.view(4 * N, Hm, T), dG_all, dA_all.view(4 * N, Hm, T), N, nsG)
     for i, h in enumerate(hts):
-        red.late.bwd_pool(ne, dA_all[i], g[h + "adj"].view(d, Hm * T))
-        red.late.bwd_emb(dA_all[i], p[h + "adj"].view(d, Hm * T), dne)
+        red.pair(red.late, ne, [(dA_all[i], 1)], [g[h + "adj"].view(d, Hm * T)], [p[h + "adj"].view(d, Hm * T)], dne)
     red.timefeat(p, g, pfx + "time_feature1.", tidx, d_te)
     red.timefeat(p, g, pfx + "time_feature1_.", tidx, d_teb)
     red.timefeat(p, g, pfx + "time_feature2.", tidx, d_tes, spg=True)
@@ -702,10 +707,8 @@
         K = neb.shape[1]
         dWb, dinp = carried[1] if carried[1] is not None else ops.guide_in_bwd(dh1, source, p[m + "ln1.weight"], p[m + "ln1.bias"], s1[1])
         dW, db = dWb[:, :C * C], dWb[:, C * C:]
-        red.jobs.bwd_pool(neb, dW, g[m + "weights_pool_spa"].view(K, C * C))
-        red.jobs.bwd_pool(neb, db, g[m + "bias_pool_spa"])
-        red.jobs.bwd_emb(dW, wpool.view(K, C * C), g["encoder.neb4mask"])
-        red.jobs.bwd_emb(db, bpool, g["encoder.neb4mask"])
+        red.pair(red.jobs, neb, [(dW, 1), (db, 1)], [g[m + "weights_pool_spa"].view(K, C * C), g[m + "bias_pool_spa"]], [wpool.view(K, C * C), bpool],
+                 g["encoder.neb4mask"])
         wb = _wb_view(g[m + "ln1.weight"], g[m + "ln1.bias"])
         if wb is not None:
             red.jobs.bwd_pool(_ones(dh1.device, N), dinp, wb)
diff --git a/gpt-st_amd/ops.py b/gpt-st_amd/ops.py
--- a/gpt-st_amd/ops.py
+++ b/gpt-st_amd/ops.py
@@ -1,3 +1,4 @@
+import threading
 import torch
 
 from . import _C
@@ -112,7 +113,8 @@
 
 
 class PoolJobs:
-    FWD, BWD_POOL, BWD_EMB, GRAM = 0, 1, 2, 3
+    FWD, BWD_POOL, BWD_EMB, GRAM, BWD_BOTH = 0, 1, 2, 3, 4
+    BOTH_MAXR = 384
 
     def __init__(self):
         self.jobs = []
@@ -155,12 +157,28 @@
         cols = pool.numel() // K
         self.jobs.append((self.BWD_EMB, None, dW, pool, demb, R, K, cols, nsplit, self._ldx(dW, cols)))
 
+    def bwd_both(self, emb, dW, pool, dpool, demb, nsplit=1, fused=True):
+        _chk(emb, pool, dpool, demb)
+        R, K = emb.shape
+        cols = dpool.numel() // K
+        ldx = self._ldx(dW, cols)
+        if not fused or _DET.on or (cols | ldx) % 4 or R > self.BOTH_MAXR or (nsplit > 1 and R < 16):
+            self.bwd_pool(emb, dW, dpool, nsplit=nsplit)
+            self.bwd_emb(dW, pool, demb, nsplit=nsplit)
+            return
+        assert tuple(demb.shape) == (R, K) and pool.numel() == K * cols
+        self.jobs.append((self.BWD_BOTH, emb, dW, pool, dpool, R, K, cols, nsplit, ldx, demb))
+
+    @staticmethod
+    def out2(js):
+        return _ptrs0([(j[10] if len(j) > 10 else None) for j in js])
+
     def launch(self):
         js, self.jobs = self.jobs, []
         post, self.post = self.post, []
         if js:
             col = lambda i: [j[i] for j in js]
-            _call("gptst_pool_jobs", len(js), _ints(col(0)), _ptrs0(col(1)), _ptrs0(col(2)), _ptrs0(col(3)), _ptrs0(col(4)), _ints(col(5)),
+            _call("gptst_pool_jobs2", len(js), _ints(col(0)), _ptrs0(col(1)), _ptrs0(col(2)), _ptrs0(col(3)), _ptrs0(col(4)), self.out2(js), _ints(col(5)),
                   _ints(col(6)), _ints(col(7)), _ints(col(8)), _ints(col(9)), nbytes=_nb(*[t for j in js for t in j[1:5]]))
         for A, G, rows, Hm in post:
             _call("gptst_gram_fwd", _p(A), _p(G), rows, Hm)
@@ -671,12 +689,12 @@
     ddyn = torch.empty_like(dyn)
     try:
         dS_ws = torch.empty(B * T, HS, C, device=dev, dtype=torch.float32) if flags is not None else None
-        js = jobs.jobs if jobs is not None and not jobs.post and all(j[0] in (PoolJobs.BWD_POOL, PoolJobs.BWD_EMB) for j in jobs.jobs) else []
+        js = jobs.jobs if jobs is not None and not jobs.post and all(j[0] in (PoolJobs.BWD_POOL, PoolJobs.BWD_EMB, PoolJobs.BWD_BOTH) for j in jobs.jobs) else []
         col = lambda i: [j[i] for j in js]
         _call("gptst_cap_cross_route_lin_bwd_split", _p(X), _p(Wp), _p(bp), _p(c), _p(dc1), _p(dv), _p(s), _p(Rt), _p(Ht), _p(dyn), _p(tmpl),
               _p(dPre), _p(out), int(bool(premul)), _p(dX), _p(dWp), _p(dbp), _p(dlogit), _p(ddyn), _p(dS_ws), _p(flags), B, T, N, C, HS, HT, nsplit,
-              len(js), _ints(col(0)), _ptrs0(col(1)), _ptrs0(col(2)), _ptrs0(col(3)), _ptrs0(col(4)), _ints(col(5)), _ints(col(6)), _ints(col(7)),
-              _ints(col(8)), _ints(col(9)), nbytes=_nb(X, Wp, bp, c, dc1, dv, s, Rt, dPre, out, dX, dWp, dlogit))
+              len(js), _ints(col(0)), _ptrs0(col(1)), _ptrs0(col(2)), _ptrs0(col(3)), _ptrs0(col(4)), PoolJobs.out2(js), _ints(col(5)), _ints(col(6)),
+              _ints(col(7)), _ints(col(8)), _ints(col(9)), nbytes=_nb(X, Wp, bp, c, dc1, dv, s, Rt, dPre, out, dX, dWp, dlogit))
         if js:
             jobs.jobs = []
     except _C.GptstError as e:
@@ -842,6 +860,14 @@
 
 def set_deterministic(on):
     _C.lib().call("gptst_set_deterministic", int(bool(on)))
+    _DET.on = bool(on)
+
+
+class _Det(threading.local):
+    on = False
+
+
+_DET = _Det()
 
 
 
diff --git a/include/gptst_hip.h b/include/gptst_hip.h
--- a/include/gptst_hip.h
+++ b/include/gptst_hip.h
@@ -9,7 +9,7 @@
 #pragma GCC visibility push(default)
 #endif
 
-#define GPTST_ABI_VERSION 16
+#define GPTST_ABI_VERSION 17
 int gptst_abi_version(void);
 int gptst_set_deterministic(int on);
 int gptst_handoff_timeouts(int* out);
@@ -34,6 +34,9 @@
 
 int gptst_pool_jobs(int njobs, const int* kind, const void* const* emb, const void* const* x, const void* const* pool,
                     const void* const* out, const int* R, const int* K, const int* cols, const int* nsplit, const int* ldx, void* stream);
+int gptst_pool_jobs2(int njobs, const int* kind, const void* const* emb, const void* const* x, const void* const* pool,
+                     const void* const* out, const void* const* out2, const int* R, const int* K, const int* cols, const int* nsplit,
+                     const int* ldx, void* stream);
 int gptst_pool_jobs_gram_rows(int K, int cols);
 
 int gptst_apply_nsplit(int mode, int BT, int N, int C);
@@ -131,7 +134,7 @@
                                         const float* dPre, const float* out, int premul, float* dX, float* dWp, float* dbp, float* dlogit,
                                         float* ddyn, float* dS_ws, void* flags, int B, int T, int N, int C, int HS, int HT, int nsplit,
                                         int njobs, const int* jkind, const void* const* jemb, const void* const* jx, const void* const* jpool,
-                                        const void* const* jout, const int* jR, const int* jK, const int* jcols, const int* jnsplit, const int* jldx,
+                                        const void* const* jout, const void* const* jout2, const int* jR, const int* jK, const int* jcols, const int* jnsplit, const int* jldx,
                                         void* stream);
 
 int gptst_cap_fits_lds(int N, int C, int HS);
```

Result: no change. 926.7 steps/s, median of 2 (+0.0%).
